# yhwu/rsicnv

Hardware: AMD Instinct MI355X
Metric: bases/sec through RSI pipeline (bin+GC+NB+segment) (higher is better)
Workload: dtype int32

## Files before the change

### include/rsi_hot.h

```cpp
#ifndef RSI_HOT_H
#define RSI_HOT_H
#include <stddef.h>
#include <stdint.h>
#ifdef __cplusplus
extern "C" {
#endif

typedef enum rsi_status {
  RSI_OK = 0,
  RSI_ERR_NO_DEVICE = -1,
  RSI_ERR_BAD_ARG = -2,
  RSI_ERR_HIP = -3,
  RSI_ERR_TOO_SMALL = -4,
  RSI_ERR_UNSUPPORTED = -5,
  RSI_ERR_INTERNAL = -6
} rsi_status;

typedef struct rsi_params {
  int32_t m;
  int32_t gcadjust;
  int32_t trans;
  int32_t merge;
  int32_t maxchkbp;
  int32_t debug;
// ... 259 lines not shown
void rsi_track_index_free(rsi_track_index* ix);
int rsi_hot_set_track_index(rsi_ctx* ctx, rsi_track_index* ix);
int rsi_track_index_append(rsi_track_index* dst, const rsi_track_index* src, int64_t shift);
int rsi_track_index_write_tbi(rsi_track_index* ix, const char* path);
int rsi_track_index_counts(const rsi_track_index* ix, int64_t* nref, int64_t* nchunks, int64_t* nwindows);
int64_t rsi_track_index_debug_tbi(const rsi_track_index* ix, uint8_t* out, int64_t cap);

int rsi_hot_loaded_depth(rsi_ctx* ctx, const void** d_depth, int64_t* n);
typedef struct rsi_depth_summary {
  int64_t n, sum;
  int64_t over;
  int64_t negative;
  int32_t min, max;
} rsi_depth_summary;
int rsi_hot_depth_summary(rsi_ctx* ctx, const void* d_depth, int64_t n, rsi_depth_summary* out, int64_t* dist, int dist_cap);
typedef struct rsi_depth_region { int64_t n, sum; int32_t min, max; } rsi_depth_region;
int rsi_hot_depth_regions(rsi_ctx* ctx, const void* d_depth, int64_t n, int nreg, const int64_t* start, const int64_t* end, rsi_depth_region* out);
int rsi_hot_write_window_track(rsi_ctx* ctx, const void* d_depth, int64_t n, const char* chrom, int64_t W, const char* path, int append,
                               rsi_track_stats* stats);
int rsi_hot_write_region_track(rsi_ctx* ctx, const void* d_depth, int64_t n, const char* chrom, int nreg, const int64_t* start,
                               const int64_t* end, const char* path, int append, rsi_track_stats* stats);
typedef struct rsi_depth_stats {
  int64_t launches;
  int64_t workgroups;
  int64_t bytes;
  double ms;
  double kernel_ms;
} rsi_depth_stats;
int rsi_hot_last_depth_stats(const rsi_ctx* ctx, rsi_depth_stats* out);
int rsi_hot_debug_depth_summary(rsi_ctx* ctx, const int32_t* values, int64_t n, int64_t span, rsi_depth_summary* out, int64_t* dist, int dist_cap);
int rsi_hot_debug_depth_regions(rsi_ctx* ctx, const int32_t* values, int64_t n, int tile, int nreg, const int64_t* start, const int64_t* end,
                                rsi_depth_region* out);
int64_t rsi_hot_debug_region_track(rsi_ctx* ctx, const int32_t* values, int64_t n, const char* chrom, int64_t W, int nreg, const int64_t* start,
                                   const int64_t* end, int span, int tile, int64_t slice_lines, int64_t pos0, char* out, int64_t cap,
                                   rsi_track_stats* stats);

int rsi_result_ncalls(const rsi_result* r, int which);
const rsi_call* rsi_result_calls(const rsi_result* r, int which);
const rsi_chrom_stats* rsi_result_stats(const rsi_result* r);
int rsi_result_noncode(const rsi_result* r, int32_t* pairs, int cap);
int rsi_result_format_row(const rsi_result* r, int i, const char* chrom, char* buf, int cap);
void rsi_result_free(rsi_result* r);

int64_t rsi_hot_fetch_i32(rsi_ctx* ctx, const char* name, int32_t* out, int64_t cap);
int64_t rsi_hot_fetch_f32(rsi_ctx* ctx, const char* name, float* out, int64_t cap);
int64_t rsi_hot_fetch_i64(rsi_ctx* ctx, const char* name, int64_t* out, int64_t cap);

int rsi_hot_debug_level_sums(rsi_ctx* ctx, const float* T, const int32_t* status, int64_t nb, int Lmax, float* sums, int32_t* counts);
int rsi_hot_debug_scan(rsi_ctx* ctx, const float* T, const int32_t* medint, int64_t nb, double RDmedian, double tmedian, double tlamda,
                       int Lmax, int32_t* status, int32_t* info);
int rsi_hot_debug_segments(rsi_ctx* ctx, const float* T, const int32_t* status, int64_t nb, const int32_t* runs, int nruns, double tmedian,
                           double tlamda, int64_t pairs_per_item, int32_t* seg_start, int32_t* seg_end, int32_t* seg_type, double* seg_score,
                           int32_t* info);
int rsi_hot_debug_sharpen(rsi_ctx* ctx, const int32_t* depth, int64_t n, int storage, int32_t* start, int32_t* end, const int32_t* type,
                          int njobs, int32_t* info);
typedef struct rsi_cand_record {
  int32_t capacity, top, margin, cut, nleft, nright;
  int32_t road;
  int32_t flags, nref, nbody, nwin, left_reach, right_reach, body_min, body_max;
  int32_t type, status, geno;
  double body_q[3], body_s1, body_s2, ref_q[3], ref_s1, ref_s2;
  double p1, cnvmed, cnvsd, cnviqr, refmed, refsd, refiqr;
} rsi_cand_record;
int rsi_hot_debug_candidate_tests(rsi_ctx* ctx, const int32_t* depth, int64_t n, int storage, int64_t span_all, double RDmedian, int m,
                                  double minmlen, double chklen, double buffer, int maxchkbp, const int32_t* start, const int32_t* end,
                                  const int32_t* type, const int32_t* status, int ncand, const int32_t* index, int nindex, int form,
                                  rsi_cand_record* out, int32_t* info);
int rsi_hot_debug_range_sums(rsi_ctx* ctx, const int32_t* depth, int64_t n, int storage, const int32_t* lo, const int32_t* hi, int nranges,
                             int64_t* sums, int32_t* info);
int rsi_hot_debug_block_stage(rsi_ctx* ctx, const int32_t* binmedint, const int32_t* status, int64_t nb, int64_t ncompact, double RDmedian,
                              const rsi_params* P, rsi_call* segs, int nsegs, int use_tester, int sparse, int32_t* road, int32_t* info);
int rsi_hot_debug_merge(rsi_ctx* ctx, const int32_t* depth, int64_t n, int storage, double RDmedian, const rsi_params* P, const rsi_call* list,
                        int nlist, int use_tester, rsi_call* out, int32_t* nout, int32_t* info);
int rsi_hot_debug_calls(rsi_ctx* ctx, const int32_t* depth, int64_t n, int storage, double RDmedian, double RDsd, const rsi_params* P,
                        const rsi_call* segs, int nsegs, const int32_t* noncode_start, const int32_t* noncode_end, int nnoncode, int use_tester,
                        rsi_call* blocks, rsi_call* raw, rsi_call* kept, int32_t* counts, int32_t* info);
int rsi_hot_debug_nb_transform(rsi_ctx* ctx, const int64_t* binsum, int64_t nb, int m, int64_t ncompact, double RDmedian, double r,
                               float* raw, float* T, int32_t* info);
int rsi_hot_debug_filterstatus(rsi_ctx* ctx, const float* T, const int32_t* status, int64_t nb, int Lmax, double dev, int32_t* status_out,
                               int32_t* info);
int rsi_hot_debug_grid_median(rsi_ctx* ctx, const float* x, const int32_t* mask, int64_t nb, int mode, double center, double* out,
                              int32_t* info);
int rsi_hot_debug_grid_mad_i32(rsi_ctx* ctx, const int32_t* x, int64_t nb, double center, double* out, int32_t* info);

int rsi_hot_debug_classify(rsi_ctx* ctx, const uint8_t* fasta, int64_t n, const int64_t* start, const int64_t* end, int count,
                           uint64_t* gcbits, uint64_t* nbits);

int rsi_hot_debug_per_base(rsi_ctx* ctx, const rsi_params* p, const int32_t* depth, const uint8_t* fasta, int64_t n, const int64_t* start,
                           const int64_t* end, int count, rsi_chrom_stats* out);

int rsi_hot_kernel_times(const rsi_ctx* ctx, const char** names, float* ms, int cap);
int rsi_hot_phase_times(const rsi_ctx* ctx, const char** names, double* ms, int cap);
void rsi_hot_set_timing(rsi_ctx* ctx, int on);
void rsi_hot_set_timing_kernel(rsi_ctx* ctx, const char* name);

typedef struct rsi_pool rsi_pool;
#define RSI_MAX_TIMED 64
typedef struct rsi_batch_times {
  int32_t nkernels, nphases;
  const char* kernel_name[RSI_MAX_TIMED];
  double kernel_ms[RSI_MAX_TIMED];
  int64_t kernel_launches[RSI_MAX_TIMED];
  int64_t kernel_bases[RSI_MAX_TIMED];
  const char* phase_name[RSI_MAX_TIMED];
  double phase_ms[RSI_MAX_TIMED];
} rsi_batch_times;

rsi_pool* rsi_pool_create(int device, int nworkers, int* status);
void rsi_pool_destroy(rsi_pool* pool);
int rsi_pool_workers(const rsi_pool* pool);
int rsi_pool_hw_queues(const rsi_pool* pool);
rsi_ctx* rsi_pool_worker(rsi_pool* pool, int w);
void rsi_pool_set_timing(rsi_pool* pool, int on);
void rsi_pool_set_timing_kernel(rsi_pool* pool, const char* name);
void rsi_pool_set_schedule(rsi_pool* pool, int isolate, int streamers);
const char* rsi_pool_last_error(const rsi_pool* pool);
int rsi_pool_run(rsi_pool* pool, const rsi_params* p, int nchrom, const void* const* d_depth,
                 const void* const* d_fasta, const int64_t* n, rsi_result** out, int* status,
                 rsi_batch_times* times);

int rsi_plot_expand(const int32_t* rdc, int64_t ncompact, const int32_t* regions, int npairs, int32_t* out, int64_t n);
int rsi_plot_write_files(const rsi_call* c, const char* title, const int32_t* rd, int64_t n, double chrom_median, int m,
                         double minmlen, double chklen, const char* format, double gnuplot_version, const char* datfile,
                         const char* gpfile, const char* imgfile);

typedef struct rsi_plot_batch rsi_plot_batch;
rsi_plot_batch* rsi_plot_batch_new(int64_t n, int m, double minmlen, double chklen);
void rsi_plot_batch_free(rsi_plot_batch* b);
int rsi_plot_batch_add(rsi_plot_batch* b, const rsi_call* c);
int rsi_plot_batch_add_span(rsi_plot_batch* b, int start, int end, int type);
int rsi_plot_batch_size(const rsi_plot_batch* b);
int rsi_plot_batch_refusal(const rsi_plot_batch* b, int i);
const char* rsi_plot_refusal_text(int refusal);
int64_t rsi_plot_batch_queries(const rsi_plot_batch* b);
int rsi_plot_batch_fill_host(rsi_plot_batch* b, const int32_t* rd, int64_t n);
double rsi_plot_batch_chrom_median(const rsi_plot_batch* b);
int rsi_plot_batch_compare(const rsi_plot_batch* a, const rsi_plot_batch* b);
int rsi_plot_batch_write(const rsi_plot_batch* b, int i, const char* title, const char* format, double gnuplot_version, const char* datfile,
                         const char* gpfile, const char* imgfile);
typedef struct rsi_plot_stats {
  int64_t launches, batches, tiles;
  int64_t calls, queries;
  int64_t bytes_up, bytes_down;
  int64_t bytes;
  double ms, expand_ms;
} rsi_plot_stats;
int rsi_hot_plot_depth(rsi_ctx* ctx, const void* d_depth, int64_t n, rsi_plot_batch* b);
int rsi_hot_plot_run(rsi_ctx* ctx, const rsi_result* res, rsi_plot_batch* b);
int rsi_hot_last_plot_stats(const rsi_ctx* ctx, rsi_plot_stats* out);
int rsi_hot_debug_plot(rsi_ctx* ctx, const int32_t* depth, int64_t n, int tile, int64_t workspace_bytes, rsi_plot_batch* b);
int rsi_hot_debug_plot_expand(rsi_ctx* ctx, const int32_t* rdc, int64_t ncompact, int storage, const int32_t* regions, int npairs, int32_t* out, int64_t n);

int rsi_pool_run_host(rsi_pool* pool, const rsi_params* p, int nchrom, const int32_t* const* depth,
                      const uint8_t* const* fasta, const int64_t* n, rsi_result** out, int* status,
                      rsi_batch_times* times);

uint64_t rsi_pool_submit(rsi_pool* pool, const rsi_params* p, int nchrom, const void* const* d_depth,
                         const void* const* d_fasta, const int64_t* n, rsi_result** out, int* status,
                         rsi_batch_times* times);
int rsi_pool_wait(rsi_pool* pool, uint64_t ticket);

#ifdef __cplusplus
}
#endif
#endif
```

### rsicnv_amd/api.py

```python
import contextlib
import ctypes as C
import os

import numpy as np

POOL_HW_QUEUES, MIN_HW_QUEUES = 32, 4


def _queue_count(s):
    return int(s) if s is not None and 1 <= len(s) <= 9 and all(c in "0123456789" for c in s) else -1


def _process_setup(env=os.environ):
    user = env.get("RSI_HOT_HW_QUEUES")
    if user != "keep":
        want = _queue_count(user)
        if want >= 0:
            env["GPU_MAX_HW_QUEUES"] = str(min(POOL_HW_QUEUES, max(MIN_HW_QUEUES, want)))
        elif _queue_count(env.get("GPU_MAX_HW_QUEUES")) < POOL_HW_QUEUES:
            env["GPU_MAX_HW_QUEUES"] = str(POOL_HW_QUEUES)
    return max(0, _queue_count(env.get("GPU_MAX_HW_QUEUES")))


HW_QUEUES = _process_setup()

_HERE = os.path.dirname(os.path.abspath(__file__))
LIB_PATH = os.environ.get("RSI_HOT_LIB") or os.path.join(_HERE, "librsi_hot.so")

RSI_OK = 0
STATUS_NAMES = {0: "RSI_OK", -1: "RSI_ERR_NO_DEVICE", -2: "RSI_ERR_BAD_ARG", -3: "RSI_ERR_HIP",
                -4: "RSI_ERR_TOO_SMALL", -5: "RSI_ERR_UNSUPPORTED", -6: "RSI_ERR_INTERNAL"}

CAND_RECORD = np.dtype([(k, np.int32) for k in ("capacity", "top", "margin", "cut", "nleft", "nright", "road", "flags", "nref", "nbody", "nwin",
                                                "left_reach", "right_reach", "body_min", "body_max", "type", "status", "geno")] +
                       [("body_q", np.float64, 3), ("body_s1", np.float64), ("body_s2", np.float64), ("ref_q", np.float64, 3),
                        ("ref_s1", np.float64), ("ref_s2", np.float64)] +
                       [(k, np.float64) for k in ("p1", "cnvmed", "cnvsd", "cnviqr", "refmed", "refsd", "refiqr")])
assert CAND_RECORD.itemsize == 18 * 4 + 17 * 8

CALL_RECORD = np.dtype([(k, np.int32) for k in ("start", "end", "type", "geno", "status", "length", "qscore", "pad")] +
                       [(k, np.float64) for k in ("score", "p1", "cnvmed", "cnvsd", "cnviqr", "refmed", "refsd", "refiqr")])
assert CALL_RECORD.itemsize == 8 * 4 + 8 * 8
LIST_INFO = ("spec_hits", "single_tests", "host_fallbacks", "block_batch_hits", "waits", "sum_launches", "sum_reused", "sum_redone", "tests")

GENO_RECORD = np.dtype([(k, np.int32) for k in ("n_body", "n_flank", "body_min", "body_max")] +
                       [("body_sum", np.int64), ("flank_sum", np.int64), ("body_q", np.float64, 3), ("flank_q", np.float64, 3),
                        ("chrom_median", np.float64)])
assert GENO_RECORD.itemsize == 4 * 4 + 2 * 8 + 7 * 8

DEPTH_SUMMARY = np.dtype([(k, np.int64) for k in ("n", "sum", "over", "negative")] + [("min", np.int32), ("max", np.int32)])
DEPTH_REGION = np.dtype([("n", np.int64), ("sum", np.int64), ("min", np.int32), ("max", np.int32)])
assert DEPTH_SUMMARY.itemsize == 40 and DEPTH_REGION.itemsize == 24
DEPTH_BINS = 65536

EXPORTS = ["rsi_default_params", "rsi_hot_create", "rsi_hot_destroy", "rsi_hot_last_error", "rsi_hot_run",
           "rsi_hot_run_device", "rsi_hot_load_depth_text", "rsi_hot_run_text", "rsi_hot_load_depth_bam", "rsi_hot_run_bam", "rsi_bam_references", "rsi_result_annotate_bam", "rsi_result_summary", "rsi_summary_format_row", "rsi_summary_format_rows", "rsi_result_pairs", "rsi_result_ncalls", "rsi_result_calls", "rsi_result_stats", "rsi_result_noncode",
           "rsi_result_format_row", "rsi_result_free", "rsi_hot_fetch_i32", "rsi_hot_fetch_f32", "rsi_hot_fetch_i64",
           "rsi_hot_kernel_times", "rsi_hot_phase_times", "rsi_hot_set_timing", "rsi_hot_process_setup", "rsi_pool_create", "rsi_pool_destroy", "rsi_pool_workers", "rsi_pool_hw_queues", "rsi_pool_worker",
           "rsi_pool_set_timing", "rsi_pool_set_timing_kernel", "rsi_hot_set_timing_kernel", "rsi_pool_set_schedule", "rsi_pool_last_error", "rsi_pool_run", "rsi_pool_run_host", "rsi_pool_submit", "rsi_pool_wait", "rsi_plot_expand", "rsi_plot_write_files", "rsi_result_log_line", "rsi_hot_debug_level_sums", "rsi_hot_debug_scan", "rsi_hot_debug_segments", "rsi_hot_debug_sharpen", "rsi_hot_debug_candidate_tests", "rsi_hot_debug_range_sums", "rsi_hot_debug_block_stage", "rsi_hot_debug_merge", "rsi_hot_debug_calls", "rsi_hot_debug_nb_transform", "rsi_hot_debug_filterstatus", "rsi_hot_debug_grid_median", "rsi_hot_debug_grid_mad_i32", "rsi_synth_generate_host", "rsi_synth_generate_device", "rsi_synth_write_depth_text", "rsi_synth_write_fasta", "rsi_synth_append_genome_text",
           "rsi_genome_text_open", "rsi_genome_text_next", "rsi_genome_text_release", "rsi_genome_text_copy_depth",
           "rsi_genome_text_kernel_ms", "rsi_genome_text_close", "rsi_genome_text_last_error", "rsi_hot_run_depth_device",
           "rsi_hot_last_inflate_stats", "rsi_hot_inflate_bgzf", "rsi_genome_text_inflate_stats",
           "rsi_synth_append_genome_bgzf", "rsi_genome_text_open_samples", "rsi_genome_text_samples", "rsi_genome_text_max_resident",
           "rsi_genome_text_sample_depth", "rsi_genome_text_copy_sample_depth", "rsi_synth_append_genome_samples",
           "rsi_genome_bedgraph_open", "rsi_synth_append_genome_bedgraph", "rsi_genome_bedgraph_open_indexed", "rsi_genome_text_index_range",
           "rsi_hot_set_exclude", "rsi_exclude_read_bed", "rsi_hot_debug_classify", "rsi_hot_debug_per_base",
           "rsi_hot_write_track", "rsi_hot_write_track_device", "rsi_hot_debug_track",
           "rsi_hot_write_bin_track", "rsi_hot_debug_bin_track",
           "rsi_hot_set_track_format", "rsi_hot_last_deflate_stats", "rsi_bgzf_write_eof", "rsi_hot_debug_deflate",
           "rsi_track_index_create", "rsi_track_index_free", "rsi_hot_set_track_index", "rsi_track_index_append",
           "rsi_track_index_write_tbi", "rsi_track_index_counts", "rsi_track_index_debug_tbi",
           "rsi_ref_open", "rsi_ref_close", "rsi_ref_last_error", "rsi_ref_count", "rsi_ref_sequence", "rsi_ref_find", "rsi_ref_format",
           "rsi_ref_index_path", "rsi_ref_load_device", "rsi_ref_load_host", "rsi_ref_device_alloc", "rsi_ref_device_free",
           "rsi_hot_run_text_dfasta", "rsi_hot_run_bam_dfasta",
           "rsi_hot_set_bam_read", "rsi_hot_last_bam_read_stats",
           "rsi_hot_set_bam_pairs", "rsi_result_annotate_device", "rsi_hot_last_pairs_stats", "rsi_hot_debug_pair_sample",
           "rsi_hot_debug_pair_annotate",
           "rsi_hot_set_bam_pin", "rsi_hot_stat_calls", "rsi_hot_pin_sample", "rsi_hot_pin_calls", "rsi_hot_last_pin_stats",
           "rsi_hot_debug_pin_sample", "rsi_hot_debug_pin_calls",
           "rsi_hot_geno_calls", "rsi_hot_last_geno_stats", "rsi_hot_debug_geno",
           "rsi_hot_loaded_depth", "rsi_hot_depth_summary", "rsi_hot_depth_regions", "rsi_hot_write_window_track", "rsi_hot_write_region_track",
           "rsi_hot_last_depth_stats", "rsi_hot_debug_depth_summary", "rsi_hot_debug_depth_regions", "rsi_hot_debug_region_track",
           "rsi_plot_batch_new", "rsi_plot_batch_free", "rsi_plot_batch_add", "rsi_plot_batch_add_span", "rsi_plot_batch_size",
           "rsi_plot_batch_refusal", "rsi_plot_refusal_text", "rsi_plot_batch_queries", "rsi_plot_batch_fill_host",
           "rsi_plot_batch_chrom_median", "rsi_plot_batch_compare", "rsi_plot_batch_write", "rsi_hot_plot_depth", "rsi_hot_plot_run", "rsi_hot_last_plot_stats",
           "rsi_hot_debug_plot", "rsi_hot_debug_plot_expand",
           "rsi_ref_debug_set_chunks", "rsi_ref_debug_fai_line", "rsi_ref_debug_ranges", "rsi_ref_debug_gzi", "rsi_ref_debug_cover"]


class RsiParams(C.Structure):
    _fields_ = [("m", C.c_int32), ("gcadjust", C.c_int32), ("trans", C.c_int32), ("merge", C.c_int32),
                ("maxchkbp", C.c_int32), ("debug", C.c_int32), ("cap", C.c_double), ("epsilon", C.c_double),
                ("threshold", C.c_double), ("chklen", C.c_double), ("minmlen", C.c_double),
                ("buffer", C.c_double), ("p", C.c_double)]


class RsiCall(C.Structure):
    _fields_ = [("start", C.c_int32), ("end", C.c_int32), ("type", C.c_int32), ("geno", C.c_int32),
                ("status", C.c_int32), ("length", C.c_int32), ("qscore", C.c_int32), ("pad", C.c_int32),
                ("score", C.c_double), ("p1", C.c_double), ("cnvmed", C.c_double), ("cnvsd", C.c_double),
                ("cnviqr", C.c_double), ("refmed", C.c_double), ("refsd", C.c_double), ("refiqr", C.c_double)]


class RsiChromStats(C.Structure):
    _fields_ = [("n", C.c_int64), ("n_compact", C.c_int64), ("nbins", C.c_int64), ("n_noncode", C.c_int32),
                ("Lmax", C.c_int32), ("gc_rdmean", C.c_double), ("cap_median", C.c_double), ("RDmedian", C.c_double),
                ("RDsd", C.c_double), ("nb_mad", C.c_double), ("nb_r", C.c_double), ("nb_tmin", C.c_double),
                ("tmedian1", C.c_double), ("tsigma1", C.c_double), ("tlamda1", C.c_double), ("tmedian2", C.c_double),
                ("tsigma2", C.c_double), ("tlamda2", C.c_double), ("trim_escapes", C.c_int32),
                ("inexact_sums", C.c_int32), ("t_device_ms", C.c_double), ("t_kernels_ms", C.c_double),
                ("byte_escapes", C.c_int64), ("scan_tiles", C.c_int32), ("scan_tiles_listed", C.c_int32)]


RSI_MAX_TIMED = 64
SUMMARY_HEAD, SUMMARY_CALL = 8, 8


class RsiTextStats(C.Structure):
    _fields_ = [("bytes", C.c_int64), ("lines", C.c_int64), ("stored", C.c_int64), ("beyond", C.c_int64),
                ("fallback", C.c_int32), ("pad", C.c_int32), ("t_total_ms", C.c_double), ("t_parse_kernel_ms", C.c_double)]


class RsiInflateStats(C.Structure):
    _fields_ = [("format", C.c_int32), ("eof_block", C.c_int32), ("input_error", C.c_int32), ("pad", C.c_int32), ("compressed_bytes", C.c_int64), ("text_bytes", C.c_int64),
                ("blocks", C.c_int64), ("t_inflate_kernel_ms", C.c_double), ("t_host_inflate_ms", C.c_double)]


class RsiTrackStats(C.Structure):
    _fields_ = [("n", C.c_int64), ("lines", C.c_int64), ("bytes", C.c_int64), ("slices", C.c_int64),
                ("t_total_ms", C.c_double), ("t_kernel_ms", C.c_double), ("t_write_ms", C.c_double)]


class RsiDeflateStats(C.Structure):
    _fields_ = [("members", C.c_int64), ("stored_members", C.c_int64), ("text_bytes", C.c_int64), ("file_bytes", C.c_int64),
                ("t_kernel_ms", C.c_double)]


INFLATE_FORMATS = {0: "text", 1: "bgzf", 2: "gzip"}
TRACK_FORMATS = {"text": 0, "bgzf": 1}


class RsiRefSeq(C.Structure):
# ... 589 lines not shown
                              maxchkbp=100000):
        d = np.ascontiguousarray(depth, dtype=np.int32)
        c = np.ascontiguousarray(cands, dtype=np.int32).reshape(-1, 4)
        cols = [np.ascontiguousarray(c[:, j]) for j in range(4)]
        ix = np.ascontiguousarray(index, dtype=np.int32).reshape(-1)
        out = np.zeros(max(ix.size, 1), dtype=CAND_RECORD)
        info = np.zeros(8, dtype=np.int32)
        self.lib.rsi_hot_debug_candidate_tests.argtypes = [C.c_void_p, C.c_void_p, C.c_int64, C.c_int, C.c_int64, C.c_double, C.c_int, C.c_double,
                                                           C.c_double, C.c_double, C.c_int, C.c_void_p, C.c_void_p, C.c_void_p, C.c_void_p, C.c_int,
                                                           C.c_void_p, C.c_int, C.c_int, C.c_void_p, C.c_void_p]
        self._check(self.lib.rsi_hot_debug_candidate_tests(self.ctx, d.ctypes.data, d.size, int(storage), int(span_all), float(RDmedian), int(m),
                                                           float(minmlen), float(chklen), float(buffer), int(maxchkbp), cols[0].ctypes.data,
                                                           cols[1].ctypes.data, cols[2].ctypes.data, cols[3].ctypes.data, c.shape[0],
                                                           ix.ctypes.data, ix.size, int(form), out.ctypes.data, info.ctypes.data))
        return out[:ix.size], info

    def debug_range_sums(self, depth, storage, lo, hi):
        d = np.ascontiguousarray(depth, dtype=np.int32)
        a = np.ascontiguousarray(lo, dtype=np.int32).reshape(-1)
        b = np.ascontiguousarray(hi, dtype=np.int32).reshape(-1)
        assert a.size == b.size
        sums = np.zeros(max(a.size, 1), dtype=np.int64)
        info = np.zeros(2, dtype=np.int32)
        self.lib.rsi_hot_debug_range_sums.argtypes = [C.c_void_p, C.c_void_p, C.c_int64, C.c_int, C.c_void_p, C.c_void_p, C.c_int, C.c_void_p, C.c_void_p]
        self._check(self.lib.rsi_hot_debug_range_sums(self.ctx, d.ctypes.data, d.size, int(storage), a.ctypes.data, b.ctypes.data, a.size,
                                                      sums.ctypes.data, info.ctypes.data))
        return sums[:a.size], info

    def debug_block_stage(self, binmedint, status, segs, ncompact, RDmedian, tester=True, sparse=False, **params):
        b = np.ascontiguousarray(binmedint, dtype=np.int32)
        st = np.ascontiguousarray(status, dtype=np.int32)
        assert b.size == st.size
        L = np.array(segs, dtype=CALL_RECORD).reshape(-1)
        road = np.full(max(L.size, 1), -1, dtype=np.int32)
        info = np.zeros(10, dtype=np.int32)
        P = make_params(**params)
        self.lib.rsi_hot_debug_block_stage.argtypes = [C.c_void_p, C.c_void_p, C.c_void_p, C.c_int64, C.c_int64, C.c_double, C.c_void_p, C.c_void_p,
                                                       C.c_int, C.c_int, C.c_int, C.c_void_p, C.c_void_p]
        self._check(self.lib.rsi_hot_debug_block_stage(self.ctx, b.ctypes.data, st.ctypes.data, b.size, int(ncompact), float(RDmedian), C.addressof(P),
                                                       L.ctypes.data, L.size, int(bool(tester)), int(bool(sparse)), road.ctypes.data, info.ctypes.data))
        return L, road[:L.size], dict(zip(LIST_INFO, (int(v) for v in info)))

    def debug_merge(self, depth, storage, cands, RDmedian, tester=True, **params):
        d = np.ascontiguousarray(depth, dtype=np.int32)
        L = np.ascontiguousarray(np.array(cands, dtype=CALL_RECORD).reshape(-1))
        out = np.zeros(max(L.size, 1), dtype=CALL_RECORD)
        nout = np.zeros(1, dtype=np.int32)
        info = np.zeros(10, dtype=np.int32)
        P = make_params(**params)
        self.lib.rsi_hot_debug_merge.argtypes = [C.c_void_p, C.c_void_p, C.c_int64, C.c_int, C.c_double, C.c_void_p, C.c_void_p, C.c_int, C.c_int,
                                                 C.c_void_p, C.c_void_p, C.c_void_p]
        self._check(self.lib.rsi_hot_debug_merge(self.ctx, d.ctypes.data, d.size, int(storage), float(RDmedian), C.addressof(P), L.ctypes.data, L.size,
                                                 int(bool(tester)), out.ctypes.data, nout.ctypes.data, info.ctypes.data))
        return out[:int(nout[0])], dict(zip(LIST_INFO, (int(v) for v in info)))

    def debug_calls(self, depth, storage, segs, noncode, RDmedian, RDsd, tester=True, **params):
        d = np.ascontiguousarray(depth, dtype=np.int32)
        L = np.ascontiguousarray(np.array(segs, dtype=CALL_RECORD).reshape(-1))
        nc = np.asarray(noncode, dtype=np.int32).reshape(-1, 2)
        a, b = np.ascontiguousarray(nc[:, 0]), np.ascontiguousarray(nc[:, 1])
        outs = [np.zeros(max(L.size, 1), dtype=CALL_RECORD) for _ in range(3)]
        counts = np.zeros(3, dtype=np.int32)
        info = np.zeros(10, dtype=np.int32)
        P = make_params(**params)
        self.lib.rsi_hot_debug_calls.argtypes = [C.c_void_p, C.c_void_p, C.c_int64, C.c_int, C.c_double, C.c_double, C.c_void_p, C.c_void_p, C.c_int,
                                                 C.c_void_p, C.c_void_p, C.c_int, C.c_int, C.c_void_p, C.c_void_p, C.c_void_p, C.c_void_p, C.c_void_p]
        self._check(self.lib.rsi_hot_debug_calls(self.ctx, d.ctypes.data, d.size, int(storage), float(RDmedian), float(RDsd), C.addressof(P),
                                                 L.ctypes.data, L.size, a.ctypes.data if a.size else None, b.ctypes.data if b.size else None, a.size,
                                                 int(bool(tester)), outs[0].ctypes.data, outs[1].ctypes.data, outs[2].ctypes.data, counts.ctypes.data,
                                                 info.ctypes.data))
        return outs[0][:counts[0]], outs[1][:counts[1]], outs[2][:counts[2]], dict(zip(LIST_INFO, (int(v) for v in info)))

    def debug_nb_transform(self, binsum, m, ncompact, RDmedian, r):
        b = np.ascontiguousarray(binsum, dtype=np.int64)
        raw = np.zeros(b.size, dtype=np.float32)
        T = np.zeros(b.size, dtype=np.float32)
        info = np.zeros(8, dtype=np.int32)
        self.lib.rsi_hot_debug_nb_transform.argtypes = [C.c_void_p, C.c_void_p, C.c_int64, C.c_int, C.c_int64, C.c_double, C.c_double, C.c_void_p,
                                                        C.c_void_p, C.c_void_p]
        self._check(self.lib.rsi_hot_debug_nb_transform(self.ctx, b.ctypes.data, b.size, int(m), int(ncompact), float(RDmedian), float(r),
                                                        raw.ctypes.data, T.ctypes.data, info.ctypes.data))
        return raw, T, info

    def debug_filterstatus(self, T, status, Lmax, dev):
        t = np.ascontiguousarray(T, dtype=np.float32)
        st = np.ascontiguousarray(status, dtype=np.int32)
        assert st.size == t.size
        out = np.zeros(t.size, dtype=np.int32)
        info = np.zeros(10, dtype=np.int32)
        self.lib.rsi_hot_debug_filterstatus.argtypes = [C.c_void_p, C.c_void_p, C.c_void_p, C.c_int64, C.c_int, C.c_double, C.c_void_p, C.c_void_p]
        self._check(self.lib.rsi_hot_debug_filterstatus(self.ctx, t.ctypes.data, st.ctypes.data, t.size, int(Lmax), float(dev), out.ctypes.data,
                                                        info.ctypes.data))
        return out, info

    GRID_MODES = {"pair": 0, "mad": 1, "host": 2}

    def debug_grid_median(self, x, mask=None, mode="pair", center=0.0):
        out = np.zeros(4, dtype=np.float64)
        info = np.zeros(8, dtype=np.int32)
        if mode == "med":
            assert mask is None
            xi = np.ascontiguousarray(x, dtype=np.int32)
            self.lib.rsi_hot_debug_grid_mad_i32.argtypes = [C.c_void_p, C.c_void_p, C.c_int64, C.c_double, C.c_void_p, C.c_void_p]
            self._check(self.lib.rsi_hot_debug_grid_mad_i32(self.ctx, xi.ctypes.data, xi.size, float(center), out.ctypes.data, info.ctypes.data))
            return out, info
        xf = np.ascontiguousarray(x, dtype=np.float32)
        mk = None if mask is None else np.ascontiguousarray(mask, dtype=np.int32)
        assert mk is None or mk.size == xf.size
        self.lib.rsi_hot_debug_grid_median.argtypes = [C.c_void_p, C.c_void_p, C.c_void_p, C.c_int64, C.c_int, C.c_double, C.c_void_p, C.c_void_p]
        self._check(self.lib.rsi_hot_debug_grid_median(self.ctx, xf.ctypes.data, None if mk is None else mk.ctypes.data, xf.size,
                                                       self.GRID_MODES[mode], float(center), out.ctypes.data, info.ctypes.data))
        return out, info

    def set_exclude(self, exclude):
        if exclude is None or len(exclude) == 0:
            self._check(self.lib.rsi_hot_set_exclude(self.ctx, None, None, 0))
            return
        s, e = _interval_arrays(exclude)
        self._check(self.lib.rsi_hot_set_exclude(self.ctx, s.ctypes.data, e.ctypes.data, s.size))

    def debug_classify(self, fasta, exclude=None):
        f = np.ascontiguousarray(fasta, dtype=np.uint8)
        gc = np.zeros(f.size // 64 + 1, dtype=np.uint64)
        nb = np.zeros(f.size // 64 + 1, dtype=np.uint64)
        if exclude is None or len(exclude) == 0:
            rc = self.lib.rsi_hot_debug_classify(self.ctx, f.ctypes.data, f.size, None, None, 0, gc.ctypes.data, nb.ctypes.data)
        else:
            s, e = _interval_arrays(exclude)
            rc = self.lib.rsi_hot_debug_classify(self.ctx, f.ctypes.data, f.size, s.ctypes.data, e.ctypes.data, s.size, gc.ctypes.data, nb.ctypes.data)
        self._check(rc)
        return gc, nb

    def debug_per_base(self, params, depth, fasta, exclude=None):
        d = np.ascontiguousarray(depth, dtype=np.int32)
        f = np.ascontiguousarray(fasta, dtype=np.uint8)
        if d.shape != f.shape or d.ndim != 1:
            raise ValueError("depth and fasta must be 1-D arrays of the same length")
        st = RsiChromStats()
        if exclude is None or len(exclude) == 0:
            rc = self.lib.rsi_hot_debug_per_base(self.ctx, C.byref(params), d.ctypes.data, f.ctypes.data, d.size, None, None, 0, C.byref(st))
        else:
            s, e = _interval_arrays(exclude)
            rc = self.lib.rsi_hot_debug_per_base(self.ctx, C.byref(params), d.ctypes.data, f.ctypes.data, d.size, s.ctypes.data, e.ctypes.data,
                                                 s.size, C.byref(st))
        self.last_stats = {k[0]: getattr(st, k[0]) for k in RsiChromStats._fields_}
        self._check(rc)
        return self.last_stats

    def run(self, params, depth, fasta, exclude=None):
        d = np.ascontiguousarray(depth, dtype=np.int32)
        f = np.ascontiguousarray(fasta, dtype=np.uint8)
        if d.shape != f.shape or d.ndim != 1:
            raise ValueError("depth and fasta must be 1-D arrays of the same length")
        out = C.c_void_p()
        if exclude is not None:
            self.set_exclude(exclude)
        self._check(self.lib.rsi_hot_run(self.ctx, C.byref(params), d.ctypes.data, f.ctypes.data, d.size, C.byref(out)))
        return Result(self.lib, out)

    def load_depth_text(self, path, n):
        st = RsiTextStats()
        self._check(self.lib.rsi_hot_load_depth_text(self.ctx, os.fsencode(path), int(n), C.byref(st)))
        return {f[0]: getattr(st, f[0]) for f in RsiTextStats._fields_ if f[0] != "pad"}

    def inflate_bgzf(self, data):
        data = bytes(data)
# ... 728 lines not shown
```

### rsicnv_amd/csrc/kernels.h

```cpp
#pragma once
#include <hip/hip_runtime.h>
#include <stdint.h>
#include <mutex>
#include "device_util.h"
#include "bam_walk_core.h"

namespace rsik {

inline void note_launch() {
  const hipError_t e = hipGetLastError();
  if (e != hipSuccess && tl_launch_error == hipSuccess) tl_launch_error = e;
}
inline void drain_stale_errors() { (void)hipGetLastError(); tl_launch_error = hipSuccess; }
inline hipError_t take_launch_error() { const hipError_t e = tl_launch_error; tl_launch_error = hipSuccess; return e; }
#define RSI_LAUNCH(...) do { hipLaunchKernelGGL(__VA_ARGS__); rsik::note_launch(); } while (0)

constexpr int kGcLevels = 202;
constexpr int kHistValues = 65536;
constexpr int kResClasses = 32;
constexpr int kTileBases = 4096;

void launch_fasta_classify(const uint8_t* fasta, int64_t n, uint64_t* gcbits, uint64_t* nbits, int64_t nwords,
                           const FillList& fill, hipStream_t stream);
void launch_fill(const FillList& fill, hipStream_t stream);
// ... 44 lines not shown
                        hipStream_t stream);

size_t gc_rescale_slab_bytes(int64_t n);
void launch_gc_rescale(const int32_t* depth, const uint64_t* gcbits, int64_t n, const double* table,
                       int adjust, int32_t* out, uint32_t* hist, ValueHistAux* aux, void* slabs, void* gsum,
                       unsigned int* counters, ValueMedian* vm, const void* head_src, void* head_dst, size_t head_bytes,
                       hipStream_t stream, uint8_t* out8 = nullptr,
                       PhaseParams* pp = nullptr ,
                       double cap_mult = 0.0);
void launch_gc_materialize(const int32_t* depth, const uint64_t* gcbits, int64_t n, const double* table, int32_t* out,
                           unsigned int* counter, hipStream_t stream);
size_t value_hist8_slab_bytes(int64_t n);
void launch_value_hist8(const uint8_t* depth8, const int32_t* depth, const uint64_t* gcbits, int64_t n, const double* table,
                        uint32_t* hist, ValueHistAux* aux, void* slabs, void* gsum, unsigned int* counters, ValueMedian* vm,
                        const void* head_src, void* head_dst, size_t head_bytes, uint8_t* rescaled8 ,
                        const unsigned int* escapes , hipStream_t stream);
unsigned int byte_escape_limit(int64_t n);

struct BinAccum {
  unsigned long long big;
  unsigned int vmax;
  unsigned int pad;
};
constexpr int kRegInline = 48;
struct K4Regions { long long brk[kRegInline]; long long cum[kRegInline + 1]; };
struct K4Form { int vr = 0, sw7 = -1, parts = 0, tile_bins = 0, tmpl = -1; };
struct K4Args {
  const int32_t* src; const uint8_t* src8; const uint64_t* gcbits; int64_t n; const double* table;
  const int64_t* cbreak; const int64_t* cum; const K4Regions* inl; int nreg; int64_t ncompact; int32_t capval; int m;
  uint8_t* rdc8; int32_t* rdc; int32_t* binmed; int64_t* binsum; uint32_t* res_hist; BinAccum* acc;
  void* slabs; void* gsum; unsigned int* counters; const void* exp_src; void* exp_dst; size_t exp_bytes;
  const unsigned int* rtab; const unsigned int* escapes; PhaseParams* pp; int vbase; int raw; hipStream_t stream;
  K4Form* form;
};
size_t cap_compact_slab_bytes(int m, int32_t capval, int64_t ncompact, int vbase);
int cap_compact_overwrites(int m, int32_t capval, int64_t ncompact, int vbase);
constexpr int kK4Window = 512;
int hist_window_base(double center, int width);
void launch_cap_compact_bin(const K4Args& a);

int cap_compact16_applies(int m, int32_t capval, int64_t ncompact);
size_t cap_compact16_slab_bytes(int m, int64_t ncompact);
void launch_cap_compact_bin16(const K4Args& a);

int cap_compact8_applies(int m, int32_t capval);
size_t cap_compact8_slab_bytes(int m, int32_t capval, int64_t ncompact);
struct ByteShape { int vr; bool sw7; bool operator==(const ByteShape& o) const { return vr == o.vr && sw7 == o.sw7; } };
inline ByteShape byte_shape(int32_t capval) { int vr = 64; while (vr < 256 && vr <= capval) vr <<= 1; return {vr, capval <= 127}; }
void launch_cap_compact_bin8(const K4Args& a);

void launch_rescale_compact_bin8(const K4Args& a);

int rescale_compact_split_applies(int m, int32_t capval, int64_t ncompact, int nreg);
size_t rescale_compact_split_slab_bytes(int32_t capval, int64_t ncompact);
size_t rescale_compact_split_rdc_bytes(int64_t ncompact);
void launch_rescale_compact_stream(const K4Args& a);
void launch_bin_median8(const K4Args& a);

struct PerBaseSwitches {
  bool joint;
  bool spec;
  bool k4j_fix;
  bool k4split;
  bool nogc_bytes;
  bool k4w;
  bool k1b_inside;
};
enum class K4Route { stream, joint, bytes, wide16, int32 };
struct K4Plan {
  K4Route route;
  bool fixed;
  bool raw;
  bool bytes_fit;
  ByteShape shape;
  const char* marks[2];
};
K4Plan k4_plan(bool gcadjust, bool capped, int32_t capval, int m, int64_t ncompact, int nreg, bool deep, bool joint_ok,
               const PerBaseSwitches& sw);

void launch_nb_raw(const int64_t* binsum, int64_t nb, int m, int64_t ncompact, double r, float* raw,
                   uint32_t* rawmin_bits, hipStream_t stream);
struct MinMaxF { uint32_t min_inv, max_bits; unsigned int nonfinite; unsigned int pad; };
struct GridMedian { double med, ymin; unsigned long long count; uint32_t np, flags; };
enum { kGridEmpty = 1, kGridNonFinite = 2, kGridDegenerate = 4, kGridTooWide = 8 };
struct GridChain { MinMaxF* mm; uint32_t* hist; uint32_t cap; unsigned int* counters; };
struct GridExport { const void* src[2]; void* dst[2]; size_t bytes[2]; };

void launch_nb_scale_minmax(float* x, int64_t nb, const uint32_t* rawmin_bits, double med_raw, double del_raw, double dup_raw,
                            double RDmedian, const GridChain& c, GridMedian* out, hipStream_t stream);
void launch_i32_to_f32_minmax(const int32_t* in, float* out_f, int64_t nb, double center, const GridChain& c, GridMedian* out,
                              hipStream_t stream);
void launch_minmax_f32(const float* x, const int32_t* mask, int64_t nb, int use_abs, double center, MinMaxF* mm,
                       hipStream_t stream);
void launch_hist_f32(const float* x, const int32_t* mask, int64_t nb, int use_abs, double center, double ymin,
                     uint32_t* hist, uint32_t np, hipStream_t stream);
void launch_minmax_plan(const float* x, const int32_t* mask, int64_t nb, int use_abs, double center, const double* d_center,
                        const GridChain& c, GridMedian* out, hipStream_t stream);
void launch_hist_walk(const float* x, const int32_t* mask, int64_t nb, int use_abs, double center, const double* d_center,
                      const GridChain& c, GridMedian* out, const GridExport* ex, const FillList* fill, hipStream_t stream);
bool hist_walk_pack16(int64_t nb);

struct ScanParams {
  int64_t nb;
  int32_t Lmax;
  int16_t pad;
  int16_t kcap;
  double tmedian;
  double lim_del;
  double lim_dup;
};
constexpr int kMaxScanL = 10400;
constexpr int kScanLdsL = 3800;
constexpr int kScanPad = 8;
constexpr int kThrInline = 232;
struct ScanThr { double del[kThrInline]; double dup[kThrInline]; };
void launch_rsi_scan(const float* T, const int32_t* medint, const ScanParams& sp, const double* thr_del,
                     const double* thr_dup, const ScanThr* inl, uint32_t* first_del, uint32_t* first_dup, uint32_t* counters,
                     uint32_t* tiles, void* tile_ws , hipStream_t stream);
size_t scan_tile_workspace_bytes(int Lmax);
constexpr int kMaxLevels = 10416;
inline int scan_level_stride(int Lmax) { return (Lmax + 1 + kScanPad + 3) & ~3; }
constexpr int kScanRecEscapes = 0, kScanRecInexact = 1, kScanRecStop = 2 , kScanRecTiles = 8, kScanRecLevels = 16;
constexpr size_t kScanWorkBytes = 64 + 2 * (size_t)kMaxLevels * 4;
void launch_level_stop(const uint32_t* first_del, const uint32_t* first_dup, int64_t nb, int32_t Lmax, uint32_t* work, void* both,
                       unsigned int* counter, void* host_copy, size_t host_bytes, hipStream_t stream);
void launch_resolve_runs(const uint32_t* first_del, const uint32_t* first_dup, const uint32_t* levels, int64_t nb, int32_t* status,
                         int32_t* copy, uint64_t* runs, uint32_t* count, uint32_t cap, unsigned int* counter, void* host_copy,
                         uint32_t host_entries, hipStream_t stream);

struct BestSeg { double score; int32_t start; int32_t len; };
struct SegItem { int32_t run; int32_t len; int32_t Lbeg; int32_t Lend; };
constexpr int kRunsInline = 200, kItemsInline = 150;
constexpr int kBestLds = 6144;
struct RunsInline { int32_t se[2 * kRunsInline]; int32_t off[kRunsInline]; };
struct ItemsInline { SegItem it[kItemsInline]; int32_t off[kRunsInline]; };
void launch_run_prefix(const float* T, const int32_t* run_start, const int32_t* run_end, const RunsInline* inl, int nruns,
                       const int64_t* poff, double* scratch, const int32_t* status, int32_t* status_out, hipStream_t stream);
void launch_best_items(const void* items, const ItemsInline* inl, int nitems, const int64_t* poff, const double* scratch,
                       double tmedian, BestSeg* out, hipStream_t stream);
void launch_trim_runs(const float* T, int32_t* status, const int32_t* run_start, const int32_t* run_end, const RunsInline* inl,
                      int nruns, double delthr, double addthr, hipStream_t stream);

size_t level_sums_head_bytes(int Lmax_cap);
size_t level_sums_workspace_bytes(int64_t nb, int32_t clist_cap, int Lmax_cap);
void launch_level_sums(const float* T, const int32_t* status, int64_t nb, int Lmax, void* ws, int Lmax_cap, int32_t clist_cap, float* out,
                       unsigned int* counter, void* host_copy, hipStream_t stream);

constexpr int kMaxDevices = 16;
void report_attribute_failure(const char* kernel, const char* what);
#define RSI_ALLOW_FULL_LDS(kernel)                                                                                  \
  do {                                                                                                              \
    static std::once_flag once__[rsik::kMaxDevices];                                                                \
    int dev__ = 0;                                                                                                  \
    if (hipGetDevice(&dev__) != hipSuccess || dev__ < 0 || dev__ >= rsik::kMaxDevices) dev__ = 0;                   \
    std::call_once(once__[dev__], [dev__] {                                                                         \
      hipFuncAttributes a__;                                                                                        \
      int lds__ = 0;                                                                                                \
      if (hipFuncGetAttributes(&a__, reinterpret_cast<const void*>(kernel)) != hipSuccess) {                        \
        rsik::report_attribute_failure(#kernel, "hipFuncGetAttributes"); return;                                    \
      }                                                                                                             \
      if (hipDeviceGetAttribute(&lds__, hipDeviceAttributeMaxSharedMemoryPerBlock, dev__) != hipSuccess || lds__ <= 0) \
        lds__ = 160 * 1024;                                                                                         \
      if (hipFuncSetAttribute(reinterpret_cast<const void*>(kernel), hipFuncAttributeMaxDynamicSharedMemorySize,   \
                              lds__ - (int)a__.sharedSizeBytes) != hipSuccess)                                      \
        rsik::report_attribute_failure(#kernel, "hipFuncSetAttribute(MaxDynamicSharedMemorySize)");                 \
    });                                                                                                             \
  } while (0)

constexpr unsigned kCandHistBins = 16384;
struct EdgeJob {
  int32_t start, end, type, pad;
};
struct CandJob {
  int32_t start, end;
  int32_t kind;
  int32_t margin;
  int32_t capacity;
  int32_t top;
  int32_t nleft, nright;
  int32_t left_off, right_off;
  int32_t budget;
  int32_t cut;
  double right_cap;
// ... 211 lines not shown
```

### rsicnv_amd/csrc/kernels_bin.hip

```cpp
#include <type_traits>
#include "kernels.h"
#include "device_util.h"

namespace rsik {

namespace {

constexpr int kThreads = 256;
constexpr int kMaxGrid = 256 * 2;

__device__ inline int lane_id() { return threadIdx.x & 63; }
inline int grid_for(int64_t items, int per_block) {
  int64_t g = (items + per_block - 1) / per_block;
  if (g < 1) g = 1;
  if (g > kMaxGrid) g = kMaxGrid;
  return (int)g;
}

__device__ inline uint32_t f32_key(float f) {
  const uint32_t b = __float_as_uint(f);
  return (b & 0x80000000u) ? ~b : (b | 0x80000000u);
}

__global__ __launch_bounds__(kThreads) void k_nb_raw(const int64_t* __restrict__ binsum, int64_t nb, int m,
                                                     int64_t ncompact, double r, float* __restrict__ raw,
                                                     uint32_t* __restrict__ rawmin_key) {
  uint32_t kmin = 0xffffffffu;
  for (int64_t b = (int64_t)blockIdx.x * kThreads + threadIdx.x; b < nb; b += (int64_t)gridDim.x * kThreads) {
    const int64_t i1 = b * m;
    int64_t i2 = b * m + m - 1;
    if (i2 > ncompact - 1) i2 = ncompact - 1;
    const double m2 = (double)(i2 - i1 + 1);
    const double sum = (double)binsum[b];
    const double q = (sum + 0.25) / (m2 * r - 0.5);
    const double t = 2.0 * sqrt(r) * log(sqrt(q) + sqrt(1.0 + q));
    const float f = (float)t;
    raw[b] = f;
    const uint32_t k = f32_key(f);
    kmin = k < kmin ? k : kmin;
  }
  for (int d = 32; d >= 1; d >>= 1) { const uint32_t o = __shfl_xor(kmin, d); kmin = o < kmin ? o : kmin; }
  __shared__ uint32_t s_min[kThreads / 64];
  if (lane_id() == 0) s_min[threadIdx.x >> 6] = kmin;
  __syncthreads();
  if (threadIdx.x == 0) {
    for (int w = 1; w < kThreads / 64; ++w) kmin = s_min[w] < kmin ? s_min[w] : kmin;
    if (kmin != 0xffffffffu) atomicMax(rawmin_key, ~kmin);
  }
}

__device__ inline float sel_value(const float* __restrict__ x, int64_t i, int use_abs, double center) {
  const float v = x[i];
  return use_abs ? (float)fabs((double)v - center) : v;
}

__device__ __forceinline__ void minmax_body(const float* __restrict__ x, const int32_t* __restrict__ mask, int64_t nb,
                                            int use_abs, double center, MinMaxF* __restrict__ mm) {
  uint32_t kmin = 0xffffffffu, kmax = 0;
  unsigned int bad = 0;
  for (int64_t i = (int64_t)blockIdx.x * kThreads + threadIdx.x; i < nb; i += (int64_t)gridDim.x * kThreads) {
    if (mask && mask[i] != 0) continue;
    const float v = sel_value(x, i, use_abs, center);
    if (!(fabsf(v) <= 3.0e38f)) bad = 1;
    const uint32_t k = f32_key(v);
    kmin = k < kmin ? k : kmin;
    kmax = k > kmax ? k : kmax;
  }
  for (int d = 32; d >= 1; d >>= 1) {
    const uint32_t a = __shfl_xor(kmin, d), b = __shfl_xor(kmax, d);
    kmin = a < kmin ? a : kmin; kmax = b > kmax ? b : kmax; bad |= __shfl_xor(bad, d);
  }
  __shared__ uint32_t s_min[kThreads / 64], s_max[kThreads / 64], s_bad[kThreads / 64];
  if (lane_id() == 0) { s_min[threadIdx.x >> 6] = kmin; s_max[threadIdx.x >> 6] = kmax; s_bad[threadIdx.x >> 6] = bad; }
  __syncthreads();
  if (threadIdx.x == 0) {
    for (int w = 1; w < kThreads / 64; ++w) { kmin = s_min[w] < kmin ? s_min[w] : kmin; kmax = s_max[w] > kmax ? s_max[w] : kmax; bad |= s_bad[w]; }
    if (kmin != 0xffffffffu) atomicMax(&mm->min_inv, ~kmin);
    if (kmax != 0) atomicMax(&mm->max_bits, kmax);
    if (bad) atomicOr(&mm->nonfinite, 1u);
  }
}

__global__ __launch_bounds__(kThreads) void k_minmax_f32(const float* __restrict__ x, const int32_t* __restrict__ mask,
                                                         int64_t nb, int use_abs, double center, MinMaxF* __restrict__ mm) {
  minmax_body(x, mask, nb, use_abs, center, mm);
}
constexpr uint32_t kLdsBins = 12288;

constexpr int kHistRun = 8;

template <bool PACK16 = false>
__device__ __forceinline__ void hist_body(const float* __restrict__ x, const int32_t* __restrict__ mask, int64_t nb, int use_abs,
                                          double center, double ymin, uint32_t* __restrict__ hist, uint32_t np, int use_lds,
                                          unsigned int* s_h) {
  const uint32_t nl = use_lds ? (np < (uint32_t)use_lds ? np : (uint32_t)use_lds) : 0;
  auto lds_add = [&](uint32_t k, uint32_t c) { if (PACK16) atomicAdd(&s_h[k >> 1], c << ((k & 1u) << 4)); else atomicAdd(&s_h[k], c); };
  auto bucket = [&](float v) {
    const double idx = ((double)v - ymin) / 0.01 + 0.5;
    uint32_t k = (uint32_t)(unsigned long long)idx;
    return k >= np ? np - 1 : k;
  };
  __shared__ uint32_t s_wb;
  if (threadIdx.x == 0) s_wb = 0u;
  if (use_lds) { for (uint32_t e = threadIdx.x; e < (PACK16 ? (nl + 1) / 2 : nl); e += kThreads) s_h[e] = 0; }
  if (use_lds && np > nl && threadIdx.x < 64) {
    const int lane = (int)threadIdx.x;
    const int64_t i = (int64_t)(((unsigned long long)(2 * lane + 1) * (unsigned long long)nb) >> 7);
    const bool valid = i < nb && !(mask && mask[i] != 0);
    const uint32_t k = valid ? bucket(sel_value(x, i, use_abs, center)) : 0xffffffffu;
    int rank = 0;
    for (int j = 0; j < 64; ++j) {
      const uint32_t kj = (uint32_t)__builtin_amdgcn_readlane((int)k, j);
      rank += (kj < k || (kj == k && j < lane)) ? 1 : 0;
    }
    const int nvalid = __popcll(__ballot(valid));
    if (valid && rank == nvalid / 2) s_wb = k < nl / 2 ? 0u : (k - nl / 2 > np - nl ? np - nl : k - nl / 2);
  }
  if (use_lds) __syncthreads();
  const uint32_t wb = use_lds ? s_wb : 0u;
  auto count = [&](uint32_t k, uint32_t c) { if (k - wb < nl) lds_add(k - wb, c); else atomicAdd(&hist[k], c); };
  const int64_t nchunks = (nb + kHistRun - 1) / kHistRun;
  for (int64_t c = (int64_t)blockIdx.x * kThreads + threadIdx.x; c < nchunks; c += (int64_t)gridDim.x * kThreads) {
    uint32_t pend_k = 0xffffffffu, pend_c = 0;
    const int64_t i0 = c * kHistRun, i1 = i0 + kHistRun < nb ? i0 + kHistRun : nb;
    auto one = [&](float xv) {
      const float v = use_abs ? (float)fabs((double)xv - center) : xv;
      const uint32_t k = bucket(v);
      if (k != pend_k) {
        if (pend_c) count(pend_k, pend_c);
        pend_k = k; pend_c = 0;
      }
      ++pend_c;
    };
    if (i1 - i0 == kHistRun) {
      static_assert(kHistRun == 8, "two quads per run");
      const float4 a = *reinterpret_cast<const float4*>(x + i0), b = *reinterpret_cast<const float4*>(x + i0 + 4);
      int4 ma = make_int4(0, 0, 0, 0), mb = ma;
      if (mask) { ma = *reinterpret_cast<const int4*>(mask + i0); mb = *reinterpret_cast<const int4*>(mask + i0 + 4); }
      const float xv[8] = {a.x, a.y, a.z, a.w, b.x, b.y, b.z, b.w};
      const int mv[8] = {ma.x, ma.y, ma.z, ma.w, mb.x, mb.y, mb.z, mb.w};
#pragma unroll
      for (int e = 0; e < 8; ++e) if (mv[e] == 0) one(xv[e]);
    } else {
      for (int64_t i = i0; i < i1; ++i) {
        if (mask && mask[i] != 0) continue;
        one(x[i]);
      }
    }
    if (pend_c) count(pend_k, pend_c);
  }
  if (use_lds) {
    __syncthreads();
    for (uint32_t e = threadIdx.x; e < nl; e += kThreads) {
      const unsigned int c = PACK16 ? (s_h[e >> 1] >> ((e & 1u) << 4)) & 0xffffu : s_h[e];
      if (c) atomicAdd(&hist[wb + e], c);
    }
  }
}

__global__ __launch_bounds__(kThreads) void k_hist_f32(const float* __restrict__ x, const int32_t* __restrict__ mask,
                                                       int64_t nb, int use_abs, double center, double ymin,
                                                       uint32_t* __restrict__ hist, uint32_t np, int use_lds) {
  extern __shared__ unsigned int s_h[];
  hist_body(x, mask, nb, use_abs, center, ymin, hist, np, use_lds, s_h);
}

__device__ inline float f32_unkey(uint32_t k) { return __uint_as_float((k & 0x80000000u) ? (k & 0x7fffffffu) : ~k); }

__device__ inline void grid_plan_block(MinMaxF* __restrict__ mm, uint32_t cap, uint32_t* __restrict__ hist, GridMedian* __restrict__ g) {
  const uint32_t kmin = ~ld_cg(&mm->min_inv), kmax = ld_cg(&mm->max_bits), bad = ld_cg(&mm->nonfinite);
  uint32_t flags = 0, np = 0;
  double ymin = 0.0;
  if (kmin == 0xffffffffu) flags = kGridEmpty;
  else if (bad) flags = kGridNonFinite;
  else {
    ymin = (double)f32_unkey(kmin);
    const double ymax = (double)f32_unkey(kmax);
    if ((ymax - ymin) < 0.01) flags = kGridDegenerate;
    else {
      const size_t n = (size_t)((ymax - ymin) / 0.01 + 2);
      if (n > cap) flags = kGridTooWide; else np = (uint32_t)n;
    }
  }
  for (uint32_t e = threadIdx.x; e < np; e += kThreads) hist[e] = 0;
  __syncthreads();
  if (threadIdx.x == 0) {
    g->med = 0.0; g->ymin = ymin; g->count = 0; g->np = np; g->flags = flags;
    mm->min_inv = 0; mm->max_bits = 0; mm->nonfinite = 0;
  }
}

__device__ inline void minmax_commit(uint32_t kmin, uint32_t kmax, unsigned int bad, MinMaxF* __restrict__ mm) {
  for (int d = 32; d >= 1; d >>= 1) {
    const uint32_t a = __shfl_xor(kmin, d), b = __shfl_xor(kmax, d);
    kmin = a < kmin ? a : kmin; kmax = b > kmax ? b : kmax; bad |= __shfl_xor(bad, d);
  }
  __shared__ uint32_t s_min[kThreads / 64], s_max[kThreads / 64], s_bad[kThreads / 64];
  if (lane_id() == 0) { s_min[threadIdx.x >> 6] = kmin; s_max[threadIdx.x >> 6] = kmax; s_bad[threadIdx.x >> 6] = bad; }
  __syncthreads();
  if (threadIdx.x == 0) {
    for (int w = 1; w < kThreads / 64; ++w) { kmin = s_min[w] < kmin ? s_min[w] : kmin; kmax = s_max[w] > kmax ? s_max[w] : kmax; bad |= s_bad[w]; }
    if (kmin != 0xffffffffu) atomicMax(&mm->min_inv, ~kmin);
    if (kmax != 0) atomicMax(&mm->max_bits, kmax);
    if (bad) atomicOr(&mm->nonfinite, 1u);
  }
}

__global__ __launch_bounds__(kThreads) void k_minmax_plan(const float* __restrict__ x, const int32_t* __restrict__ mask,
                                                          int64_t nb, int use_abs, double center, const double* __restrict__ center_ptr,
                                                          MinMaxF* __restrict__ mm, unsigned int* __restrict__ counter, uint32_t cap,
                                                          uint32_t* __restrict__ hist, GridMedian* __restrict__ g) {
  const double c = center_ptr ? *center_ptr : center;
  uint32_t kmin = 0xffffffffu, kmax = 0;
  unsigned int bad = 0;
  auto one = [&](float xv) {
    const float v = use_abs ? (float)fabs((double)xv - c) : xv;
    if (!(fabsf(v) <= 3.0e38f)) bad = 1;
    const uint32_t k = f32_key(v);
    kmin = k < kmin ? k : kmin;
    kmax = k > kmax ? k : kmax;
  };
  const int64_t stride = (int64_t)gridDim.x * kThreads;
  int64_t i = (int64_t)blockIdx.x * kThreads + threadIdx.x;
  for (; i + 3 * stride < nb; i += 4 * stride) {
    float xv[4]; int mv[4] = {0, 0, 0, 0};
#pragma unroll
    for (int e = 0; e < 4; ++e) xv[e] = x[i + e * stride];
    if (mask) {
#pragma unroll
      for (int e = 0; e < 4; ++e) mv[e] = mask[i + e * stride];
    }
#pragma unroll
    for (int e = 0; e < 4; ++e) if (mv[e] == 0) one(xv[e]);
  }
  for (; i < nb; i += stride) {
    if (mask && mask[i] != 0) continue;
    one(x[i]);
  }
  minmax_commit(kmin, kmax, bad, mm);
  if (last_block_done(counter)) grid_plan_block(mm, cap, hist, g);
}

struct ExportPair { const void* src[2]; void* dst[2]; unsigned int bytes[2]; };

__device__ inline void grid_walk_block(const uint32_t* __restrict__ hist, GridMedian* __restrict__ g) {
  __shared__ unsigned long long s_sum[kThreads];
  __shared__ unsigned long long s_seen;
  __shared__ unsigned int s_cross;
  const uint32_t np = g->np;
  const uint32_t chunk = (((np + kThreads - 1) / kThreads) + 3u) & ~3u;
  const uint32_t b0 = threadIdx.x * chunk < np ? threadIdx.x * chunk : np;
  const uint32_t b1 = b0 + chunk < np ? b0 + chunk : np;
  const __amdgpu_buffer_rsrc_t rs = coherent_buffer(hist);
  unsigned long long mine = 0;
  for (uint32_t b = b0; b < b1; b += 32) {
    u32x4 v[8];
#pragma unroll
    for (int j = 0; j < 8; ++j) { const uint32_t q = b + 4u * j; v[j] = ld_cg_buf_x4(rs, (q < b1 ? q : b0) * 4u, 0u); }
#pragma unroll
    for (int j = 0; j < 8; ++j) {
      const uint32_t q = b + 4u * j;
      const unsigned int c[4] = {v[j].x, v[j].y, v[j].z, v[j].w};
#pragma unroll
      for (int e = 0; e < 4; ++e) mine += q + e < b1 ? c[e] : 0u;
    }
  }
  s_sum[threadIdx.x] = mine;
  if (threadIdx.x == 0) s_cross = 0xffffffffu;
  __syncthreads();
  unsigned long long seen = 0, total = 0;
  for (int t = 0; t < kThreads; ++t) { const unsigned long long v = s_sum[t]; if (t < (int)threadIdx.x) seen += v; total += v; }
  const unsigned long long r2 = total / 2;
  unsigned long long* med_bits = reinterpret_cast<unsigned long long*>(&g->med);
  if (threadIdx.x == 0) { st_cg(&g->count, total); if (r2 == 0) st_cg(med_bits, (unsigned long long)__double_as_longlong(g->ymin)); }
  if (r2 != 0 && mine != 0 && seen < r2 && seen + mine >= r2) { s_cross = b0; s_seen = seen; }
  __syncthreads();
  const uint32_t cb = s_cross;
  if (cb == 0xffffffffu) return;
  const unsigned long long before = s_seen;
  const uint32_t ce = cb + chunk < np ? cb + chunk : np;
  const uint32_t per = (chunk + kThreads - 1) / kThreads;
  const uint32_t m0 = cb + threadIdx.x * per < ce ? cb + threadIdx.x * per : ce;
  const uint32_t m1 = m0 + per < ce ? m0 + per : ce;
  unsigned long long part = 0;
  for (uint32_t bb = m0; bb < m1; ++bb) part += ld_cg(hist + bb);
  __syncthreads();
  s_sum[threadIdx.x] = part;
  __syncthreads();
  unsigned long long run = before;
  for (int t = 0; t < (int)threadIdx.x; ++t) run += s_sum[t];
  if (part != 0 && run < r2 && run + part >= r2) {
    for (uint32_t bb = m0; bb < m1; ++bb) {
      const unsigned long long upto = run + ld_cg(hist + bb);
      if (run < r2 && upto >= r2) st_cg(med_bits, (unsigned long long)__double_as_longlong(g->ymin + (double)bb * 0.01));
      run = upto;
    }
  }
}

template <bool PACK16>
__global__ __launch_bounds__(kThreads) void k_hist_walk(const float* __restrict__ x, const int32_t* __restrict__ mask,
                                                        int64_t nb, int use_abs, double center,
                                                        const double* __restrict__ center_ptr,
                                                        GridMedian* __restrict__ g, uint32_t* __restrict__ hist,
                                                        unsigned int* __restrict__ counter, ExportPair ex, FillList fill, uint32_t lds_bins) {
  extern __shared__ unsigned int s_h[];
  fill_ranges(fill);
  if (!g->flags) {
    const uint32_t np = g->np;
    hist_body<PACK16>(x, mask, nb, use_abs, center_ptr ? *center_ptr : center, g->ymin, hist, np, (int)lds_bins, s_h);
  }
  if (!last_block_done(counter)) return;
  if (!g->flags) grid_walk_block(hist, g);
  sync_drained();
  for (int k = 0; k < 2; ++k) export_words(ex.dst[k], ex.src[k], ex.bytes[k]);
}

struct NbLevels { double med_raw, del_raw, dup_raw, RDmedian; };
__global__ __launch_bounds__(kThreads) void k_nb_scale_mm(float* __restrict__ x, int64_t nb, const uint32_t* __restrict__ rawmin_inv,
                                                          NbLevels lv, MinMaxF* __restrict__ mm, unsigned int* __restrict__ counter,
                                                          uint32_t cap, uint32_t* __restrict__ hist, GridMedian* __restrict__ g) {
  const uint32_t key = ~(*rawmin_inv);
  const double tmin = (double)__uint_as_float((key & 0x80000000u) ? (key & 0x7fffffffu) : ~key);
  const double med_nbt = lv.med_raw - tmin;
  const double del_s = (lv.del_raw - tmin) / med_nbt * lv.RDmedian, dup_s = (lv.dup_raw - tmin) / med_nbt * lv.RDmedian;
  const double med_s = med_nbt / med_nbt * lv.RDmedian;
  const float lev0 = (float)del_s, lev1 = (float)dup_s, lev2 = (float)med_s;
  uint32_t kmin = 0xffffffffu, kmax = 0;
  unsigned int bad = 0;
  for (int64_t b = (int64_t)blockIdx.x * kThreads + threadIdx.x; b < nb; b += (int64_t)gridDim.x * kThreads) {
    float v = x[b];
    v = (float)((double)v - tmin);
    v = (float)((double)v / med_nbt * lv.RDmedian);
    if (b == 0) v = lev0;
    if (b == 1) v = lev1;
    if (b == 2) v = lev2;
    x[b] = v;
    if (!(fabsf(v) <= 3.0e38f)) bad = 1;
    const uint32_t k = f32_key(v);
    kmin = k < kmin ? k : kmin;
    kmax = k > kmax ? k : kmax;
  }
  minmax_commit(kmin, kmax, bad, mm);
  if (last_block_done(counter)) grid_plan_block(mm, cap, hist, g);
}

__global__ __launch_bounds__(kThreads) void k_i32_to_f32_mm(const int32_t* __restrict__ in, float* __restrict__ out, int64_t nb,
                                                            double center, MinMaxF* __restrict__ mm, unsigned int* __restrict__ counter,
                                                            uint32_t cap, uint32_t* __restrict__ hist, GridMedian* __restrict__ g) {
  uint32_t kmin = 0xffffffffu, kmax = 0;
  unsigned int bad = 0;
  for (int64_t b = (int64_t)blockIdx.x * kThreads + threadIdx.x; b < nb; b += (int64_t)gridDim.x * kThreads) {
    const float f = (float)in[b];
    out[b] = f;
    const float v = (float)fabs((double)f - center);
    if (!(fabsf(v) <= 3.0e38f)) bad = 1;
    const uint32_t k = f32_key(v);
    kmin = k < kmin ? k : kmin;
    kmax = k > kmax ? k : kmax;
  }
  minmax_commit(kmin, kmax, bad, mm);
  if (last_block_done(counter)) grid_plan_block(mm, cap, hist, g);
}

constexpr int kScanTile = 256;
constexpr uint32_t kUnmarked = 0xffffffffu;

template <class IX>
struct ScanLdsT {
  using index = IX;
  double* P;
  double* tot;
  uint32_t* TB;
  int* M;
  IX* CB;
  IX* RB;
  IX* PF;
  int stride;
  int count, kcap;
  __device__ IX& C(int q, int x) const { return CB[(size_t)q * stride + x]; }
  __device__ IX& R(int q, int r) const { return RB[(size_t)q * stride + r]; }
  __device__ uint32_t* level(int side, int k) const { return TB + ((size_t)side * (kcap + 1) + k) * count; }
};
enum { kCL = 0, kCG = 1, kCTd = 2, kCTu = 3 };
constexpr int kScanNarrowL = 32000;

__host__ __device__ inline size_t scan_lds_bytes(int count, int kcap, int ix_bytes = 2) {
  size_t b = ((size_t)(count + 1) + kThreads) * sizeof(double);
  b += 2 * (size_t)(kcap + 1) * count * 4 + (size_t)count * 4;
  b += 9 * (size_t)(count + 2) * ix_bytes;
  return b;
}
template <class SL>
__device__ inline void scan_lds_carve(SL& S, double* sm, int count, int kcap) {
  S.count = count; S.kcap = kcap; S.stride = count + 2;
  S.P = sm;
  S.tot = S.P + count + 1;
  S.TB = reinterpret_cast<uint32_t*>(S.tot + kThreads);
  S.M = reinterpret_cast<int*>(S.TB + 2 * (size_t)(kcap + 1) * count);
  S.CB = reinterpret_cast<typename SL::index*>(S.M + count);
  S.RB = S.CB + 4 * (size_t)S.stride;
  S.PF = S.RB + 4 * (size_t)S.stride;
}

template <class SL>
__device__ inline int scan_next(const SL& S, int q, int x, int vhi) {
  const int r = S.C(q, x);
  return r < (int)S.C(q, S.count) ? (int)S.R(q, r) : vhi;
}
template <class SL>
__device__ inline int scan_prev(const SL& S, int q, int x, int vlo) {
  const int r = S.C(q, x + 1);
  return r > 0 ? (int)S.R(q, r - 1) : vlo - 1;
}
template <class SL>
__device__ inline void scan_mark(const SL& S, int side, int lo, int hi, int L) {
  const int len = hi - lo + 1;
  int k = 31 - __clz(len);
  k = k > S.kcap ? S.kcap : k;
  const int step = 1 << k;
  uint32_t* tab = S.level(side, k);
  for (int a = lo; a + step - 1 < hi; a += step) atomicMin(&tab[a], (uint32_t)L);
  atomicMin(&tab[hi - step + 1], (uint32_t)L);
}

template <class SL>
__device__ __noinline__ long long scan_hit_slow(int count, int kcap, int w0, int L, int side, int vlo, int vhi, int ends,
                                                uint32_t* counters, double* gtile ) {
  extern __shared__ __align__(16) double sm[];
  SL S;
  if (gtile) scan_lds_carve(S, gtile, count, kcap); else scan_lds_carve(S, sm, count, kcap);
  const int qm = side ? kCG : kCL, qt = side ? kCTu : kCTd;
  int i1 = scan_next(S, qt, w0, vhi);
  i1 = scan_next(S, qm, i1, vhi);
  int i2 = scan_prev(S, qt, w0 + L - 1, vlo);
  i2 = scan_prev(S, qm, i2, vlo);
  if (i1 >= vhi || i2 < vlo) {
    if ((i1 >= vhi && (ends & 2)) || (i2 < vlo && (ends & 1))) atomicAdd(&counters[0], 1u);
    return -1;
  }
  if (i1 <= i2) scan_mark(S, side, i1, i2, L);
  return (long long)i1 | ((long long)i2 << 32);
}

struct ScanTile { int vlo, vhi, fl_del, ce_dup, ends; double lim_del, lim_dup; double* gtile; };
// ... 650 lines not shown
#pragma unroll
      for (int u = 0; u < 4; ++u) { const int L = L0 + u; sum[u] = (L < it.Lend && j + L <= it.len) ? Q[j + L] - pj : 0.0; }
#pragma unroll
      for (int u = 0; u < 4; ++u) {
        const int L = L0 + u;
        if (L < it.Lend && j + L <= it.len) {
          const double score = fabs(sum[u] / dL[u] - tmedian) * sq[u];
          if (seg_better(score, L, j, bs, bL, bj)) { bs = score; bL = L; bj = j; }
        }
      }
    }
  }
  s_s[threadIdx.x] = bs; s_L[threadIdx.x] = bL; s_j[threadIdx.x] = bj;
  __syncthreads();
  for (int d = kThreads / 2; d >= 1; d >>= 1) {
    if ((int)threadIdx.x < d) {
      if (seg_better(s_s[threadIdx.x + d], s_L[threadIdx.x + d], s_j[threadIdx.x + d], s_s[threadIdx.x], s_L[threadIdx.x], s_j[threadIdx.x])) {
        s_s[threadIdx.x] = s_s[threadIdx.x + d]; s_L[threadIdx.x] = s_L[threadIdx.x + d]; s_j[threadIdx.x] = s_j[threadIdx.x + d];
      }
    }
    __syncthreads();
  }
  if (threadIdx.x == 0) { out[blockIdx.x].score = s_s[0]; out[blockIdx.x].start = s_j[0]; out[blockIdx.x].len = s_L[0]; }
}

}

static int bounded_grid(int64_t n, int per_block, int cap) { const int g = grid_for(n, per_block); return g > cap ? cap : g; }
void launch_nb_raw(const int64_t* binsum, int64_t nb, int m, int64_t ncompact, double r, float* raw, uint32_t* rawmin_bits,
                   hipStream_t stream) {
  int grid = grid_for(nb, kThreads * 4);
  if (grid > 1024) grid = 1024;
  RSI_LAUNCH(k_nb_raw, dim3(grid), dim3(kThreads), 0, stream, binsum, nb, m, ncompact, r, raw, rawmin_bits);
}
void launch_nb_scale_minmax(float* x, int64_t nb, const uint32_t* rawmin_bits, double med_raw, double del_raw, double dup_raw,
                            double RDmedian, const GridChain& c, GridMedian* out, hipStream_t stream) {
  NbLevels lv{med_raw, del_raw, dup_raw, RDmedian};
  RSI_LAUNCH(k_nb_scale_mm, dim3(bounded_grid(nb, kThreads * 4, 512)), dim3(kThreads), 0, stream, x, nb, rawmin_bits, lv, c.mm, c.counters, c.cap,
                     c.hist, out);
}
void launch_i32_to_f32_minmax(const int32_t* in, float* out_f, int64_t nb, double center, const GridChain& c, GridMedian* out,
                              hipStream_t stream) {
  RSI_LAUNCH(k_i32_to_f32_mm, dim3(bounded_grid(nb, kThreads * 4, 512)), dim3(kThreads), 0, stream, in, out_f, nb, center, c.mm, c.counters, c.cap,
                     c.hist, out);
}
void launch_minmax_f32(const float* x, const int32_t* mask, int64_t nb, int use_abs, double center, MinMaxF* mm,
                       hipStream_t stream) {
  RSI_LAUNCH(k_minmax_f32, dim3(grid_for(nb, kThreads * 16)), dim3(kThreads), 0, stream, x, mask, nb, use_abs, center, mm);
}
void launch_hist_f32(const float* x, const int32_t* mask, int64_t nb, int use_abs, double center, double ymin, uint32_t* hist,
                     uint32_t np, hipStream_t stream) {
  const int use_lds = (int)kLdsBins;
  const size_t lds = (size_t)(np < kLdsBins ? np : kLdsBins) * 4;
  RSI_ALLOW_FULL_LDS(k_hist_f32);
  int grid = grid_for(nb, kThreads * kHistRun * 8);
  if (grid > 128) grid = 128;
  RSI_LAUNCH(k_hist_f32, dim3(grid), dim3(kThreads), lds, stream, x, mask, nb, use_abs, center, ymin, hist, np, use_lds);
}
void launch_minmax_plan(const float* x, const int32_t* mask, int64_t nb, int use_abs, double center, const double* d_center,
                        const GridChain& c, GridMedian* out, hipStream_t stream) {
  RSI_LAUNCH(k_minmax_plan, dim3(bounded_grid(nb, kThreads * 16, 256)), dim3(kThreads), 0, stream, x, mask, nb, use_abs, center, d_center, c.mm,
                     c.counters, c.cap, c.hist, out);
}
static int hist_walk_grid(int64_t nb) { const int g = grid_for(nb, kThreads * kHistRun * 2); return g > 256 ? 256 : g; }
bool hist_walk_pack16(int64_t nb) {
  const int64_t run = (int64_t)kThreads * kHistRun, stride = (int64_t)hist_walk_grid(nb) * run;
  const int64_t tail = nb % stride;
  const int64_t most = nb / stride * run + (tail < run ? tail : run);
  return most < 65536;
}
void launch_hist_walk(const float* x, const int32_t* mask, int64_t nb, int use_abs, double center, const double* d_center,
                      const GridChain& c, GridMedian* out, const GridExport* ex, const FillList* fill, hipStream_t stream) {
  const uint32_t bins = kLdsBins;
  const int grid = hist_walk_grid(nb);
  const bool pack16 = hist_walk_pack16(nb);
  const size_t lds = pack16 ? (size_t)bins * 2 : (size_t)bins * 4;
  ExportPair e{};
  if (ex) for (int k = 0; k < 2; ++k) { e.src[k] = ex->src[k]; e.dst[k] = ex->dst[k]; e.bytes[k] = (unsigned int)ex->bytes[k]; }
  FillList f{};
  if (fill) f = *fill;
  if (pack16) RSI_LAUNCH(k_hist_walk<true>, dim3(grid), dim3(kThreads), lds, stream, x, mask, nb, use_abs, center, d_center, out, c.hist, c.counters + 1, e, f, bins);
  else { RSI_ALLOW_FULL_LDS(k_hist_walk<false>); RSI_LAUNCH(k_hist_walk<false>, dim3(grid), dim3(kThreads), lds, stream, x, mask, nb, use_abs, center, d_center, out, c.hist, c.counters + 1, e, f, bins); }
}
constexpr int kGTileGrid = 256;
constexpr size_t kGTileBudget = size_t(8) << 30;
struct ScanShape { int count, kcap, grid; bool gtile, wide; size_t tile_bytes; };
static ScanShape scan_tile_shape(int Lmax) {
  ScanShape sh;
  const int halo = Lmax / 2 + 1;
  sh.count = kScanTile + 2 * halo;
  sh.kcap = 0;
  while ((2 << sh.kcap) <= Lmax && sh.kcap < 6) ++sh.kcap;
  sh.gtile = Lmax > kScanLdsL;
  sh.wide = Lmax > kScanNarrowL;
  if (!sh.gtile) while (sh.kcap > 0 && scan_lds_bytes(sh.count, sh.kcap) + 4 * kThreads * sizeof(int) + 1024 > 160 * 1024) --sh.kcap;
  sh.tile_bytes = scan_lds_bytes(sh.count, sh.kcap, sh.wide ? 4 : 2);
  sh.grid = kGTileGrid;
  if (sh.gtile) {
    const size_t slice = (sh.tile_bytes + 255) & ~size_t(255);
    if (slice * (size_t)sh.grid > kGTileBudget) sh.grid = (int)std::max<size_t>(1, kGTileBudget / slice);
  }
  return sh;
}
size_t scan_tile_workspace_bytes(int Lmax) {
  const ScanShape sh = scan_tile_shape(Lmax);
  return sh.gtile ? (size_t)sh.grid * ((sh.tile_bytes + 255) & ~size_t(255)) : 0;
}
void launch_rsi_scan(const float* T, const int32_t* medint, const ScanParams& sp_in, const double* thr_del, const double* thr_dup,
                     const ScanThr* inl, uint32_t* first_del, uint32_t* first_dup, uint32_t* counters, uint32_t* tiles, void* tile_ws,
                     hipStream_t stream) {
  ScanParams sp = sp_in;
  const ScanShape sh = scan_tile_shape(sp.Lmax);
  const bool gtile = sh.gtile;
  sp.kcap = (int16_t)sh.kcap;
  const size_t tile_bytes = sh.tile_bytes;
  const size_t lds = gtile ? 0 : tile_bytes;
  const unsigned long long gbytes = (tile_bytes + 255) & ~size_t(255);
  const int64_t ntiles = (sp.nb + kScanTile - 1) / kScanTile;
  static const ScanThr none{};
  const char* det_env = getenv("RSI_HOT_SCAN_DETECT");
  const size_t dlds = detect_lds_bytes(sp.Lmax);
  const bool detect = tiles != nullptr && !(det_env && atoi(det_env) == 0) && dlds + kThreads * 8 + 64 <= 160 * 1024;
  int parts = 1;
  if (detect || gtile) {
    const int groups = (sp.Lmax + kScanPad - 1) / kScanPad;
    parts = groups < kScanPartsMax ? groups : kScanPartsMax;
    if (const char* pe = getenv("RSI_HOT_SCAN_PARTS")) { const int v = atoi(pe); if (v >= 1 && v <= groups) parts = v; }
  }
  if (detect) {
    const int dgrid = (int)((sp.nb + kDetBins - 1) / kDetBins);
    if (inl) { RSI_ALLOW_FULL_LDS(k_scan_detect<true>); RSI_LAUNCH(k_scan_detect<true>, dim3(dgrid), dim3(kThreads), dlds, stream, T, sp.nb, sp.Lmax, nullptr, nullptr, tiles, counters, *inl); }
    else { RSI_ALLOW_FULL_LDS(k_scan_detect<false>); RSI_LAUNCH(k_scan_detect<false>, dim3(dgrid), dim3(kThreads), dlds, stream, T, sp.nb, sp.Lmax, thr_del, thr_dup, tiles, counters, none); }
  }
  int64_t grid = ntiles * parts;
  const int64_t resident = gtile ? sh.grid : 256 * (int64_t)(lds > 80 * 1024 ? 1 : lds > 52 * 1024 ? 2 : lds > 39 * 1024 ? 3 : 4);
  if ((detect || gtile) && grid > resident) grid = resident;
  const uint32_t* list = detect ? tiles : nullptr;
  unsigned char* gws = static_cast<unsigned char*>(tile_ws);
#define RSI_SCAN(INL_, GT_, WIDE_, ...) do { RSI_ALLOW_FULL_LDS((k_rsi_scan<INL_, GT_, WIDE_>));                                             \
    RSI_LAUNCH((k_rsi_scan<INL_, GT_, WIDE_>), dim3((unsigned)grid), dim3(kThreads), lds, stream, T, medint, sp, __VA_ARGS__, first_del, first_dup, \
               counters, list, parts, inl ? *inl : none, gws, gbytes); } while (0)
  if (gtile && sh.wide) RSI_SCAN(false, true, true, thr_del, thr_dup);
  else if (gtile) { if (inl) RSI_SCAN(true, true, false, nullptr, nullptr); else RSI_SCAN(false, true, false, thr_del, thr_dup); }
  else { if (inl) RSI_SCAN(true, false, false, nullptr, nullptr); else RSI_SCAN(false, false, false, thr_del, thr_dup); }
#undef RSI_SCAN
}
void launch_level_stop(const uint32_t* first_del, const uint32_t* first_dup, int64_t nb, int32_t Lmax, uint32_t* work, void* both,
                       unsigned int* counter, void* host_copy, size_t host_bytes, hipStream_t stream) {
  const size_t lds = (size_t)(Lmax + 1) * 8;
  if (lds + 256 <= 160 * 1024) {
    RSI_ALLOW_FULL_LDS(k_level_stop<false>);
    RSI_LAUNCH(k_level_stop<false>, dim3(grid_for(nb, kThreads * 16)), dim3(kThreads), lds, stream, first_del, first_dup, nb,
                       Lmax, work, static_cast<uint2*>(both), counter, host_copy, (unsigned int)host_bytes);
  } else {
    RSI_LAUNCH(k_level_stop<true>, dim3(grid_for(nb, kThreads * 16)), dim3(kThreads), 0, stream, first_del, first_dup, nb,
                       Lmax, work, static_cast<uint2*>(both), counter, host_copy, (unsigned int)host_bytes);
  }
}
void launch_resolve_runs(const uint32_t* first_del, const uint32_t* first_dup, const uint32_t* levels, int64_t nb, int32_t* status,
                         int32_t* copy, uint64_t* runs, uint32_t* count, uint32_t cap, unsigned int* counter, void* host_copy,
                         uint32_t host_entries, hipStream_t stream) {
  RSI_LAUNCH(k_resolve_runs, dim3(grid_for(nb, kThreads * 4)), dim3(kThreads), 0, stream, first_del, first_dup, levels, nb, status, copy,
                     runs, count, cap, counter, host_copy, host_entries);
}
void launch_trim_runs(const float* T, int32_t* status, const int32_t* run_start, const int32_t* run_end, const RunsInline* inl, int nruns,
                      double delthr, double addthr, hipStream_t stream) {
// ... 22 lines not shown
```

### rsicnv_amd/csrc/pipeline.hip

```cpp
#include <new>
#include "pipeline_internal.h"
#include "geno_host.h"
#include "pipeline_steps.h"

using namespace rsik;
using namespace rsip;
using rsih::Candidate;
using rsih::Region;

namespace {

struct ScanOut {
  double tmedian1 = 0, tsigma1 = 0, tlamda1 = 0, tmedian2 = 0, tsigma2 = 0, tlamda2 = 0;
  int Lmax = 0;
  rsih::IntSpan status2;
  std::vector<int> run_status;
  std::vector<rsih::IntSpan::Range> run_ranges;
  std::vector<Candidate> segs;
  uint32_t escapes = 0, inexact = 0;
  uint32_t tiles_listed = 0;
  std::vector<uint32_t> level_log[4];
  uint32_t stop_levels[4] = {0, 0, 0, 0};
  std::vector<std::string> fs_lines;
};
// ... 25 lines not shown
int grid_median(rsi_ctx* ctx, const float* d_x, const int32_t* d_mask, int64_t nb, int use_abs, double center,
                double* med, uint64_t* count) {
  uint8_t* small = ctx->small.as<uint8_t>();
  { Timer t(ctx, "minmax_f32"); launch_minmax_f32(d_x, d_mask, nb, use_abs, center, reinterpret_cast<MinMaxF*>(small + kOffMinMax), ctx->stream); }
  MinMaxF mm;
  HIPCHK(copy_d2h(ctx, &mm, small + kOffMinMax, sizeof(mm)));
  HIPCHK(hipMemsetAsync(small + kOffMinMax, 0, sizeof(MinMaxF), ctx->stream));
  HIPCHK(CTX_SYNC());
  if (mm.min_inv == 0u) { *count = 0; *med = 0; return RSI_OK; }
  if (mm.nonfinite) return fail(ctx, RSI_ERR_UNSUPPORTED, "non-finite value in the transformed bins");
  const double ymin = rsih::unkey_f32(~mm.min_inv), ymax = rsih::unkey_f32(mm.max_bits);
  if ((ymax - ymin) < 0.01) return selection_mean(ctx, d_x, d_mask, nb, use_abs, center, med, count);
  const size_t np = (size_t)((ymax - ymin) / 0.01 + 2);
  if (np > (64u << 20)) return fail(ctx, RSI_ERR_UNSUPPORTED, "transformed bin range too wide for the 0.01 grid");
  HIPCHK(ctx->hist_f.ensure(np * 4));
  HIPCHK(hipMemsetAsync(ctx->hist_f.p, 0, np * 4, ctx->stream));
  { Timer t(ctx, "hist_f32"); launch_hist_f32(d_x, d_mask, nb, use_abs, center, ymin, ctx->hist_f.as<uint32_t>(), (uint32_t)np, ctx->stream); }
  std::vector<uint32_t> h(np);
  HIPCHK(copy_d2h(ctx, h.data(), ctx->hist_f.p, np * 4));
  HIPCHK(CTX_SYNC());
  uint64_t total = 0;
  for (uint32_t c : h) total += c;
  *count = total;
  *med = rsih::hist_median_grid(h.data(), np, total, ymin);
  return RSI_OK;
}

constexpr uint32_t kGridCap = 1u << 20;
constexpr int32_t kFsListCap = 1 << 20;
struct ChainOut { GridMedian g[2]; uint32_t rawmin_inv; uint32_t pad[15]; };
GridChain grid_chain(rsi_ctx* ctx) {
  uint8_t* small = ctx->small.as<uint8_t>();
  return GridChain{reinterpret_cast<MinMaxF*>(small + kOffMinMax), ctx->hist_f.as<uint32_t>(), kGridCap,
                   reinterpret_cast<unsigned int*>(small + kOffDone) + kDoneBinSlot};
}
int nb_transform(rsi_ctx* ctx, const int64_t* d_binsum, int64_t nb, int m, int64_t ncompact, double RDmedian, double r, rsih::NbLevels& lev,
                 float* raw_out) {
  uint8_t* small = ctx->small.as<uint8_t>();
  hipStream_t st = ctx->stream;
  HIPCHK(ctx->tnb.ensure((size_t)nb * 4));
  HIPCHK(ctx->hist_f.ensure((size_t)kGridCap * 4));
  uint32_t* d_rawmin = reinterpret_cast<uint32_t*>(small + kOffRawMin);
  GridMedian* d_g = reinterpret_cast<GridMedian*>(small + kOffGrid);
  { Timer t(ctx, "nb_raw"); launch_nb_raw(d_binsum, nb, m, ncompact, r, ctx->tnb.as<float>(), d_rawmin, st); }
  if (raw_out) HIPCHK(hipMemcpyAsync(raw_out, ctx->tnb.p, (size_t)nb * 4, hipMemcpyDeviceToHost, st));
  lev = rsih::nb_reference_levels(RDmedian, m, r);
  { Timer t(ctx, "nb_scale"); launch_nb_scale_minmax(ctx->tnb.as<float>(), nb, d_rawmin, lev.med_raw, lev.del_raw, lev.dup_raw, RDmedian, grid_chain(ctx), d_g, st); }
  return RSI_OK;
}
void scan_fill_list(rsi_ctx* ctx, int pass, int64_t nb, FillList& fl) {
  uint8_t* small = ctx->small.as<uint8_t>();
  uint32_t* d_first_del = ctx->first_del.as<uint32_t>();
  const int64_t nbpad = (nb + 3) & ~int64_t(3);
  fill_add(fl, d_first_del, (size_t)(nbpad + nb) * 4, 0xffffffffu);
  fill_add(fl, small + kOffScanPass + (size_t)pass * kScanPassBytes, kScanPassBytes, 0u);
  fill_add(fl, small + kOffCounters, 32, 0u);
  if (pass == 0 && ctx->fs_ws.p) fill_add(fl, ctx->fs_ws.p, level_sums_head_bytes(kMaxL), 0u);
}
int grid_pair_issue(rsi_ctx* ctx, const float* d_x, const int32_t* d_mask, int64_t nb, bool with_median, double center, bool planned,
                    int fill_pass, ChainOut** out) {
  uint8_t* small = ctx->small.as<uint8_t>();
  GridMedian* d_g = reinterpret_cast<GridMedian*>(small + kOffGrid);
  const GridChain gc = grid_chain(ctx);
  ChainOut* slot = static_cast<ChainOut*>(mb_alloc(ctx, sizeof(ChainOut)));
  if (!slot) return fail(ctx, RSI_ERR_INTERNAL, "out of pinned mailbox memory");
  memset(slot, 0, sizeof(*slot));
  GateShared gs(ctx);
  if (with_median) {
    if (!planned) { Timer t(ctx, "minmax_plan"); launch_minmax_plan(d_x, d_mask, nb, 0, 0.0, nullptr, gc, d_g, ctx->stream); }
    { Timer t(ctx, "hist_walk"); launch_hist_walk(d_x, d_mask, nb, 0, 0.0, nullptr, gc, d_g, nullptr, nullptr, ctx->stream); }
    planned = false;
  }
  const double* d_center = with_median ? &d_g->med : nullptr;
  if (!planned) { Timer t(ctx, "minmax_plan"); launch_minmax_plan(d_x, d_mask, nb, 1, center, d_center, gc, d_g + 1, ctx->stream); }
  GridExport ex{};
  ex.src[0] = d_g; ex.dst[0] = slot->g; ex.bytes[0] = 2 * sizeof(GridMedian);
  ex.src[1] = small + kOffRawMin; ex.dst[1] = &slot->rawmin_inv; ex.bytes[1] = 4;
  FillList fl{};
  if (fill_pass >= 0) scan_fill_list(ctx, fill_pass, nb, fl);
  { Timer t(ctx, "hist_walk"); launch_hist_walk(d_x, d_mask, nb, 1, center, d_center, gc, d_g + 1, &ex, &fl, ctx->stream); }
  *out = slot;
  return RSI_OK;
}
struct Selection { const float* d_x; const int32_t* d_mask; int64_t nb; int use_abs; double center; };
int grid_result(rsi_ctx* ctx, const GridMedian& g, const Selection& sel, double* med, uint64_t* count) {
  if (g.flags & kGridEmpty) { *count = 0; *med = 0; return RSI_OK; }
  if (g.flags & kGridNonFinite) return fail(ctx, RSI_ERR_UNSUPPORTED, "non-finite value in the transformed bins");
  if (g.flags & kGridDegenerate) return selection_mean(ctx, sel.d_x, sel.d_mask, sel.nb, sel.use_abs, sel.center, med, count);
  *med = g.med; *count = g.count;
  return RSI_OK;
}

void scan_thresholds(double tmedian, double tlamda, int Lmax, std::vector<double>& del, std::vector<double>& dup) {
  del.assign((size_t)Lmax + 1 + kScanPad, -INFINITY);
  dup.assign((size_t)Lmax + 1 + kScanPad, INFINITY);
  del[0] = -1.0;
  for (int L = 1; L <= Lmax; ++L) {
    const double dL = (double)L, sq = sqrt(dL);
    auto score = [&](double sum) { const float meanf = (float)(sum / dL); return ((double)meanf - tmedian) * sq; };
    del[L] = rsih::last_true([&](double s) { return !(score(s) > -tlamda); });
    dup[L] = rsih::first_true([&](double s) { return !(score(s) < tlamda); });
  }
}

constexpr uint32_t kEagerBounds = 1024;
int runs_from_export(rsi_ctx* ctx, const uint32_t* slot, const uint64_t* d_list, std::vector<Region>& runs) {
  const uint32_t cnt = slot[0];
  runs.clear();
  if (cnt == 0) return RSI_OK;
  if (cnt > kMaxRunEntries) return fail(ctx, RSI_ERR_UNSUPPORTED, "boundary list overflow");
  std::vector<uint64_t> raw(cnt);
  memcpy(raw.data(), slot + 2, (size_t)std::min(cnt, kEagerBounds) * 8);
  if (cnt > kEagerBounds) {
    HIPCHK(copy_d2h(ctx, raw.data() + kEagerBounds, d_list + kEagerBounds, (size_t)(cnt - kEagerBounds) * 8));
    HIPCHK(CTX_SYNC());
  }
  if (!rsih::boundary_pairs(raw.data(), raw.size(), false, runs)) return fail(ctx, RSI_ERR_INTERNAL, "unbalanced run boundaries");
  runs.pop_back();
  return RSI_OK;
}

struct RunArgs { RunsInline inl; bool use_inl = false; int32_t* d_start = nullptr; int32_t* d_end = nullptr; };
int prepare_runs(rsi_ctx* ctx, const std::vector<Region>& runs, RunArgs& ra) {
  const size_t k = runs.size();
  if (k <= (size_t)kRunsInline) {
    memset(&ra.inl, 0, sizeof(ra.inl));
    for (size_t i = 0; i < k; ++i) { ra.inl.se[2 * i] = runs[i].start; ra.inl.se[2 * i + 1] = runs[i].end; }
    ra.use_inl = true;
    return RSI_OK;
  }
  HIPCHK(ctx->run_se.ensure(k * 8 + 64));
  std::vector<int32_t> se(2 * k);
  for (size_t i = 0; i < k; ++i) { se[i] = runs[i].start; se[k + i] = runs[i].end; }
  HIPCHK(copy_h2d(ctx, ctx->run_se.p, se.data(), k * 8));
  ra.use_inl = false;
  ra.d_start = ctx->run_se.as<int32_t>();
  ra.d_end = ctx->run_se.as<int32_t>() + k;
  return RSI_OK;
}

constexpr size_t kCandScratchBytes = size_t(512) << 20;
class DeviceTester : public rsih::NeighbourTester {
 public:
  DeviceTester(rsi_ctx* c, DepthRef rdc, int64_t n, double RDmedian) : ctx(c), d_rdc(rdc), N(n), median(RDmedian) {}
  double kernel_wait_ms = 0;
  int launches = 0;
  int force_split = -1, force_bytes = -1;
  std::vector<CandOut>* sink = nullptr;
  int mailbox_lists = 0, copied_lists = 0;

  bool sharpen(std::vector<Candidate>& L) override {
    if (L.empty()) return true;
    const int nj = (int)L.size();
    EdgeJob* slot = static_cast<EdgeJob*>(mb_alloc(ctx, (size_t)nj * sizeof(EdgeJob)));
    std::vector<EdgeJob> spill;
    EdgeJob* jobs = slot;
    if (!slot) { spill.resize((size_t)nj); jobs = spill.data(); }
    for (int i = 0; i < nj; ++i) jobs[i] = {L[(size_t)i].start, L[(size_t)i].end, L[(size_t)i].type, 0};
    {
      Phase ph(ctx, "cand.ensure");
      if (nj > ctx->sharpen_ws_jobs) {
        const int cap = std::max(256, 2 * nj);
        if (!ok(ctx->sharpen_ws.ensure(sharpen_workspace_bytes(cap)))) return false;
        if (!ok(hipMemsetAsync(ctx->sharpen_ws.p, 0, sharpen_workspace_zero_bytes(cap), ctx->stream))) return false;
        ctx->sharpen_ws_jobs = cap;
      }
// ... 271 lines not shown
    int64_t* d_poff = reinterpret_cast<int64_t*>(d_scratch + poff.back());
    HIPCHK(ctx->items.ensure(items.size() * sizeof(SegItem)));
    HIPCHK(ctx->best.ensure(items.size() * sizeof(BestSeg)));
    HIPCHK(copy_h2d(ctx, d_poff, poff.data(), poff.size() * 8));
    HIPCHK(copy_h2d(ctx, ctx->items.p, items.data(), items.size() * sizeof(SegItem)));
    HIPCHK(ctx->h_status2.ensure((size_t)nb * 4));
    HIPCHK(hipMemcpyAsync(ctx->h_status2.p, d_st2, (size_t)nb * 4, hipMemcpyDeviceToHost, ctx->stream));
    out.status2 = rsih::IntSpan(ctx->h_status2.as<int>(), nb);
    { Timer t(ctx, "run_prefix"); launch_run_prefix(d_T, ctx->run_se.as<int32_t>(), ctx->run_se.as<int32_t>() + kr, nullptr, (int)kr, d_poff, d_scratch, nullptr, nullptr, ctx->stream); }
    { Timer t(ctx, "best_subsegment"); launch_best_items(ctx->items.p, nullptr, (int)items.size(), d_poff, d_scratch, tmedian, ctx->best.as<BestSeg>(), ctx->stream); }
    HIPCHK(copy_d2h(ctx, best.data(), ctx->best.p, items.size() * sizeof(BestSeg)));
    HIPCHK(CTX_SYNC());
  }
  if (form) {
    form->runs = (int)runs.size(); form->items = (int)items.size(); form->inl = inl ? 1 : 0;
    form->mailbox_status = out.status2.ranges ? 1 : 0;
    form->pairs_per_item = pairs_per_item;
    for (const Region& r : runs) if (r.end - r.start + 2 > kBestLds) ++form->unstaged;
  }
  rsih::segments_from_best(runs, items, best.data(), out.status2, tlamda, out.segs);
  return RSI_OK;
}

struct FsForm { int runs = -1, inl = -1, copied = -1, route = 0, has_level0 = 0, trim = 0, leveldel = 0, leveladd = 0; float m0 = 0.0f; };
template <class Synced>
int rsi_filterstatus(rsi_ctx* ctx, const float* d_T, const int32_t* d_st1, int32_t* d_st1f, int64_t nb, int Lmax, double dev,
                     const uint32_t* rslot, Synced&& synced, std::vector<std::string>* fs_lines, FsForm* form) {
  int rc;
  const bool long_scan = Lmax > kMaxL;
  const int nlev = 2 * Lmax + 1;
  uint32_t* fs_slot = long_scan ? nullptr : static_cast<uint32_t*>(mb_alloc(ctx, (size_t)nlev * 8));
  if (!fs_slot && !long_scan) return fail(ctx, RSI_ERR_INTERNAL, "out of pinned mailbox memory");
  if (!long_scan) {
    GateShared gs(ctx);
    Timer t(ctx, "level_sums");
    launch_level_sums(d_T, d_st1, nb, Lmax, ctx->fs_ws.p, kMaxL, kFsListCap, ctx->fs_out.as<float>(),
                      reinterpret_cast<unsigned int*>(ctx->small.as<uint8_t>() + kOffDone) + kDoneBinSlot + 4, fs_slot, ctx->stream);
  }
  { Phase phc(ctx, "fs.wait"); HIPCHK(CTX_SYNC()); }
  if ((rc = synced()) != RSI_OK) return rc;
  {
    Phase phs(ctx, "fs.sums");
    std::vector<float> wsum((size_t)nlev, 0.0f);
    std::vector<int> wcnt((size_t)nlev, 0);
    if (fs_slot) {
      memcpy(wsum.data(), fs_slot, (size_t)nlev * 4);
      memcpy(wcnt.data(), fs_slot + nlev, (size_t)nlev * 4);
    }
    if (form) form->route = long_scan ? 2 : (wcnt[(size_t)Lmax] < 0 ? 1 : 0);
    if (long_scan || wcnt[(size_t)Lmax] < 0) {
      Phase phc(ctx, "fs.copy");
      HIPCHK(ctx->h_T.ensure((size_t)nb * 4));
      HIPCHK(ctx->h_status.ensure((size_t)nb * 4));
      HIPCHK(hipMemcpyAsync(ctx->h_T.p, d_T, (size_t)nb * 4, hipMemcpyDeviceToHost, ctx->stream));
      HIPCHK(hipMemcpyAsync(ctx->h_status.p, d_st1, (size_t)nb * 4, hipMemcpyDeviceToHost, ctx->stream));
      HIPCHK(CTX_SYNC());
      rsih::level_sums_host(ctx->h_T.as<float>(), ctx->h_status.as<int>(), nb, Lmax, wsum, wcnt);
    }
    rsih::LevelChoice lc = rsih::choose_levels(wsum, wcnt, Lmax, dev);
    phs.stop();
    Phase phr(ctx, "fs.runs");
    if (form) { form->has_level0 = lc.has_level0; form->trim = lc.trim; form->leveldel = lc.leveldel; form->leveladd = lc.leveladd; form->m0 = lc.m0; }
    if (lc.has_level0) {
      const float m0 = lc.m0;
      if (fs_lines) *fs_lines = std::move(lc.lines);
      if (lc.trim) {
        std::vector<Region> runs;
        GateShared gs(ctx);
        if ((rc = runs_from_export(ctx, rslot, ctx->runs.as<uint64_t>(), runs)) != RSI_OK) return rc;
        if (form) { form->runs = (int)runs.size(); form->copied = rslot[0] > kEagerBounds ? 1 : 0; form->inl = runs.size() <= (size_t)kRunsInline ? 1 : 0; }
        if (!runs.empty()) {
          RunArgs ra;
          if ((rc = prepare_runs(ctx, runs, ra)) != RSI_OK) return rc;
          Timer t(ctx, "trim_runs");
          launch_trim_runs(d_T, d_st1f, ra.d_start, ra.d_end, ra.use_inl ? &ra.inl : nullptr, (int)runs.size(), (double)m0 - dev, (double)m0 + dev, ctx->stream);
        }
      }
    }
  }
  return RSI_OK;
}

int run_scan(rsi_ctx* ctx, const rsi_params& P, bool use_med, const float* d_T, int64_t nb, double RDmedian,
             double factor, int LmaxBase, ChainOut* first, double nb_med_raw, double nb_del_raw, double nb_dup_raw, ScanOut& out) {
  const int32_t* d_medint = ctx->binmed.as<int32_t>();
  double tmedian, absmed;
  uint64_t cnt;
  int rc;
  rsih::NbScaled lv{0, 0};
  {
    Phase ph(ctx, "scan.quantiles");
    HIPCHK(CTX_SYNC());
    const GridMedian* g = first->g;
    if ((!use_med && (g[0].flags & kGridTooWide)) || (g[1].flags & kGridTooWide)) {
      GateShared gs(ctx);
      if (!use_med) {
        if ((rc = grid_median(ctx, d_T, nullptr, nb, 0, 0.0, &tmedian, &cnt)) != RSI_OK) return rc;
      } else {
        tmedian = RDmedian;
      }
      if ((rc = grid_median(ctx, d_T, nullptr, nb, 1, tmedian, &absmed, &cnt)) != RSI_OK) return rc;
    } else {
      tmedian = RDmedian;
      if (!use_med && (rc = grid_result(ctx, g[0], Selection{d_T, nullptr, nb, 0, 0.0}, &tmedian, &cnt)) != RSI_OK) return rc;
      if (!use_med && (g[0].flags & kGridDegenerate)) rc = grid_median(ctx, d_T, nullptr, nb, 1, tmedian, &absmed, &cnt);
      else rc = grid_result(ctx, g[1], Selection{d_T, nullptr, nb, 1, tmedian}, &absmed, &cnt);
      if (rc != RSI_OK) return rc;
    }
    if (!use_med) {
      lv = rsih::nb_scaled_levels(rsih::unkey_f32(~first->rawmin_inv), nb_med_raw, nb_del_raw, RDmedian);
      (void)nb_dup_raw;
    }
  }
  const rsih::ScanSetup su = rsih::scan_first_pass(use_med, tmedian, absmed, factor, LmaxBase, lv.t0, lv.t2, P.threshold, nb);
  double tsigma = su.tsigma, tlamda = su.tlamda;
  const double target = su.target, dev = su.dev;
  const int Lmax = su.Lmax;
  const bool clipped = su.clipped;
  out.tmedian1 = tmedian; out.tsigma1 = tsigma; out.tlamda1 = tlamda; out.Lmax = su.Lmax_ref;
  if (Lmax > kHardMaxL) return fail(ctx, RSI_ERR_UNSUPPORTED, "scan length Lmax beyond 4194304 bins");
  std::vector<uint32_t> spill1, spill2;
  auto take_record = [&](const uint32_t* w, int pass) -> int {
    const rsih::ScanRecord rec{w, Lmax};
    if (clipped && !rec.sweeps_stopped(nb)) return fail(ctx, RSI_ERR_TOO_SMALL, "fewer bins than the scan length, and a sweep reached them all (the reference exits in runmean)");
    out.escapes += rec.escapes(); out.inexact = rec.inexact(); out.tiles_listed += rec.tiles_listed();
    for (int k = 0; k < 2; ++k) {
      out.level_log[2 * pass + k].assign(rec.level_counts(k), rec.level_counts(k) + Lmax + 1);
      out.stop_levels[2 * pass + k] = rec.stop_level(k);
    }
    return RSI_OK;
  };

  int32_t* d_st1 = ctx->status1.as<int32_t>();
  int32_t* d_st1f = ctx->status1f.as<int32_t>();
  int32_t* d_st2 = ctx->status2.as<int32_t>();
  const uint32_t* wslot = nullptr;
  const uint32_t* rslot = nullptr;
  { Phase ph(ctx, "scan.pass"); GateShared gs(ctx); if ((rc = scan_pass(ctx, 0, d_T, d_medint, nb, RDmedian, tmedian, tlamda, Lmax, d_st1, d_st1f, &wslot, &rslot, &spill1)) != RSI_OK) return rc; }

  Phase ph_filter(ctx, "scan.filterstatus");
  if ((rc = rsi_filterstatus(ctx, d_T, d_st1, d_st1f, nb, Lmax, dev, rslot, [&] { return take_record(wslot, 0); }, &out.fs_lines, nullptr)) != RSI_OK) return rc;
  ph_filter.stop();
  Phase ph_q2(ctx, "scan.quantiles");
  double tmed2;
  uint64_t k = 0;
  ChainOut* second = nullptr;
  if ((rc = grid_pair_issue(ctx, d_T, d_st1f, nb, true, 0.0, false, 1, &second)) != RSI_OK) return rc;
  HIPCHK(CTX_SYNC());
  const GridMedian* g2 = second->g;
  {
    GateShared gs_q2(ctx);
    const bool wide2 = (g2[0].flags & kGridTooWide) != 0;
    if ((rc = wide2 ? grid_median(ctx, d_T, d_st1f, nb, 0, 0.0, &tmed2, &k) : grid_result(ctx, g2[0], Selection{d_T, d_st1f, nb, 0, 0.0}, &tmed2, &k)) != RSI_OK) return rc;
    if (k > (uint64_t)(nb / 2)) {
      tmedian = tmed2;
      if ((rc = (wide2 || (g2[1].flags & (kGridTooWide)) || (g2[0].flags & kGridDegenerate)) ? grid_median(ctx, d_T, d_st1f, nb, 1, tmedian, &absmed, &cnt)
                                                        : grid_result(ctx, g2[1], Selection{d_T, d_st1f, nb, 1, tmedian}, &absmed, &cnt)) != RSI_OK) return rc;
      const rsih::Lamda l2 = rsih::lamda_from_mad(absmed, factor, target);
      tsigma = l2.tsigma; tlamda = l2.tlamda;
    }
  }
  out.tmedian2 = tmedian; out.tsigma2 = tsigma; out.tlamda2 = tlamda;
  ph_q2.stop();
  { Phase ph(ctx, "scan.pass"); GateShared gs(ctx); if ((rc = scan_pass(ctx, 1, d_T, d_medint, nb, RDmedian, tmedian, tlamda, Lmax, d_st2, nullptr, &wslot, &rslot, &spill2)) != RSI_OK) return rc; }
  Phase ph_seg(ctx, "scan.segments");
  GateShared gs_seg(ctx);

  HIPCHK(CTX_SYNC());
  std::vector<Region> runs;
  if ((rc = runs_from_export(ctx, rslot, ctx->runs.as<uint64_t>(), runs)) != RSI_OK) return rc;
  if ((rc = take_record(wslot, 1)) != RSI_OK) return rc;
  return rsi_segments(ctx, d_T, d_st2, nb, runs, tmedian, tlamda, 0, out, nullptr);
}

void to_call(const Candidate& c, rsi_call* o) {
  memset(o, 0, sizeof(*o));
  o->start = c.start; o->end = c.end; o->type = c.type; o->geno = c.geno; o->status = c.status; o->length = c.length;
  const double q1 = c.p1 < 1.0E-10 ? 99 : -10.0 * log(c.p1) / log(10.0);
  o->qscore = (int)q1;
  o->score = c.score; o->p1 = c.p1; o->cnvmed = c.cnvmed; o->cnvsd = c.cnvsd; o->cnviqr = c.cnviqr;
  o->refmed = c.refmed; o->refsd = c.refsd; o->refiqr = c.refiqr;
}

struct PerBase {
  std::vector<Region> noncode;
  int64_t ncompact = 0, nb = 0;
  size_t res_vals = 0;
  std::vector<uint32_t> hres_all;
  double RDmedian = 0;
  bool host_stats = false;
  double mads[31] = {};
};
constexpr size_t kResHead = 256;

static int fetch_i32(rsi_ctx* ctx, const int32_t* d_src, int64_t n, std::vector<int32_t>& out) {
  out.resize((size_t)n);
  HIPCHK(hipMemcpyAsync(out.data(), d_src, (size_t)n * 4, hipMemcpyDeviceToHost, ctx->stream));
  HIPCHK(CTX_SYNC());
  return RSI_OK;
}

int materialize_rd_gc(rsi_ctx* ctx) {
  if (ctx->rd_gc_valid) return RSI_OK;
  if (!ctx->have_gc || !ctx->last_depth) return fail(ctx, RSI_ERR_BAD_ARG, "no GC-adjusted run to build rd_gc from");
  uint8_t* small = ctx->small.as<uint8_t>();
  HIPCHK(ctx->rd_gc.ensure((size_t)(ctx->n + 4) * 4));
  { Timer t(ctx, "gc_materialize", true); launch_gc_materialize(ctx->last_depth, ctx->gcbits.as<uint64_t>(), ctx->n, reinterpret_cast<double*>(small + kOffTable), ctx->rd_gc.as<int32_t>(), reinterpret_cast<unsigned int*>(small + kOffDone) + 4 * kDoneStride, ctx->stream); }
  ctx->rd_gc_valid = true;
  return RSI_OK;
}

int materialize_rdc(rsi_ctx* ctx) {
  if (!ctx->rdc_is_bytes || ctx->rdc_valid) return RSI_OK;
  HIPCHK(ctx->rdc.ensure((size_t)(ctx->ncompact + 4) * 4));
  { Timer t(ctx, "rdc_widen", true); launch_widen_u8(ctx->rdc8.as<uint8_t>(), ctx->ncompact, ctx->rdc.as<int32_t>(), ctx->stream); }
  ctx->rdc_valid = true;
  return RSI_OK;
}

static void issue_k4(rsi_ctx* ctx, const K4Plan& plan, K4Args a) {
  a.src8 = (plan.route == K4Route::bytes || plan.raw ? ctx->rescaled8 : ctx->depth8).as<uint8_t>();
  if (!plan.fixed) a.rtab = a.escapes = nullptr;
  a.raw = plan.raw;
  ctx->k4_form = K4Form{};
  a.form = &ctx->k4_form;
  if (plan.route == K4Route::stream && plan.raw) a.table = nullptr;
  {
    Timer t(ctx, "cap_compact_bin", true);
    switch (plan.route) {
      case K4Route::stream: launch_rescale_compact_stream(a); break;
      case K4Route::joint: launch_rescale_compact_bin8(a); break;
      case K4Route::bytes: launch_cap_compact_bin8(a); break;
      case K4Route::wide16: launch_cap_compact_bin16(a); break;
      case K4Route::int32: launch_cap_compact_bin(a); break;
    }
  }
  if (plan.route == K4Route::stream) { Timer t(ctx, "bin_median", true); launch_bin_median8(a); }
}

int issue_exclude_mask(rsi_ctx* ctx, std::vector<std::pair<int64_t, int64_t>> iv, int64_t n) {
  normalize_intervals(iv, n);
  if (iv.empty()) return RSI_OK;
  if (iv.size() > (size_t)0x7fffffff) return fail(ctx, RSI_ERR_UNSUPPORTED, "more than 2^31 excluded intervals");
  const size_t k = iv.size();
  ctx->excl_host.resize(2 * k);
  for (size_t i = 0; i < k; ++i) { ctx->excl_host[i] = iv[i].first; ctx->excl_host[k + i] = iv[i].second; }
  HIPCHK(ctx->excl_dev.ensure(2 * k * 8));
  HIPCHK(copy_h2d(ctx, ctx->excl_dev.p, ctx->excl_host.data(), 2 * k * 8));
  Timer t(ctx, "exclude_mask", true);
  launch_exclude_mask(ctx->excl_dev.as<int64_t>(), ctx->excl_dev.as<int64_t>() + k, (int)k, iv.front().first, iv.back().second,
                      ctx->gcbits.as<uint64_t>(), ctx->nbits.as<uint64_t>(), ctx->stream);
  return RSI_OK;
}

int per_base_phase(rsi_ctx* ctx, const rsi_params& P, const int32_t* d_depth, const uint8_t* d_fasta, int64_t n, rsi_result* res,
                   PerBase& pb) {
  std::vector<Region>& noncode = pb.noncode;
  PerBaseSwitches sw;
  sw.joint = !env_off("RSI_HOT_JOINT");
  sw.spec = !env_off("RSI_HOT_SPEC");
  sw.k4j_fix = !env_off("RSI_HOT_K4J_FIX");
  sw.k4split = !env_off("RSI_HOT_K4SPLIT");
  sw.nogc_bytes = !env_off("RSI_HOT_NOGC_BYTES");
  sw.k4w = !env_off("RSI_HOT_K4W");
  sw.k1b_inside = env_on("RSI_HOT_K1B_INSIDE");
  struct StreamTurn {
    GpuGate* g = nullptr;
    ~StreamTurn() { if (g) g->unlock(); }
    void release() { if (g) { g->unlock(); g = nullptr; } }
  } hbm_turn;
  if (ctx->gate) {
    Phase ph_wait(ctx, "wait.hbm_turn");
// ... 242 lines not shown
  const int64_t nb = ncompact / P.m;
  S.n_compact = ncompact; S.nbins = nb;
  ctx->ncompact = ncompact; ctx->nb = nb;
  if (ncompact <= 0 || nb < 8) return fail(ctx, RSI_ERR_TOO_SMALL, "nothing left after removing N regions");
  K4Regions inl;
  memset(&inl, 0, sizeof(inl));
  if ((int)noncode.size() <= kRegInline) {
    for (size_t k = 0; k < ct.cbreak.size(); ++k) inl.brk[k] = ct.cbreak[k];
    for (size_t k = 0; k < ct.cum.size(); ++k) inl.cum[k] = ct.cum[k];
  } else {
    std::vector<int64_t> both((size_t)4100 + ct.cum.size(), 0);
    std::copy(ct.cbreak.begin(), ct.cbreak.end(), both.begin());
    std::copy(ct.cum.begin(), ct.cum.end(), both.begin() + 4100);
    HIPCHK(copy_h2d(ctx, d_cbreak, both.data(), both.size() * 8));
  }
  HIPCHK(ctx->rdc.ensure((size_t)(ncompact + 4) * 4));
  HIPCHK(ctx->binmed.ensure((size_t)nb * 4));
  HIPCHK(ctx->binsum.ensure((size_t)nb * 8));
  const size_t res_vals = want_cap && capval < kHistValues - 1 ? (size_t)std::max(capval, 0) + 1 : (size_t)kHistValues;
  size_t exp_bytes = kResHead + res_vals * kResClasses * 4;
  const K4Plan plan = k4_plan(P.gcadjust, want_cap, capval, P.m, ncompact, (int)noncode.size(), deep, joint_ok, sw);
  PhaseParams hpp;
  memcpy(&hpp, head + kOffPhase, sizeof(hpp));
  bool spec_done = false;
  if (spec_slot) {
    const bool ran = spec_slot[3] != kSpecMagic;
    spec_done = ran && (!P.gcadjust || (joint_ok && !deep && !jinfo.esc_pending)) && hpp.regions_ok == 1 && hpp.capval == capval &&
                hpp.nreg == (int32_t)noncode.size() && hpp.ncompact == ncompact && plan.bytes_fit && plan.shape == spec_plan.shape &&
                (int)noncode.size() <= kMaxRegions;
    if (ran && !spec_done) HIPCHK(hipMemsetAsync(ctx->hist_res.p, 0, kResHead + (size_t)256 * kResClasses * 4, st));
    ctx->phases.push_back({spec_done ? "spec.k4j accepted" : "spec.k4j rejected", 1.0});
  }
  uint32_t* exp_slot = spec_done ? spec_slot : (exp_bytes <= kMailboxMaxCopy ? static_cast<uint32_t*>(mb_alloc(ctx, exp_bytes)) : nullptr);
  if (spec_done) {
    ctx->rdc_is_bytes = true;
    for (const char* mark : spec_plan.marks)
      if (mark) ctx->phases.push_back({mark, 1.0});
  } else {
    int vbase = 0;
    if (plan.route == K4Route::wide16 || plan.route == K4Route::int32) {
      if (P.gcadjust) {
        const int rcm = materialize_rd_gc(ctx);
        if (rcm != RSI_OK) return rcm;
        d_src = ctx->rd_gc.as<int32_t>();
      }
      vbase = want_cap ? hist_window_base(S.cap_median, kK4Window) : (P.gcadjust ? hist_window_base(S.gc_rdmean, kK4Window) : 0);
      if (plan.route == K4Route::wide16 || !cap_compact_overwrites(P.m, capval, ncompact, vbase)) HIPCHK(hipMemsetAsync(d_res, 0, res_vals * kResClasses * 4, st));
      HIPCHK(ctx->slabs.ensure(plan.route == K4Route::wide16 ? cap_compact16_slab_bytes(P.m, ncompact) : cap_compact_slab_bytes(P.m, capval, ncompact, vbase)));
    } else {
      HIPCHK(ctx->slabs.ensure(cap_compact8_slab_bytes(P.m, capval, ncompact)));
      HIPCHK(ctx->rdc8.ensure((size_t)ncompact + 64));
      if (plan.route == K4Route::stream) {
        HIPCHK(ctx->slabs.ensure(rescale_compact_split_slab_bytes(capval, ncompact)));
        HIPCHK(ctx->rdc8.ensure(rescale_compact_split_rdc_bytes(ncompact)));
      }
      ctx->rdc_is_bytes = true;
    }
    for (const char* mark : plan.marks)
      if (mark) ctx->phases.push_back({mark, 1.0});
    K4Args a = k4_args(inl, (int)noncode.size(), ncompact, capval, exp_slot, exp_slot ? exp_bytes : 0);
    a.vbase = vbase;
    issue_k4(ctx, plan, a);
  }
  BinAccum bacc;
  std::vector<uint32_t> hres_all(kResHead / 4 + res_vals * kResClasses);
  if (!exp_slot) HIPCHK(copy_d2h(ctx, hres_all.data(), ctx->hist_res.p, hres_all.size() * 4));
  if (!spec_done) HIPCHK(CTX_SYNC());
  if ((joint_ok || nogc_bytes) && plan.bytes_fit) { ctx->spec_capval = capval; ctx->spec_m = P.m; ctx->spec_cap = (double)P.cap; ctx->spec_gc = P.gcadjust != 0; }
  if (exp_slot) memcpy(hres_all.data(), exp_slot, exp_bytes);
  memcpy(&bacc, hres_all.data(), sizeof(bacc));
  const uint32_t* hres = hres_all.data() + kResHead / 4;
  if (bacc.big) {
    Phase ph_h(ctx, "a6.statistics on the host (depth > 65535)");
    if (ctx->rdc_is_bytes) return fail(ctx, RSI_ERR_INTERNAL, "values beyond the histogram on the byte path");
    std::vector<int32_t> rd;
    const int rcf = fetch_i32(ctx, ctx->rdc.as<int32_t>(), ncompact, rd);
    if (rcf != RSI_OK) return rcf;
    rsih::ChromStats cs;
    rsih::array_chrom_stats(rd, cs, pb.mads);
    const double RDmed = cs.median;
    S.RDsd = cs.sd;
    S.RDmedian = RDmed;
    pb.host_stats = true;
    pb.ncompact = ncompact; pb.nb = nb; pb.res_vals = 0; pb.RDmedian = RDmed;
    return RSI_OK;
  }
  rsih::ChromStats cs;
  if (!rsih::hist_chrom_stats(hres, res_vals, ncompact, cs)) return fail(ctx, RSI_ERR_INTERNAL, "empty depth histogram");
  const double RDmedian = cs.median;
  S.RDsd = cs.sd;
  S.RDmedian = RDmedian;
  pb.ncompact = ncompact; pb.nb = nb; pb.res_vals = res_vals; pb.RDmedian = RDmedian;
  pb.hres_all = std::move(hres_all);
  return RSI_OK;
}

int bin_level_stages(rsi_ctx* ctx, const rsi_params& P, int64_t n, rsi_result* res, const PerBase& pb,
                     std::vector<Candidate>& blocks, std::vector<Candidate>& raw, std::vector<Candidate>& kept,
                     std::vector<Candidate>& segs_all) {
  rsi_chrom_stats& S = res->stats;
  uint8_t* small = ctx->small.as<uint8_t>();
  hipStream_t st = ctx->stream;
  const std::vector<Region>& noncode = pb.noncode;
  const int64_t ncompact = pb.ncompact, nb = pb.nb;
  const size_t res_vals = pb.res_vals;
  const uint32_t* hres = pb.hres_all.data() + kResHead / 4;
  const double RDmedian = pb.RDmedian;
  int rc = RSI_OK;

  if (!(RDmedian < 5)) {
    Phase ph_nb(ctx, "a9-10.mad+nb");
    GateShared gs_nb(ctx);
    double mads[31];
    const uint64_t sublen = (uint64_t)(ncompact / 31);
    if (sublen == 0) return fail(ctx, RSI_ERR_TOO_SMALL, "fewer than 31 bases");
    if (pb.host_stats) std::copy(pb.mads, pb.mads + 31, mads);
    else if (!rsih::hist_subsample_mads(hres, res_vals, RDmedian, sublen, mads)) return fail(ctx, RSI_ERR_INTERNAL, "empty MAD histogram");
    const double mad = rsih::grid_quantiles(mads, (size_t)31).med;
    const double r = RDmedian / mad;
    S.nb_mad = mad; S.nb_r = r;
    const double factor = sqrt(2.0 * (1.0 + P.epsilon) * log(3.1E9));
    const int LmaxBase = std::max(20, 10000 / P.m);

    HIPCHK(ctx->first_del.ensure((size_t)(2 * nb + 8) * 4));
    HIPCHK(ctx->status1.ensure((size_t)nb * 4));
    HIPCHK(ctx->status1f.ensure((size_t)nb * 4));
    HIPCHK(ctx->status2.ensure((size_t)nb * 4));
    HIPCHK(ctx->runs.ensure((size_t)kMaxRunEntries * 8));
    HIPCHK(ctx->scan_tiles.ensure((size_t)(nb / 256 + 2) * 4));
    HIPCHK(ctx->fs_ws.ensure(level_sums_workspace_bytes(nb, kFsListCap, kMaxL)));
    HIPCHK(ctx->fs_out.ensure((size_t)(2 * kMaxL + 1) * 8 + 64));

    GridMedian* d_g = reinterpret_cast<GridMedian*>(small + kOffGrid);
    rsih::NbLevels lev;
    if ((rc = nb_transform(ctx, ctx->binsum.as<int64_t>(), nb, P.m, ncompact, RDmedian, r, lev, nullptr)) != RSI_OK) return rc;
    const double med_raw = lev.med_raw, del_raw = lev.del_raw, dup_raw = lev.dup_raw;
    bool nb_planned = true;
    ctx->have_nb = true;

    ph_nb.stop();
    gs_nb.release();
    rsih::CallerInput in;
    int short_neighbourhoods = 0;
    in.short_neighbourhoods = &short_neighbourhoods;
    in.P = P; in.RDmedian = RDmedian; in.RDsd = S.RDsd; in.ncompact = ncompact; in.noncode = &noncode;
    HIPCHK(ctx->h_medint.ensure((size_t)nb * 4));
    struct CopyJoin { rsi_ctx* c; ~CopyJoin() { (void)join_copy(c); } } copy_join{ctx};
    HIPCHK(hipMemcpyAsync(ctx->h_medint.p, ctx->binmed.p, (size_t)nb * 4, hipMemcpyDeviceToHost, ctx->copy_stream));
    ctx->copy_pending = true;
    HIPCHK(hipEventRecord(ctx->copy_ev, ctx->copy_stream));
    ctx->copy_recorded = true;
    in.binmedint = rsih::IntSpan(ctx->h_medint.as<int>(), nb);

    auto do_scan = [&](bool use_med, std::vector<Candidate>& segs) -> int {
      ScanOut so;
      const float* d_T;
      ChainOut* first = nullptr;
      int rc2;
      if (use_med) {
        HIPCHK(ctx->tmed.ensure((size_t)nb * 4));
        { Timer t(ctx, "i32_to_f32"); launch_i32_to_f32_minmax(ctx->binmed.as<int32_t>(), ctx->tmed.as<float>(), nb, RDmedian, grid_chain(ctx), d_g + 1, st); }
        d_T = ctx->tmed.as<float>();
        ctx->have_med = true;
        nb_planned = false;
        if ((rc2 = grid_pair_issue(ctx, d_T, nullptr, nb, false, RDmedian, true, 0, &first)) != RSI_OK) return rc2;
      } else {
        d_T = ctx->tnb.as<float>();
        if ((rc2 = grid_pair_issue(ctx, d_T, nullptr, nb, true, 0.0, nb_planned, 0, &first)) != RSI_OK) return rc2;
        nb_planned = false;
      }
      rc2 = run_scan(ctx, P, use_med, d_T, nb, RDmedian, factor, LmaxBase, first, med_raw, del_raw, dup_raw, so);
      if (rc2 != RSI_OK) return rc2;
      S.nb_tmin = rsih::unkey_f32(~first->rawmin_inv);
      ctx->last_scan_med = use_med;
      S.tmedian1 = so.tmedian1; S.tsigma1 = so.tsigma1; S.tlamda1 = so.tlamda1;
      S.tmedian2 = so.tmedian2; S.tsigma2 = so.tsigma2; S.tlamda2 = so.tlamda2;
      S.Lmax = so.Lmax; S.trim_escapes += (int)so.escapes; S.inexact_sums = (int)so.inexact;
      S.scan_tiles = (int32_t)((nb + 255) / 256); S.scan_tiles_listed = (int32_t)so.tiles_listed;
      for (int w = 0; w < 4; ++w) { res->level_log[w] = so.level_log[w]; res->stop_levels[w] = so.stop_levels[w]; }
      res->fs_lines = so.fs_lines;
      res->log_nb = !use_med;
      for (const Candidate& c : so.segs) segs_all.push_back(c);
      segs = so.segs;
      {
        Phase ph(ctx, "a15.blocks");
        HIPCHK(join_copy(ctx));
        DeviceTester block_tester(ctx, DepthRef{ctx->binmed.p, 4}, nb, RDmedian);
        rsih::CallProfile bprof;
        in.block_tester = env_off("RSI_HOT_BLOCK_BATCH") ? nullptr : &block_tester;
        in.prof = &bprof;
        rsih::test_block_segments(in, so.status2, segs);
        in.block_tester = nullptr;
        in.prof = nullptr;
        if (block_tester.failed) return RSI_ERR_HIP;
        if (bprof.block_batch_hits) ctx->phases.push_back({"a15.block batch hits", (double)bprof.block_batch_hits});
      }
      return RSI_OK;
    };
    std::vector<Candidate> tested;
    if (P.trans != 0) { if ((rc = do_scan(true, tested)) != RSI_OK) return rc; }
    if (P.trans == 0) { if ((rc = do_scan(false, tested)) != RSI_OK) return rc; }
    if (P.trans == 2) {
      std::vector<Candidate> more;
      if ((rc = do_scan(false, more)) != RSI_OK) return rc;
      tested.insert(tested.end(), more.begin(), more.end());
    }
    auto mirror_source = [ctx, ncompact]() -> int32_t* {
      if (materialize_rdc(ctx) != RSI_OK) return nullptr;
      if (ctx->mirror_cap < (size_t)ncompact) {
        if (ctx->mirror) (void)hipHostFree(ctx->mirror);
        ctx->mirror = nullptr;
        ctx->mirror_cap = (size_t)ncompact + (size_t)ncompact / 8 + 1024;
        if (hipHostMalloc(reinterpret_cast<void**>(&ctx->mirror), ctx->mirror_cap * sizeof(int32_t), hipHostMallocDefault) != hipSuccess) {
          ctx->mirror = nullptr; ctx->mirror_cap = 0;
        }
      }
      return ctx->mirror;
    };
    rsih::DepthPager pager(ctx->rdc.as<int32_t>(), ncompact, st, mirror_source, nullptr, 0, ctx->sync_ev);
    rsih::CallProfile prof;
    in.prof = &prof;
    const DepthRef depth_ref = ctx->rdc_is_bytes ? DepthRef{ctx->rdc8.p, 1} : DepthRef{ctx->rdc.p, 4};
    DeviceTester tester(ctx, depth_ref, ncompact, RDmedian);
    const bool host_tests = env_int("RSI_HOT_HOST_CANDIDATES", 0) != 0;
    in.tester = host_tests ? nullptr : &tester;
    { Phase ph(ctx, "a16-19.calls"); rsih::call_from_segments(in, tested, pager, blocks, raw, kept); }
    if (tester.failed) return RSI_ERR_HIP;
    if (short_neighbourhoods) return fail(ctx, RSI_ERR_UNSUPPORTED, "a candidate longer than the neighbourhood left around it (the reference aborts in isitcnv, rsi.cpp:107)");
    if (pager.failed()) return fail(ctx, RSI_ERR_INTERNAL, "no pinned host memory for the candidate stages' depth mirror");
    ctx->phases.push_back({"calls.device(wait)", tester.kernel_wait_ms});
    ctx->phases.push_back({"calls.device_ms", prof.device_ms});
    ctx->phases.push_back({"calls.final", prof.final_tests});
    ctx->phases.push_back({"calls.launches", (double)tester.launches});
    ctx->phases.push_back({"calls.spec_hits", (double)prof.spec_hits});
    ctx->phases.push_back({"calls.single_tests", (double)prof.single_tests});
    ctx->phases.push_back({"calls.host_fallbacks", (double)prof.host_fallbacks});
    ctx->phases.push_back({"calls.fetch", pager.fetch_ms()});
    ctx->phases.push_back({"calls.gather(incl fetch)", prof.gather});
    ctx->phases.push_back({"calls.winmean", prof.winmean});
    ctx->phases.push_back({"calls.quantiles", prof.quantiles});
    ctx->phases.push_back({"calls.variance", prof.variance});
    ctx->phases.push_back({"calls.sharpen", prof.sharpen});
    ctx->phases.push_back({"calls.merge(incl tests)", prof.merge});
    ctx->phases.push_back({"calls.ntests", (double)prof.tests});
  }
  return RSI_OK;
}

int run_enter(rsi_ctx* ctx, const rsi_params& P, const int32_t* d_depth, const uint8_t* d_fasta, int64_t n) {
  ctx->run_m = 0; ctx->run_rdmedian = 0.0;
  if (n <= 0 || n >= (1ll << 31) - 4096) return fail(ctx, RSI_ERR_BAD_ARG, "chromosome length must be in (0, 2^31)");
  if (P.m < 1 || (P.m % 2) != 1) return fail(ctx, RSI_ERR_BAD_ARG, "m must be odd (the reference forces it, rsi.cpp:2061-2064)");
  if (P.m > 3000) return fail(ctx, RSI_ERR_UNSUPPORTED, "bin size above 3000 is not supported by the bin kernel");
  if (((uintptr_t)d_depth & 15) || ((uintptr_t)d_fasta & 15)) return fail(ctx, RSI_ERR_BAD_ARG, "device inputs must be 16-byte aligned");
// ... 925 lines not shown
  return RSI_OK;
}
extern "C" {

int rsi_hot_geno_calls(rsi_ctx* ctx, int m, int ncalls, const int32_t* start, const int32_t* end, rsi_geno_record* out) {
  if (!ctx || ncalls < 0 || m < 1 || (ncalls > 0 && (!start || !end || !out))) return fail(ctx, RSI_ERR_BAD_ARG, "bad argument");
  if (!ctx->run_m || ctx->ncompact <= 0 || !(ctx->rdc_is_bytes ? ctx->rdc8.p : ctx->rdc.p))
    return fail(ctx, RSI_ERR_BAD_ARG, "geno: the context holds no successful run's compacted depth (none yet, the last one failed, or a debug hook has overwritten it)");
  HIPCHK(hipSetDevice(ctx->device));
  if (!ctx_enter(ctx)) return RSI_ERR_HIP;
  mailbox_reset(ctx);
  const int npairs = (int)(ctx->noncode_pairs.size() / 2);
  std::vector<rsigeno::Ranges> lines((size_t)ncalls);
  for (int i = 0; i < ncalls; ++i)
    lines[(size_t)i] = rsigeno::line_ranges(rsigeno::map_line(start[i], end[i], ctx->n, ctx->noncode_pairs.data(), npairs), m, ctx->ncompact);
  return geno_run(ctx, ctx->rdc_is_bytes ? ctx->rdc8.p : ctx->rdc.p, ctx->rdc_is_bytes ? 1 : 4, ctx->ncompact, lines, 0, ctx->run_rdmedian, out);
}

int rsi_hot_last_geno_stats(const rsi_ctx* ctx, rsi_geno_stats* out) {
  if (!ctx || !out) return RSI_ERR_BAD_ARG;
  *out = ctx->geno.stats;
  return RSI_OK;
}

int rsi_hot_debug_geno(rsi_ctx* ctx, const int32_t* depth, int64_t n, int storage, const int32_t* lo, const int32_t* hi, const int32_t* flo0,
                       const int32_t* fhi0, const int32_t* flo1, const int32_t* fhi1, int njobs, int tile, rsi_geno_record* out) {
  if (njobs < 0 || tile < 0 || (njobs > 0 && (!lo || !hi || !flo0 || !fhi0 || !flo1 || !fhi1 || !out))) return fail(ctx, RSI_ERR_BAD_ARG, "bad argument");
  DepthRef ref;
  int rc;
  if ((rc = debug_depth_upload(ctx, depth, n, storage, &ref)) != RSI_OK) return rc;
  std::vector<rsigeno::Ranges> lines((size_t)njobs);
  for (int i = 0; i < njobs; ++i) {
    rsigeno::Ranges& r = lines[(size_t)i];
    r.body.a = lo[i]; r.body.b = hi[i]; r.left.a = flo0[i]; r.left.b = fhi0[i]; r.right.a = flo1[i]; r.right.b = fhi1[i];
  }
  return geno_run(ctx, ref.p, storage, n, lines, tile, 0.0, out);
}

int rsi_hot_debug_grid_median(rsi_ctx* ctx, const float* x, const int32_t* mask, int64_t nb, int mode, double center, double* out,
                              int32_t* info) {
  int rc;
  if (!x || mode < 0 || mode > 2) return fail(ctx, RSI_ERR_BAD_ARG, "bad argument");
  if ((rc = grid_debug_enter(ctx, nb, out, info)) != RSI_OK) return rc;
  HIPCHK(ctx->tnb.ensure((size_t)nb * 4));
  HIPCHK(hipMemcpyAsync(ctx->tnb.p, x, (size_t)nb * 4, hipMemcpyHostToDevice, ctx->stream));
  ctx->have_nb = false;
  const int32_t* d_mask = nullptr;
  if (mask) {
    HIPCHK(ctx->status1f.ensure((size_t)nb * 4));
    HIPCHK(hipMemcpyAsync(ctx->status1f.p, mask, (size_t)nb * 4, hipMemcpyHostToDevice, ctx->stream));
    d_mask = ctx->status1f.as<int32_t>();
  }
  const float* d_x = ctx->tnb.as<float>();
  if (mode == 1) return grid_debug_mad(ctx, d_x, d_mask, nb, center, false, out, info);
  double med = 0, mad = 0;
  uint64_t c0 = 0, c1 = 0;
  if (mode == 2) {
    info[5] = 2;
    if ((rc = grid_median(ctx, d_x, d_mask, nb, 0, 0.0, &med, &c0)) != RSI_OK) return rc;
    if ((rc = grid_median(ctx, d_x, d_mask, nb, 1, med, &mad, &c1)) != RSI_OK) return rc;
  } else {
    ChainOut* co = nullptr;
    if ((rc = grid_pair_issue(ctx, d_x, d_mask, nb, true, 0.0, false, -1, &co)) != RSI_OK) return rc;
    HIPCHK(CTX_SYNC());
    const GridMedian g0 = co->g[0], g1 = co->g[1];
    grid_debug_record(g0, info);
    grid_debug_record(g1, info + 2);
    info[4] = hist_walk_pack16(nb) ? 1 : 0;
    if ((g0.flags | g1.flags) & kGridTooWide) {
      info[5] = 2;
      if ((rc = grid_median(ctx, d_x, d_mask, nb, 0, 0.0, &med, &c0)) != RSI_OK) return rc;
      if ((rc = grid_median(ctx, d_x, d_mask, nb, 1, med, &mad, &c1)) != RSI_OK) return rc;
    } else {
      if ((rc = grid_result(ctx, g0, Selection{d_x, d_mask, nb, 0, 0.0}, &med, &c0)) != RSI_OK) return rc;
      if (g0.flags & kGridDegenerate) { info[5] = 1; rc = grid_median(ctx, d_x, d_mask, nb, 1, med, &mad, &c1); }
      else rc = grid_result(ctx, g1, Selection{d_x, d_mask, nb, 1, med}, &mad, &c1);
      if (rc != RSI_OK) return rc;
    }
  }
  out[0] = med; out[1] = (double)c0; out[2] = mad; out[3] = (double)c1;
  return RSI_OK;
}

int rsi_hot_debug_grid_mad_i32(rsi_ctx* ctx, const int32_t* x, int64_t nb, double center, double* out, int32_t* info) {
  int rc;
  if (!x) return fail(ctx, RSI_ERR_BAD_ARG, "bad argument");
  if ((rc = grid_debug_enter(ctx, nb, out, info)) != RSI_OK) return rc;
  ctx->run_m = 0;
  HIPCHK(ctx->binmed.ensure((size_t)nb * 4));
  HIPCHK(ctx->tmed.ensure((size_t)nb * 4));
  HIPCHK(hipMemcpyAsync(ctx->binmed.p, x, (size_t)nb * 4, hipMemcpyHostToDevice, ctx->stream));
  ctx->have_med = false;
  GridMedian* d_g = reinterpret_cast<GridMedian*>(ctx->small.as<uint8_t>() + kOffGrid);
  { Timer t(ctx, "i32_to_f32"); launch_i32_to_f32_minmax(ctx->binmed.as<int32_t>(), ctx->tmed.as<float>(), nb, center, grid_chain(ctx), d_g + 1, ctx->stream); }
  return grid_debug_mad(ctx, ctx->tmed.as<float>(), nullptr, nb, center, true, out, info);
}

int rsi_hot_phase_times(const rsi_ctx* ctx, const char** names, double* ms, int cap) {
  if (!ctx) return 0;
  int k = 0;
  for (const auto& p : ctx->phases) { if (k < cap) { names[k] = p.first; ms[k] = p.second; } ++k; }
  return k;
}

int rsi_hot_kernel_times(const rsi_ctx* ctx, const char** names, float* ms, int cap) {
  if (!ctx) return 0;
  int k = 0;
  for (const KernelTime& t : ctx->ktimes) {
    if (k < cap) { names[k] = t.name; ms[k] = (float)elapsed_ms(t.a, t.b); }
    ++k;
  }
  return k;
}

int rsi_result_format_row(const rsi_result* r, int i, const char* chrom, char* buf, int cap) {
  if (!r || i < 0 || i >= (int)r->lists[0].size()) return RSI_ERR_BAD_ARG;
  const rsi_call& c = r->lists[0][(size_t)i];
  static const char* kType[3] = {"DEL", "DUP", "UNKNOWN"};
  const int k = snprintf(buf, (size_t)cap, "%s\t%d\t%d\t%s\t%d\t%d\t%g(%g);%g(%g);%g(%g)\tRP=%d;Q0=%g\trsi", chrom, c.start, c.end,
                         kType[c.type < 0 || c.type > 2 ? 2 : c.type], c.qscore, c.end - c.start + 1, c.cnvmed,
                         c.cnviqr / 1.349, c.refmed, c.refiqr / 1.349, r->stats.RDmedian, r->stats.RDsd,
                         (size_t)i < r->rp.size() ? r->rp[(size_t)i] : -1, (size_t)i < r->q0.size() ? r->q0[(size_t)i] : -1.0);
  return k;
}

int rsi_result_log_line(const rsi_result* r, int i, char* buf, int cap) {
  if (!r || i < 0 || !buf || cap <= 0) return 0;
  int left = i;
  if (r->log_nb) {
    if (left == 0) { snprintf(buf, (size_t)cap, "RD median : %g", r->stats.RDmedian); return i + 1; }
    if (left == 1) { snprintf(buf, (size_t)cap, "RD median absolute deviation : %g", r->stats.nb_mad); return i + 1; }
    left -= 2;
  }
  for (int w = 0; w < 4; ++w) {
    if (w == 2) {
      if (left < (int)r->fs_lines.size()) { snprintf(buf, (size_t)cap, "%s", r->fs_lines[(size_t)left].c_str()); return i + 1; }
      left -= (int)r->fs_lines.size();
    }
    const int stop = (int)r->stop_levels[w];
    const std::vector<uint32_t>& h = r->level_log[w];
    if (stop <= 0 || h.empty()) continue;
    if (left >= stop) { left -= stop; continue; }
    const int L = left + 1;
    unsigned long long cum = 0;
    for (int l = 1; l <= L && l < (int)h.size(); ++l) cum += h[(size_t)l];
    const double portion = (double)(int)cum / (double)(int)r->stats.nbins;
    snprintf(buf, (size_t)cap, "%s\t%d\t%d\t%d\t%g", (w & 1) ? "DUP+" : "DEL-", L, (int)cum, (int)r->stats.nbins, portion);
    return i + 1;
  }
  return 0;
}

int rsi_result_summary(const rsi_result* r, int chrom_id, double* out, int max_calls) {
  if (!r || !out || max_calls < 0) return RSI_ERR_BAD_ARG;
  const std::vector<rsi_call>& L = r->lists[0];
  const int stored = (int)std::min<size_t>(L.size(), (size_t)max_calls);
  out[0] = (double)chrom_id; out[1] = r->stats.RDmedian; out[2] = r->stats.RDsd; out[3] = (double)L.size(); out[4] = (double)stored;
  out[5] = out[6] = out[7] = 0.0;
  for (int i = 0; i < stored; ++i) {
    const rsi_call& c = L[(size_t)i];
    double* o = out + RSI_SUMMARY_HEAD + RSI_SUMMARY_CALL * i;
    o[0] = c.start; o[1] = c.end; o[2] = c.type; o[3] = c.qscore; o[4] = c.cnvmed; o[5] = c.cnviqr; o[6] = c.refmed; o[7] = c.refiqr;
  }
  return RSI_SUMMARY_HEAD + RSI_SUMMARY_CALL * stored;
}

// ... 54 lines not shown
```

### rsicnv_amd/csrc/pipeline_internal.h

```cpp
#pragma once
#include <hip/hip_runtime.h>
#include <math.h>
#include <stdio.h>
#include <stdlib.h>
#include <string.h>
#include <time.h>
#include <sys/prctl.h>
#include <fcntl.h>
#include <unistd.h>
#include <sys/stat.h>
#include <algorithm>
#include <atomic>
#include <chrono>
#include <condition_variable>
#include <mutex>
#include <thread>
#include <string>
#include <vector>

#include "../../include/rsi_hot.h"
#include "bam_host.h"
#include "host_calls.h"
#include "hostmath.h"
#include "kernels.h"
// ... 96 lines not shown
  bool log_nb = false;
  rsi_chrom_stats stats;
  rsi_params params;
};

struct rsi_ctx {
  int device = 0;
  hipStream_t stream = nullptr;
  hipEvent_t sync_ev = nullptr;
  hipStream_t copy_stream = nullptr;
  hipEvent_t copy_ev = nullptr;
  bool copy_pending = false, copy_recorded = false;
  std::string err;
  int timing = 0;
  std::string timing_kernel = "cap_compact_bin";
  std::vector<KernelTime> ktimes;
  std::vector<hipEvent_t> event_pool;
  size_t event_next = 0;
  DevBuf in_depth, in_fasta;
  DevBuf in_d8, in_esc;
  PinBuf h_d8;
  DevBuf text_dev[2], text_wg;
  char* text_pin[2] = {nullptr, nullptr};
  size_t text_pin_cap = 0;
  rsi_inflate_stats last_inflate{};
  rsing::BgzfLaunch inflate;
  int bam_read = RSI_BAM_READ_HOST;
  size_t bam_chunk = 0;
  rsi_bam_read_stats last_bam_read{};
  struct BamDev {
    PinBuf cpin[2], wpin;
    DevBuf cdev[2], wdev, guess, segout, lists, rec, reflen;
    rsing::BgzfLaunch inflate[2];
    hipStream_t istream = nullptr;
    hipEvent_t ev[2][4] = {{nullptr, nullptr, nullptr, nullptr}, {nullptr, nullptr, nullptr, nullptr}};
    hipEvent_t find[2] = {nullptr, nullptr};
  } bamdev;
  struct Pairs {
    bool armed = false, valid = false;
    DevBuf tab, words, ws, calls, out;
    size_t cap = 0;
    int64_t n = 0, tid_len = 0;
    int tid = -1, parity = 0;
    int32_t maxspan = 0;
    uint32_t flags = 0;
    std::vector<hipEvent_t> events;
    size_t ev_next = 0;
    rsi_pairs_stats stats{};
  } pairs;
  struct Pin {
    bool armed = false, valid = false, sampled = false;
    DevBuf tab, pool, cursor, rdc, drd, scan, state, bps, out;
    size_t cap = 0, pool_cap = 0;
    int64_t n = 0;
    uint32_t cursor_h = 1;
    bool launched = false;
    hipEvent_t ev[2] = {nullptr, nullptr};
    double t_table_ms = 0;
    rsi_pin_stats stats{};
  } pin;
  struct Geno {
    DevBuf tiles, hist, state, out;
    rsi_geno_stats stats{};
  } geno;
  struct Depth {
    DevBuf acc, dist, tiles, state;
    hipEvent_t ev[2] = {nullptr, nullptr};
    rsi_depth_stats stats{};
  } depth;
  struct Plot {
    DevBuf ws, full, pairs;
    hipEvent_t ev[2] = {nullptr, nullptr};
    rsi_plot_stats stats{};
  } plot;
  int64_t n_in = 0;
  DevBuf gcbits, nbits, rd_gc, rdc, binmed, binsum, tnb, tmed, first_del;
  DevBuf depth8, rescaled8;
  DevBuf slabs;
  DevBuf gsum;
  DevBuf status1, status1f, status2, hist_val, hist_res, hist_f, small, thr, runs, run_se, scratch, items, best;
  DevBuf cand_jobs, cand_chains, cand_outs, cand_i32, cand_i64, cand_mid, cand_hist;
  DevBuf sharpen_ws;
  DevBuf fs_ws, fs_out;
  DevBuf scan_tiles;
  DevBuf scan_ws;
  DevBuf joint_tot;
  int32_t spec_capval = -1; int32_t spec_m = 0; double spec_cap = 0.0; bool spec_gc = true;
  int sharpen_ws_jobs = 0;
  int64_t n = 0, ncompact = 0, nb = 0;
  int run_m = 0; double run_rdmedian = 0.0;
  bool have_gc = false, have_nb = false, have_med = false;
  DevBuf rdc8;
  bool rdc_is_bytes = false, rdc_valid = false;
  bool rd_gc_valid = false;
  const int32_t* last_depth = nullptr;
  int last_scan_med = 0;
  std::vector<int32_t> noncode_pairs;
  rsik::K4Form k4_form;
  std::vector<std::pair<const char*, double>> phases;
  DevBuf scan_work_big;
  PinBuf h_T, h_status, h_status2, h_medint;
  char* mailbox = nullptr;
  size_t mb_cap = 0, mb_used = 0;
  struct Pending { void* dst; const void* src; size_t bytes; };
  std::vector<Pending> pending;
  int32_t* mirror = nullptr;
  size_t mirror_cap = 0;
  GpuGate* gate = nullptr;
  std::atomic<int64_t> reserve_n{0};
  bool poisoned = false;
  bool gate_shared = false;
  std::vector<std::pair<int64_t, int64_t>> excl_armed;
  std::vector<int64_t> excl_host;
  DevBuf excl_dev;
  struct TrackWs {
    void* dev = nullptr; size_t dev_bytes = 0;
    char* pin[2] = {nullptr, nullptr}; size_t pin_bytes = 0;
    void* pin_state = nullptr;
    hipEvent_t ev[12] = {nullptr, nullptr, nullptr, nullptr, nullptr, nullptr, nullptr, nullptr, nullptr, nullptr, nullptr, nullptr};
    void* idx_dev = nullptr; char* idx_pin = nullptr; size_t idx_bytes = 0;
  } track;
  int track_format = RSI_TRACK_TEXT;
  rsi_deflate_stats last_deflate{};
  rsi_track_index* track_index = nullptr;
};

namespace rsip {


#define HIPCHK(expr)                                                                          \
  do {                                                                                        \
    hipError_t e__ = (expr);                                                                  \
    if (e__ != hipSuccess) {                                                                  \
      ctx->err = std::string(#expr) + ": " + hipGetErrorString(e__);                          \
      set_global_error(ctx->err);                                                             \
      return RSI_ERR_HIP;                                                                     \
    }                                                                                         \
  } while (0)

constexpr double kStreamWaitDeadlineMs = 60000.0;
inline hipError_t event_wait(hipEvent_t ev, bool busy_pool = false) {
  static const int spin_env = env_int("RSI_HOT_SPIN", -1);
  const int spins = spin_env >= 0 ? spin_env : (busy_pool ? 50 : 2000);
  hipError_t e = hipSuccess;
  for (int spin = 0; spin < spins; ++spin) {
    e = hipEventQuery(ev);
    if (e != hipErrorNotReady) return e;
  }
  const int slack_before = prctl(PR_GET_TIMERSLACK, 0UL, 0UL, 0UL, 0UL);
  (void)prctl(PR_SET_TIMERSLACK, 2000UL, 0UL, 0UL, 0UL);
  const auto t0 = std::chrono::steady_clock::now();
  for (;;) {
    struct timespec nap = {0, 10000};
    nanosleep(&nap, nullptr);
    e = hipEventQuery(ev);
    if (e != hipErrorNotReady) break;
    if (std::chrono::duration<double, std::milli>(std::chrono::steady_clock::now() - t0).count() > kStreamWaitDeadlineMs) { e = hipErrorLaunchTimeOut; break; }
  }
  if (slack_before > 0) (void)prctl(PR_SET_TIMERSLACK, (unsigned long)slack_before, 0UL, 0UL, 0UL);
  return e;
}
inline hipError_t stream_wait(hipStream_t stream, hipEvent_t ev, bool busy_pool = false) {
  const hipError_t e = hipEventRecord(ev, stream);
  return e != hipSuccess ? e : event_wait(ev, busy_pool);
}

// ... 158 lines not shown
```

### rsicnv_amd/csrc/pipeline_steps.h

```cpp
#pragma once
#include <math.h>
#include <stdio.h>
#include <string.h>
#include <algorithm>
#include <string>
#include <vector>
#include "host_calls.h"
#include "hostmath.h"
#include "kernels.h"

namespace rsih {

inline bool boundary_pairs(const uint64_t* raw, size_t cnt, bool end_exclusive, std::vector<Region>& out) {
  out.clear();
  std::vector<int64_t> s, e;
  for (size_t i = 0; i < cnt; ++i) { const uint64_t v = raw[i]; ((v & 1) ? e : s).push_back((int64_t)(v >> 1)); }
  if (s.size() != e.size()) return false;
  std::sort(s.begin(), s.end());
  std::sort(e.begin(), e.end());
  for (size_t i = 0; i < s.size(); ++i) out.push_back({(int)s[i], (int)(e[i] - (end_exclusive ? 1 : 0))});
  return true;
}

inline float unkey_f32(uint32_t k) {
// ... 21 lines not shown
    t.cbreak[k] = (int64_t)noncode[k].start - t.cum[k];
    t.cum[k + 1] = t.cum[k] + (noncode[k].end - noncode[k].start + 1);
  }
  t.ncompact = n - t.cum.back();
  return t;
}

struct CapMedian { double med; bool beyond; };
inline CapMedian cap_median(const rsik::ValueMedian& vm, int64_t n) {
  CapMedian c;
  c.med = (double)vm.lo;
  if (vm.lo <= vm.hi && (double)vm.hi - (double)vm.lo >= 1.0 && vm.med >= 0) c.med = (double)vm.med;
  c.beyond = (uint64_t)n / 2 > vm.inrange;
  return c;
}
inline int32_t cap_value(double med, double cap) { return (int32_t)(med * cap); }

struct ChromStats { double median = 0, sd = 0; };
inline bool hist_chrom_stats(const uint32_t* hres, size_t res_vals, int64_t ncompact, ChromStats& out) {
  std::vector<uint64_t> hall(res_vals, 0);
  for (size_t v = 0; v < res_vals; ++v) for (int c = 0; c < rsik::kResClasses; ++c) hall[v] += hres[v * rsik::kResClasses + c];
  Quantiles qall;
  if (!hist_quantiles_int(hall.data(), hall.size(), (uint64_t)ncompact, qall)) return false;
  out.median = qall.med;
  {
    unsigned __int128 s1 = 0, s2 = 0;
    for (size_t v = 0; v < res_vals; ++v) { s1 += (unsigned __int128)v * hall[v]; s2 += (unsigned __int128)v * v * hall[v]; }
    const double d1 = (double)s1, d2 = (double)s2;
    const double mean = d1 / double((int)ncompact);
    out.sd = sqrt(d2 / double((int)ncompact) - mean * mean);
  }
  return true;
}
inline bool hist_subsample_mads(const uint32_t* hres, size_t res_vals, double RDmedian, uint64_t sublen, double mads[31]) {
  for (int j = 0; j < 31; ++j) {
    std::vector<uint64_t> hd(res_vals + 1, 0);
    for (size_t v = 0; v < res_vals; ++v) {
      const uint32_t c = hres[v * rsik::kResClasses + j];
      if (!c) continue;
      const int a = (int)fabs((float)(int)v - RDmedian);
      hd[(size_t)a] += c;
    }
    Quantiles qd;
    if (!hist_quantiles_int(hd.data(), hd.size(), sublen, qd)) return false;
    mads[j] = qd.med;
  }
  return true;
}
inline double rank_value_i32(std::vector<int32_t>& v, uint64_t rank) {
  if (v.empty()) return 0.0;
  const auto mm = std::minmax_element(v.begin(), v.end());
  const int32_t lo = *mm.first, hi = *mm.second;
  if ((double)hi - (double)lo < 1.0 || rank == 0) return (double)lo;
  const size_t k = (size_t)std::min<uint64_t>(rank, v.size()) - 1;
  std::nth_element(v.begin(), v.begin() + k, v.end());
  return (double)v[k];
}
inline void array_chrom_stats(const std::vector<int32_t>& rd, ChromStats& out, double mads[31]) {
  const int64_t ncompact = (int64_t)rd.size();
  out.sd = sqrt(variance_pop(rd.data(), (size_t)ncompact));
  const uint64_t sublen = (uint64_t)(ncompact / 31);
  std::vector<int32_t> sub((size_t)sublen);
  std::vector<int32_t> sorted = rd;
  const double RDmed = rank_value_i32(sorted, (uint64_t)ncompact / 2);
  for (int j = 0; j < 31 && sublen > 0; ++j) {
    for (uint64_t k = 0; k < sublen; ++k) sub[(size_t)k] = (int)fabs((float)rd[(size_t)(j + 31 * k)] - RDmed);
    mads[j] = rank_value_i32(sub, sublen / 2);
  }
  out.median = RDmed;
}

struct NbLevels { double med_raw, del_raw, dup_raw; };
inline NbLevels nb_reference_levels(double RDmedian, int m, double r) {
  auto nbf = [&](double sum) {
    const double mm = (double)m;
    return 2.0 * sqrt(r) * log(sqrt((sum + 0.25) / (mm * r - 0.5)) + sqrt(1.0 + (sum + 0.25) / (mm * r - 0.5)));
  };
  return NbLevels{nbf(RDmedian * m), nbf(RDmedian / 2.0 * (double)m), nbf(RDmedian * 1.5 * (double)m)};
}
struct NbScaled { float t0, t2; };
inline NbScaled nb_scaled_levels(double tmin, double nb_med_raw, double nb_del_raw, double RDmedian) {
  const double med_nbt = nb_med_raw - tmin;
  return NbScaled{(float)((nb_del_raw - tmin) / med_nbt * RDmedian), (float)(med_nbt / med_nbt * RDmedian)};
}

struct Lamda { double tsigma, tlamda; };
inline Lamda lamda_from_mad(double absmed, double factor, double target) {
  Lamda l;
  l.tsigma = absmed / 0.6745;
  l.tlamda = factor * l.tsigma;
  l.tlamda = std::max(l.tlamda, target);
  return l;
}
struct ScanSetup { double tsigma, tlamda, target, dev; int cal_max, Lmax_ref, Lmax; bool clipped; };
inline ScanSetup scan_first_pass(bool use_med, double tmedian, double absmed, double factor, int LmaxBase, float t0, float t2,
                                 double threshold, int64_t nb) {
  ScanSetup s;
  if (!use_med) {
    s.target = (t2 - t0) * sqrt(2.5);
    const Lamda l = lamda_from_mad(absmed, factor, s.target);
    s.tsigma = l.tsigma; s.tlamda = l.tlamda;
    const double dnb = fabsf(t2 - t0) + 0.0001;
    const double q = s.tlamda * 2 / dnb;
    s.cal_max = (int)(q * q);
    s.dev = s.tsigma * 3.0;
  } else {
    s.target = tmedian * sqrt(2.0);
    const Lamda l = lamda_from_mad(absmed, factor, s.target);
    s.tsigma = l.tsigma; s.tlamda = l.tlamda;
    if (threshold > 0) s.tlamda = tmedian * threshold;
    const double q = s.tlamda * 4 / (tmedian + 0.001);
    s.cal_max = (int)(q * q);
    s.dev = tmedian * 0.6;
  }
  s.Lmax = LmaxBase;
  if (s.Lmax < s.cal_max) s.Lmax = s.cal_max;
  s.Lmax_ref = s.Lmax;
  s.clipped = s.Lmax > nb;
  if (s.clipped) s.Lmax = (int)nb;
  return s;
}

struct ScanRecord {
  const uint32_t* w;
  int Lmax;
  uint32_t escapes() const { return w[rsik::kScanRecEscapes]; }
  uint32_t inexact() const { return w[rsik::kScanRecInexact]; }
  uint32_t stop_level(int sweep) const { return w[rsik::kScanRecStop + sweep]; }
  uint32_t tiles_listed() const { return w[rsik::kScanRecTiles]; }
  const uint32_t* level_counts(int sweep) const { return w + rsik::kScanRecLevels + (size_t)sweep * rsik::scan_level_stride(Lmax); }
  bool sweeps_stopped(int64_t nb) const {
    for (int k = 0; k < 2; ++k) {
      const uint32_t* cnt = level_counts(k);
      uint64_t cum = 0;
      for (uint32_t L = 0; L <= stop_level(k) && L <= (uint32_t)Lmax; ++L) cum += cnt[L];
      if (!((double)(int)cum / (double)(int)nb > 0.2)) return false;
    }
    return true;
  }
};

inline void level_sums_host(const float* tv, const int* st, int64_t nb, int Lmax, std::vector<float>& wsum, std::vector<int>& wcnt) {
  std::fill(wsum.begin(), wsum.end(), 0.0f);
  std::fill(wcnt.begin(), wcnt.end(), 0);
  float s0 = 0.0f;
  int n0 = 0;
  for (int64_t i = 0; i < nb; ++i) {
    const int sv = st[i];
    if (sv == 0) { s0 += tv[i]; ++n0; }
    else { wsum[(size_t)(sv + Lmax)] += tv[i]; ++wcnt[(size_t)(sv + Lmax)]; }
  }
  wsum[(size_t)Lmax] = s0; wcnt[(size_t)Lmax] = n0;
}
struct LevelChoice {
  bool has_level0 = false, trim = false;
  int lo = 0, hi = 0, leveldel = 0, leveladd = 0;
  float m0 = 0.0f;
  std::vector<std::string> lines;
};
inline LevelChoice choose_levels(const std::vector<float>& wsum, const std::vector<int>& wcnt, int Lmax, double dev) {
  LevelChoice c;
  int lo = 0, hi = 0;
  { int a = 0, b = 2 * Lmax; while (a < b && wcnt[a] == 0) ++a; while (b > a && wcnt[b] == 0) --b; lo = a - Lmax; hi = b - Lmax; }
  const int nl = hi - lo + 1;
  std::vector<float> lsum(wsum.begin() + (lo + Lmax), wsum.begin() + (hi + Lmax + 1));
  std::vector<int> lcnt(wcnt.begin() + (lo + Lmax), wcnt.begin() + (hi + Lmax + 1));
// ... 65 lines not shown
```

Before: 263.5 billion.

## Compute NB transform median/MAD via keyed histogram over capped bin sums

When depth values are capped, each bin sum can take at most m*capval+1 distinct values. The NB transform and its grid median/MAD are therefore computed through a histogram over those keys, with a per-key value table, instead of evaluating the transcendental transform per bin and running separate minmax and histogram passes over floats. This is meant to cut the per-bin log/sqrt work and the extra passes over T. It adds new kernels, a declined-path fallback and an env switch, and the median results must match the float grid path exactly.

```diff
diff --git a/include/rsi_hot.h b/include/rsi_hot.h
--- a/include/rsi_hot.h
+++ b/include/rsi_hot.h
@@ -365,6 +365,8 @@
 int rsi_hot_debug_grid_median(rsi_ctx* ctx, const float* x, const int32_t* mask, int64_t nb, int mode, double center, double* out,
                               int32_t* info);
 int rsi_hot_debug_grid_mad_i32(rsi_ctx* ctx, const int32_t* x, int64_t nb, double center, double* out, int32_t* info);
+int rsi_hot_debug_nb_keyed(rsi_ctx* ctx, const int64_t* binsum, const int32_t* mask, int64_t nb, int m, int64_t K, double RDmedian, double r,
+                           float* T, double* out, int32_t* info);
 
 int rsi_hot_debug_classify(rsi_ctx* ctx, const uint8_t* fasta, int64_t n, const int64_t* start, const int64_t* end, int count,
                            uint64_t* gcbits, uint64_t* nbits);
diff --git a/rsicnv_amd/api.py b/rsicnv_amd/api.py
--- a/rsicnv_amd/api.py
+++ b/rsicnv_amd/api.py
@@ -57,7 +57,7 @@
            "rsi_hot_run_device", "rsi_hot_load_depth_text", "rsi_hot_run_text", "rsi_hot_load_depth_bam", "rsi_hot_run_bam", "rsi_bam_references", "rsi_result_annotate_bam", "rsi_result_summary", "rsi_summary_format_row", "rsi_summary_format_rows", "rsi_result_pairs", "rsi_result_ncalls", "rsi_result_calls", "rsi_result_stats", "rsi_result_noncode",
            "rsi_result_format_row", "rsi_result_free", "rsi_hot_fetch_i32", "rsi_hot_fetch_f32", "rsi_hot_fetch_i64",
            "rsi_hot_kernel_times", "rsi_hot_phase_times", "rsi_hot_set_timing", "rsi_hot_process_setup", "rsi_pool_create", "rsi_pool_destroy", "rsi_pool_workers", "rsi_pool_hw_queues", "rsi_pool_worker",
-           "rsi_pool_set_timing", "rsi_pool_set_timing_kernel", "rsi_hot_set_timing_kernel", "rsi_pool_set_schedule", "rsi_pool_last_error", "rsi_pool_run", "rsi_pool_run_host", "rsi_pool_submit", "rsi_pool_wait", "rsi_plot_expand", "rsi_plot_write_files", "rsi_result_log_line", "rsi_hot_debug_level_sums", "rsi_hot_debug_scan", "rsi_hot_debug_segments", "rsi_hot_debug_sharpen", "rsi_hot_debug_candidate_tests", "rsi_hot_debug_range_sums", "rsi_hot_debug_block_stage", "rsi_hot_debug_merge", "rsi_hot_debug_calls", "rsi_hot_debug_nb_transform", "rsi_hot_debug_filterstatus", "rsi_hot_debug_grid_median", "rsi_hot_debug_grid_mad_i32", "rsi_synth_generate_host", "rsi_synth_generate_device", "rsi_synth_write_depth_text", "rsi_synth_write_fasta", "rsi_synth_append_genome_text",
+           "rsi_pool_set_timing", "rsi_pool_set_timing_kernel", "rsi_hot_set_timing_kernel", "rsi_pool_set_schedule", "rsi_pool_last_error", "rsi_pool_run", "rsi_pool_run_host", "rsi_pool_submit", "rsi_pool_wait", "rsi_plot_expand", "rsi_plot_write_files", "rsi_result_log_line", "rsi_hot_debug_level_sums", "rsi_hot_debug_scan", "rsi_hot_debug_segments", "rsi_hot_debug_sharpen", "rsi_hot_debug_candidate_tests", "rsi_hot_debug_range_sums", "rsi_hot_debug_block_stage", "rsi_hot_debug_merge", "rsi_hot_debug_calls", "rsi_hot_debug_nb_transform", "rsi_hot_debug_nb_keyed", "rsi_hot_debug_filterstatus", "rsi_hot_debug_grid_median", "rsi_hot_debug_grid_mad_i32", "rsi_synth_generate_host", "rsi_synth_generate_device", "rsi_synth_write_depth_text", "rsi_synth_write_fasta", "rsi_synth_append_genome_text",
            "rsi_genome_text_open", "rsi_genome_text_next", "rsi_genome_text_release", "rsi_genome_text_copy_depth",
            "rsi_genome_text_kernel_ms", "rsi_genome_text_close", "rsi_genome_text_last_error", "rsi_hot_run_depth_device",
            "rsi_hot_last_inflate_stats", "rsi_hot_inflate_bgzf", "rsi_genome_text_inflate_stats",
@@ -813,6 +813,19 @@
                                                         raw.ctypes.data, T.ctypes.data, info.ctypes.data))
         return raw, T, info
 
+    def debug_nb_keyed(self, binsum, m, K, RDmedian, r, mask=None):
+        b = np.ascontiguousarray(binsum, dtype=np.int64)
+        mk = None if mask is None else np.ascontiguousarray(mask, dtype=np.int32)
+        assert mk is None or mk.size == b.size
+        T = np.zeros(b.size, dtype=np.float32)
+        out = np.zeros(4, dtype=np.float64)
+        info = np.zeros(8, dtype=np.int32)
+        self.lib.rsi_hot_debug_nb_keyed.argtypes = [C.c_void_p, C.c_void_p, C.c_void_p, C.c_int64, C.c_int, C.c_int64, C.c_double, C.c_double,
+                                                    C.c_void_p, C.c_void_p, C.c_void_p]
+        self._check(self.lib.rsi_hot_debug_nb_keyed(self.ctx, b.ctypes.data, None if mk is None else mk.ctypes.data, b.size, int(m), int(K),
+                                                    float(RDmedian), float(r), T.ctypes.data, out.ctypes.data, info.ctypes.data))
+        return T, out, info
+
     def debug_filterstatus(self, T, status, Lmax, dev):
         t = np.ascontiguousarray(T, dtype=np.float32)
         st = np.ascontiguousarray(status, dtype=np.int32)
diff --git a/rsicnv_amd/csrc/kernels.h b/rsicnv_amd/csrc/kernels.h
--- a/rsicnv_amd/csrc/kernels.h
+++ b/rsicnv_amd/csrc/kernels.h
@@ -150,7 +150,8 @@
                    uint32_t* rawmin_bits, hipStream_t stream);
 struct MinMaxF { uint32_t min_inv, max_bits; unsigned int nonfinite; unsigned int pad; };
 struct GridMedian { double med, ymin; unsigned long long count; uint32_t np, flags; };
-enum { kGridEmpty = 1, kGridNonFinite = 2, kGridDegenerate = 4, kGridTooWide = 8 };
+enum { kGridEmpty = 1, kGridNonFinite = 2, kGridDegenerate = 4, kGridTooWide = 8,
+       kGridDeclined = 16  };
 struct GridChain { MinMaxF* mm; uint32_t* hist; uint32_t cap; unsigned int* counters; };
 struct GridExport { const void* src[2]; void* dst[2]; size_t bytes[2]; };
 
@@ -167,6 +168,13 @@
 void launch_hist_walk(const float* x, const int32_t* mask, int64_t nb, int use_abs, double center, const double* d_center,
                       const GridChain& c, GridMedian* out, const GridExport* ex, const FillList* fill, hipStream_t stream);
 bool hist_walk_pack16(int64_t nb);
+
+constexpr int64_t kNbKeyMax = 1 << 15;
+size_t nb_keys_workspace_bytes();
+void launch_nb_keys(const int64_t* binsum, const int32_t* mask, int64_t nb, int m, int64_t K, double r, double med_raw, double del_raw,
+                    double dup_raw, double RDmedian, void* ws, uint32_t* rawmin_bits, const GridChain& c, GridMedian* g,
+                    const GridExport* ex, const FillList* fill, hipStream_t stream);
+void launch_nb_apply(const int64_t* binsum, int64_t nb, int64_t K, const void* ws, float* T, const FillList* fill, hipStream_t stream);
 
 struct ScanParams {
   int64_t nb;
diff --git a/rsicnv_amd/csrc/kernels_bin.hip b/rsicnv_amd/csrc/kernels_bin.hip
--- a/rsicnv_amd/csrc/kernels_bin.hip
+++ b/rsicnv_amd/csrc/kernels_bin.hip
@@ -21,6 +21,31 @@
   const uint32_t b = __float_as_uint(f);
   return (b & 0x80000000u) ? ~b : (b | 0x80000000u);
 }
+
+__device__ __forceinline__ float nb_raw_value(double sum, double m2, double r) {
+  const double q = (sum + 0.25) / (m2 * r - 0.5);
+  const double t = 2.0 * sqrt(r) * log(sqrt(q) + sqrt(1.0 + q));
+  return (float)t;
+}
+struct NbLevels { double med_raw, del_raw, dup_raw, RDmedian; };
+struct NbScale { double tmin, med_nbt, RDmedian; float lev[3]; };
+__device__ __forceinline__ NbScale nb_scale_constants(uint32_t rawmin_inv, const NbLevels& lv) {
+  const uint32_t key = ~rawmin_inv;
+  NbScale s;
+  s.tmin = (double)__uint_as_float((key & 0x80000000u) ? (key & 0x7fffffffu) : ~key);
+  s.med_nbt = lv.med_raw - s.tmin;
+  s.RDmedian = lv.RDmedian;
+  const double del_s = (lv.del_raw - s.tmin) / s.med_nbt * lv.RDmedian, dup_s = (lv.dup_raw - s.tmin) / s.med_nbt * lv.RDmedian;
+  const double med_s = s.med_nbt / s.med_nbt * lv.RDmedian;
+  s.lev[0] = (float)del_s; s.lev[1] = (float)dup_s; s.lev[2] = (float)med_s;
+  return s;
+}
+__device__ __forceinline__ float nb_scaled_value(float raw, const NbScale& s) {
+  const float v = (float)((double)raw - s.tmin);
+  return (float)((double)v / s.med_nbt * s.RDmedian);
+}
+__device__ __forceinline__ float abs_dev_value(float v, double center) { return (float)fabs((double)v - center); }
+__device__ __forceinline__ bool f32_out_of_range(float v) { return !(fabsf(v) <= 3.0e38f); }
 
 __global__ __launch_bounds__(kThreads) void k_nb_raw(const int64_t* __restrict__ binsum, int64_t nb, int m,
                                                      int64_t ncompact, double r, float* __restrict__ raw,
@@ -31,10 +56,7 @@
     int64_t i2 = b * m + m - 1;
     if (i2 > ncompact - 1) i2 = ncompact - 1;
     const double m2 = (double)(i2 - i1 + 1);
-    const double sum = (double)binsum[b];
-    const double q = (sum + 0.25) / (m2 * r - 0.5);
-    const double t = 2.0 * sqrt(r) * log(sqrt(q) + sqrt(1.0 + q));
-    const float f = (float)t;
+    const float f = nb_raw_value((double)binsum[b], m2, r);
     raw[b] = f;
     const uint32_t k = f32_key(f);
     kmin = k < kmin ? k : kmin;
@@ -51,7 +73,7 @@
 
 __device__ inline float sel_value(const float* __restrict__ x, int64_t i, int use_abs, double center) {
   const float v = x[i];
-  return use_abs ? (float)fabs((double)v - center) : v;
+  return use_abs ? abs_dev_value(v, center) : v;
 }
 
 __device__ __forceinline__ void minmax_body(const float* __restrict__ x, const int32_t* __restrict__ mask, int64_t nb,
@@ -89,17 +111,19 @@
 
 constexpr int kHistRun = 8;
 
+__device__ __forceinline__ uint32_t grid_bucket(float v, double ymin, uint32_t np) {
+  const double idx = ((double)v - ymin) / 0.01 + 0.5;
+  const uint32_t k = (uint32_t)(unsigned long long)idx;
+  return k >= np ? np - 1 : k;
+}
+
 template <bool PACK16 = false>
 __device__ __forceinline__ void hist_body(const float* __restrict__ x, const int32_t* __restrict__ mask, int64_t nb, int use_abs,
                                           double center, double ymin, uint32_t* __restrict__ hist, uint32_t np, int use_lds,
                                           unsigned int* s_h) {
   const uint32_t nl = use_lds ? (np < (uint32_t)use_lds ? np : (uint32_t)use_lds) : 0;
   auto lds_add = [&](uint32_t k, uint32_t c) { if (PACK16) atomicAdd(&s_h[k >> 1], c << ((k & 1u) << 4)); else atomicAdd(&s_h[k], c); };
-  auto bucket = [&](float v) {
-    const double idx = ((double)v - ymin) / 0.01 + 0.5;
-    uint32_t k = (uint32_t)(unsigned long long)idx;
-    return k >= np ? np - 1 : k;
-  };
+  auto bucket = [&](float v) { return grid_bucket(v, ymin, np); };
   __shared__ uint32_t s_wb;
   if (threadIdx.x == 0) s_wb = 0u;
   if (use_lds) { for (uint32_t e = threadIdx.x; e < (PACK16 ? (nl + 1) / 2 : nl); e += kThreads) s_h[e] = 0; }
@@ -124,7 +148,7 @@
     uint32_t pend_k = 0xffffffffu, pend_c = 0;
     const int64_t i0 = c * kHistRun, i1 = i0 + kHistRun < nb ? i0 + kHistRun : nb;
     auto one = [&](float xv) {
-      const float v = use_abs ? (float)fabs((double)xv - center) : xv;
+      const float v = use_abs ? abs_dev_value(xv, center) : xv;
       const uint32_t k = bucket(v);
       if (k != pend_k) {
         if (pend_c) count(pend_k, pend_c);
@@ -167,8 +191,8 @@
 
 __device__ inline float f32_unkey(uint32_t k) { return __uint_as_float((k & 0x80000000u) ? (k & 0x7fffffffu) : ~k); }
 
-__device__ inline void grid_plan_block(MinMaxF* __restrict__ mm, uint32_t cap, uint32_t* __restrict__ hist, GridMedian* __restrict__ g) {
-  const uint32_t kmin = ~ld_cg(&mm->min_inv), kmax = ld_cg(&mm->max_bits), bad = ld_cg(&mm->nonfinite);
+struct GridPlan { uint32_t flags, np; double ymin; };
+__device__ __forceinline__ GridPlan grid_plan_values(uint32_t kmin, uint32_t kmax, uint32_t bad, uint32_t cap) {
   uint32_t flags = 0, np = 0;
   double ymin = 0.0;
   if (kmin == 0xffffffffu) flags = kGridEmpty;
@@ -182,6 +206,13 @@
       if (n > cap) flags = kGridTooWide; else np = (uint32_t)n;
     }
   }
+  return GridPlan{flags, np, ymin};
+}
+__device__ inline void grid_plan_block(MinMaxF* __restrict__ mm, uint32_t cap, uint32_t* __restrict__ hist, GridMedian* __restrict__ g) {
+  const uint32_t kmin = ~ld_cg(&mm->min_inv), kmax = ld_cg(&mm->max_bits), bad = ld_cg(&mm->nonfinite);
+  const GridPlan pl = grid_plan_values(kmin, kmax, bad, cap);
+  const uint32_t flags = pl.flags, np = pl.np;
+  const double ymin = pl.ymin;
   for (uint32_t e = threadIdx.x; e < np; e += kThreads) hist[e] = 0;
   __syncthreads();
   if (threadIdx.x == 0) {
@@ -214,7 +245,7 @@
   uint32_t kmin = 0xffffffffu, kmax = 0;
   unsigned int bad = 0;
   auto one = [&](float xv) {
-    const float v = use_abs ? (float)fabs((double)xv - c) : xv;
+    const float v = use_abs ? abs_dev_value(xv, c) : xv;
     if (!(fabsf(v) <= 3.0e38f)) bad = 1;
     const uint32_t k = f32_key(v);
     kmin = k < kmin ? k : kmin;
@@ -243,11 +274,10 @@
 
 struct ExportPair { const void* src[2]; void* dst[2]; unsigned int bytes[2]; };
 
-__device__ inline void grid_walk_block(const uint32_t* __restrict__ hist, GridMedian* __restrict__ g) {
+__device__ inline void grid_walk_block(const uint32_t* __restrict__ hist, GridMedian* __restrict__ g, const uint32_t np, const double ymin) {
   __shared__ unsigned long long s_sum[kThreads];
   __shared__ unsigned long long s_seen;
   __shared__ unsigned int s_cross;
-  const uint32_t np = g->np;
   const uint32_t chunk = (((np + kThreads - 1) / kThreads) + 3u) & ~3u;
   const uint32_t b0 = threadIdx.x * chunk < np ? threadIdx.x * chunk : np;
   const uint32_t b1 = b0 + chunk < np ? b0 + chunk : np;
@@ -272,7 +302,7 @@
   for (int t = 0; t < kThreads; ++t) { const unsigned long long v = s_sum[t]; if (t < (int)threadIdx.x) seen += v; total += v; }
   const unsigned long long r2 = total / 2;
   unsigned long long* med_bits = reinterpret_cast<unsigned long long*>(&g->med);
-  if (threadIdx.x == 0) { st_cg(&g->count, total); if (r2 == 0) st_cg(med_bits, (unsigned long long)__double_as_longlong(g->ymin)); }
+  if (threadIdx.x == 0) { st_cg(&g->count, total); if (r2 == 0) st_cg(med_bits, (unsigned long long)__double_as_longlong(ymin)); }
   if (r2 != 0 && mine != 0 && seen < r2 && seen + mine >= r2) { s_cross = b0; s_seen = seen; }
   __syncthreads();
   const uint32_t cb = s_cross;
@@ -292,7 +322,7 @@
   if (part != 0 && run < r2 && run + part >= r2) {
     for (uint32_t bb = m0; bb < m1; ++bb) {
       const unsigned long long upto = run + ld_cg(hist + bb);
-      if (run < r2 && upto >= r2) st_cg(med_bits, (unsigned long long)__double_as_longlong(g->ymin + (double)bb * 0.01));
+      if (run < r2 && upto >= r2) st_cg(med_bits, (unsigned long long)__double_as_longlong(ymin + (double)bb * 0.01));
       run = upto;
     }
   }
@@ -311,27 +341,20 @@
     hist_body<PACK16>(x, mask, nb, use_abs, center_ptr ? *center_ptr : center, g->ymin, hist, np, (int)lds_bins, s_h);
   }
   if (!last_block_done(counter)) return;
-  if (!g->flags) grid_walk_block(hist, g);
+  if (!g->flags) grid_walk_block(hist, g, g->np, g->ymin);
   sync_drained();
   for (int k = 0; k < 2; ++k) export_words(ex.dst[k], ex.src[k], ex.bytes[k]);
 }
 
-struct NbLevels { double med_raw, del_raw, dup_raw, RDmedian; };
 __global__ __launch_bounds__(kThreads) void k_nb_scale_mm(float* __restrict__ x, int64_t nb, const uint32_t* __restrict__ rawmin_inv,
                                                           NbLevels lv, MinMaxF* __restrict__ mm, unsigned int* __restrict__ counter,
                                                           uint32_t cap, uint32_t* __restrict__ hist, GridMedian* __restrict__ g) {
-  const uint32_t key = ~(*rawmin_inv);
-  const double tmin = (double)__uint_as_float((key & 0x80000000u) ? (key & 0x7fffffffu) : ~key);
-  const double med_nbt = lv.med_raw - tmin;
-  const double del_s = (lv.del_raw - tmin) / med_nbt * lv.RDmedian, dup_s = (lv.dup_raw - tmin) / med_nbt * lv.RDmedian;
-  const double med_s = med_nbt / med_nbt * lv.RDmedian;
-  const float lev0 = (float)del_s, lev1 = (float)dup_s, lev2 = (float)med_s;
+  const NbScale sc = nb_scale_constants(*rawmin_inv, lv);
+  const float lev0 = sc.lev[0], lev1 = sc.lev[1], lev2 = sc.lev[2];
   uint32_t kmin = 0xffffffffu, kmax = 0;
   unsigned int bad = 0;
   for (int64_t b = (int64_t)blockIdx.x * kThreads + threadIdx.x; b < nb; b += (int64_t)gridDim.x * kThreads) {
-    float v = x[b];
-    v = (float)((double)v - tmin);
-    v = (float)((double)v / med_nbt * lv.RDmedian);
+    float v = nb_scaled_value(x[b], sc);
     if (b == 0) v = lev0;
     if (b == 1) v = lev1;
     if (b == 2) v = lev2;
@@ -361,6 +384,180 @@
   }
   minmax_commit(kmin, kmax, bad, mm);
   if (last_block_done(counter)) grid_plan_block(mm, cap, hist, g);
+}
+
+constexpr uint32_t kKeyLds = 16384;
+constexpr uint32_t kKeyPad = (uint32_t)kNbKeyMax + 8;
+constexpr int64_t kKeySliceMax = 61440;
+struct NbKeyArgs {
+  const int64_t* binsum; const int32_t* mask; int64_t nb, slice;
+  int m; uint32_t K; double r; NbLevels lv;
+  uint32_t* keyhist; float* tval; uint32_t* occ_key; uint32_t* occ_cnt; uint32_t* occ_val; uint32_t* flag;
+  uint32_t* rawmin_inv; unsigned int* counter; uint32_t cap; uint32_t* hist; GridMedian* g;
+};
+
+__device__ inline void block_minmax(uint32_t& kmin, uint32_t& kmax, unsigned int& bad) {
+  __shared__ uint32_t s_bmin[kThreads / 64], s_bmax[kThreads / 64], s_bbad[kThreads / 64];
+  for (int d = 32; d >= 1; d >>= 1) {
+    const uint32_t a = __shfl_xor(kmin, d), b = __shfl_xor(kmax, d);
+    kmin = a < kmin ? a : kmin; kmax = b > kmax ? b : kmax; bad |= __shfl_xor(bad, d);
+  }
+  __syncthreads();
+  if (lane_id() == 0) { s_bmin[threadIdx.x >> 6] = kmin; s_bmax[threadIdx.x >> 6] = kmax; s_bbad[threadIdx.x >> 6] = bad; }
+  __syncthreads();
+  kmin = s_bmin[0]; kmax = s_bmax[0]; bad = s_bbad[0];
+  for (int w = 1; w < kThreads / 64; ++w) { kmin = s_bmin[w] < kmin ? s_bmin[w] : kmin; kmax = s_bmax[w] > kmax ? s_bmax[w] : kmax; bad |= s_bbad[w]; }
+}
+__device__ inline void grid_record_store(GridMedian* g, double med, double ymin, unsigned long long count, uint32_t np, uint32_t flags) {
+  unsigned long long* w = reinterpret_cast<unsigned long long*>(g);
+  static_assert(sizeof(GridMedian) == 32, "four 64-bit words");
+  st_cg(w + 0, (unsigned long long)__double_as_longlong(med));
+  st_cg(w + 1, (unsigned long long)__double_as_longlong(ymin));
+  st_cg(w + 2, count);
+  st_cg(w + 3, (unsigned long long)np | ((unsigned long long)flags << 32));
+}
+__device__ inline void keyed_link(const uint32_t* occ_cnt, const uint32_t* occ_val, uint32_t n, int use_abs, double c, uint32_t cap,
+                                  uint32_t* hist, GridMedian* g) {
+  uint32_t kmin = 0xffffffffu, kmax = 0;
+  unsigned int bad = 0;
+  for (uint32_t i = threadIdx.x; i < n; i += kThreads) {
+    const float xv = __uint_as_float(ld_cg(occ_val + i));
+    const float v = use_abs ? abs_dev_value(xv, c) : xv;
+    if (f32_out_of_range(v)) bad = 1;
+    const uint32_t k = f32_key(v);
+    kmin = k < kmin ? k : kmin;
+    kmax = k > kmax ? k : kmax;
+  }
+  block_minmax(kmin, kmax, bad);
+  const GridPlan pl = grid_plan_values(kmin, kmax, bad, cap);
+  for (uint32_t e = threadIdx.x; e < pl.np; e += kThreads) st_cg(hist + e, 0u);
+  if (threadIdx.x == 0) grid_record_store(g, 0.0, pl.ymin, 0ull, pl.np, pl.flags);
+  sync_drained();
+  if (pl.flags) return;
+  for (uint32_t i = threadIdx.x; i < n; i += kThreads) {
+    const float xv = __uint_as_float(ld_cg(occ_val + i));
+    const float v = use_abs ? abs_dev_value(xv, c) : xv;
+    atomicAdd(&hist[grid_bucket(v, pl.ymin, pl.np)], ld_cg(occ_cnt + i));
+  }
+  sync_drained();
+  grid_walk_block(hist, g, pl.np, pl.ymin);
+  sync_drained();
+}
+
+template <bool MASKED>
+__global__ __launch_bounds__(kThreads) void k_nb_keys(NbKeyArgs a, ExportPair ex, FillList fill) {
+  __shared__ unsigned int s_k[kKeyLds / 2];
+  __shared__ unsigned int s_n;
+  fill_ranges(fill);
+  const uint32_t K = a.K;
+  const uint32_t nl = K < kKeyLds ? K : kKeyLds;
+  for (uint32_t e = threadIdx.x; e < (nl + 1) / 2; e += kThreads) s_k[e] = 0;
+  __syncthreads();
+  {
+    const int64_t b0 = (int64_t)blockIdx.x * a.slice, b1 = b0 + a.slice < a.nb ? b0 + a.slice : a.nb;
+    unsigned int outside = 0;
+    auto one = [&](int64_t b, int64_t s) {
+      if (b < 3) { atomicAdd(&a.keyhist[K + (uint32_t)b], 1u); return; }
+      if (s < 0 || s >= (int64_t)K) { outside = 1; return; }
+      const uint32_t k = (uint32_t)s;
+      if (k < nl) atomicAdd(&s_k[k >> 1], 1u << ((k & 1u) << 4)); else atomicAdd(&a.keyhist[k], 1u);
+    };
+    int64_t b = b0 + threadIdx.x;
+    for (; b + 3 * kThreads < b1; b += 4 * kThreads) {
+      int64_t sv[4]; int mv[4] = {0, 0, 0, 0};
+#pragma unroll
+      for (int e = 0; e < 4; ++e) sv[e] = a.binsum[b + e * kThreads];
+      if (MASKED) {
+#pragma unroll
+        for (int e = 0; e < 4; ++e) mv[e] = a.mask[b + e * kThreads];
+      }
+#pragma unroll
+      for (int e = 0; e < 4; ++e) if (mv[e] == 0) one(b + e * kThreads, sv[e]);
+    }
+    for (; b < b1; b += kThreads) {
+      if (MASKED && a.mask[b] != 0) continue;
+      one(b, a.binsum[b]);
+    }
+    if (outside) atomicOr(a.flag, 1u);
+  }
+  __syncthreads();
+  for (uint32_t e = threadIdx.x; e < nl; e += kThreads) {
+    const unsigned int c = (s_k[e >> 1] >> ((e & 1u) << 4)) & 0xffffu;
+    if (c) atomicAdd(&a.keyhist[e], c);
+  }
+  if (!last_block_done(a.counter)) return;
+
+  if (threadIdx.x == 0) s_n = 0;
+  __syncthreads();
+  const uint32_t declined = ld_cg(a.flag);
+  {
+    const uint32_t nq = (K + 3 + 3) / 4;
+    const __amdgpu_buffer_rsrc_t rs = coherent_buffer(a.keyhist);
+    for (uint32_t q0 = threadIdx.x; q0 < nq; q0 += 4 * kThreads) {
+      u32x4 v[4];
+#pragma unroll
+      for (int j = 0; j < 4; ++j) { const uint32_t q = q0 + j * kThreads; v[j] = ld_cg_buf_x4(rs, (q < nq ? q : q0) * 16u, 0u); }
+#pragma unroll
+      for (int j = 0; j < 4; ++j) {
+        const uint32_t q = q0 + j * kThreads;
+        if (q >= nq) continue;
+        const unsigned int c[4] = {v[j].x, v[j].y, v[j].z, v[j].w};
+#pragma unroll
+        for (int e = 0; e < 4; ++e) {
+          if (!c[e]) continue;
+          const uint32_t slot = atomicAdd(&s_n, 1u);
+          st_cg(a.occ_key + slot, q * 4u + e);
+          st_cg(a.occ_cnt + slot, c[e]);
+          st_cg(a.keyhist + q * 4u + e, 0u);
+        }
+      }
+    }
+  }
+  sync_drained();
+  const uint32_t n = s_n;
+  if (declined) {
+    if (threadIdx.x == 0) { grid_record_store(a.g, 0.0, 0.0, 0ull, 0u, kGridDeclined); grid_record_store(a.g + 1, 0.0, 0.0, 0ull, 0u, 0u); st_cg(a.flag, 0u); }
+  } else {
+    const double m2 = (double)a.m;
+    auto slot_sum = [&](uint32_t key) { return key < K ? (double)key : (double)a.binsum[key - K]; };
+    if (!MASKED) {
+      uint32_t kmin = 0xffffffffu, kmax = 0;
+      unsigned int bad = 0;
+      for (uint32_t i = threadIdx.x; i < n; i += kThreads) {
+        const uint32_t k = f32_key(nb_raw_value(slot_sum(ld_cg(a.occ_key + i)), m2, a.r));
+        kmin = k < kmin ? k : kmin;
+      }
+      block_minmax(kmin, kmax, bad);
+      if (threadIdx.x == 0) st_cg(a.rawmin_inv, ~kmin);
+      const NbScale sc = nb_scale_constants(~kmin, a.lv);
+      for (uint32_t i = threadIdx.x; i < n; i += kThreads) {
+        const uint32_t key = ld_cg(a.occ_key + i);
+        const float v = key < K ? nb_scaled_value(nb_raw_value((double)key, m2, a.r), sc) : key == K ? sc.lev[0] : key == K + 1 ? sc.lev[1] : sc.lev[2];
+        a.tval[key] = v;
+        st_cg(a.occ_val + i, __float_as_uint(v));
+      }
+    } else {
+      for (uint32_t i = threadIdx.x; i < n; i += kThreads) st_cg(a.occ_val + i, __float_as_uint(a.tval[ld_cg(a.occ_key + i)]));
+    }
+    sync_drained();
+    keyed_link(a.occ_cnt, a.occ_val, n, 0, 0.0, a.cap, a.hist, a.g);
+    const double med = __longlong_as_double((long long)ld_cg(reinterpret_cast<const unsigned long long*>(&a.g->med)));
+    keyed_link(a.occ_cnt, a.occ_val, n, 1, med, a.cap, a.hist, a.g + 1);
+  }
+  sync_drained();
+  for (int k = 0; k < 2; ++k) export_words(ex.dst[k], ex.src[k], ex.bytes[k]);
+}
+
+__global__ __launch_bounds__(kThreads) void k_nb_apply(const int64_t* __restrict__ binsum, int64_t nb, uint32_t K, const float* __restrict__ tval,
+                                                       float* __restrict__ T, FillList fill) {
+  fill_ranges(fill);
+  for (int64_t b = (int64_t)blockIdx.x * kThreads + threadIdx.x; b < nb; b += (int64_t)gridDim.x * kThreads) {
+    const int64_t s = binsum[b];
+    float v = 0.0f;
+    if (b < 3) v = tval[K + (uint32_t)b];
+    else if (s >= 0 && s < (int64_t)K) v = tval[s];
+    T[b] = v;
+  }
 }
 
 constexpr int kScanTile = 256;
@@ -1177,6 +1374,40 @@
   if (pack16) RSI_LAUNCH(k_hist_walk<true>, dim3(grid), dim3(kThreads), lds, stream, x, mask, nb, use_abs, center, d_center, out, c.hist, c.counters + 1, e, f, bins);
   else { RSI_ALLOW_FULL_LDS(k_hist_walk<false>); RSI_LAUNCH(k_hist_walk<false>, dim3(grid), dim3(kThreads), lds, stream, x, mask, nb, use_abs, center, d_center, out, c.hist, c.counters + 1, e, f, bins); }
 }
+size_t nb_keys_workspace_bytes() { return (size_t)(5 * kKeyPad + 4) * 4; }
+static NbKeyArgs nb_key_args(const int64_t* binsum, const int32_t* mask, int64_t nb, int m, int64_t K, double r, const NbLevels& lv, void* ws,
+                             uint32_t* rawmin_bits, const GridChain& c, GridMedian* g) {
+  uint32_t* w = static_cast<uint32_t*>(ws);
+  NbKeyArgs a{};
+  a.binsum = binsum; a.mask = mask; a.nb = nb;
+  a.slice = (((nb + 127) / 128) + 255) & ~int64_t(255);
+  if (a.slice < 1024) a.slice = 1024;
+  if (a.slice > kKeySliceMax) a.slice = kKeySliceMax;
+  a.m = m; a.K = (uint32_t)K; a.r = r; a.lv = lv;
+  a.keyhist = w; a.tval = reinterpret_cast<float*>(w + kKeyPad); a.occ_key = w + 2 * kKeyPad; a.occ_cnt = w + 3 * kKeyPad;
+  a.occ_val = w + 4 * kKeyPad; a.flag = w + 5 * kKeyPad;
+  a.rawmin_inv = rawmin_bits; a.counter = c.counters; a.cap = c.cap; a.hist = c.hist; a.g = g;
+  return a;
+}
+void launch_nb_keys(const int64_t* binsum, const int32_t* mask, int64_t nb, int m, int64_t K, double r, double med_raw, double del_raw,
+                    double dup_raw, double RDmedian, void* ws, uint32_t* rawmin_bits, const GridChain& c, GridMedian* g,
+                    const GridExport* ex, const FillList* fill, hipStream_t stream) {
+  if (K < 1 || K > kNbKeyMax || nb < 3) { if (tl_launch_error == hipSuccess) tl_launch_error = hipErrorInvalidValue; return; }
+  const NbKeyArgs a = nb_key_args(binsum, mask, nb, m, K, r, NbLevels{med_raw, del_raw, dup_raw, RDmedian}, ws, rawmin_bits, c, g);
+  const int grid = (int)((nb + a.slice - 1) / a.slice);
+  ExportPair e{};
+  if (ex) for (int k = 0; k < 2; ++k) { e.src[k] = ex->src[k]; e.dst[k] = ex->dst[k]; e.bytes[k] = (unsigned int)ex->bytes[k]; }
+  FillList f{};
+  if (fill) f = *fill;
+  if (mask) RSI_LAUNCH(k_nb_keys<true>, dim3(grid), dim3(kThreads), 0, stream, a, e, f);
+  else RSI_LAUNCH(k_nb_keys<false>, dim3(grid), dim3(kThreads), 0, stream, a, e, f);
+}
+void launch_nb_apply(const int64_t* binsum, int64_t nb, int64_t K, const void* ws, float* T, const FillList* fill, hipStream_t stream) {
+  FillList f{};
+  if (fill) f = *fill;
+  RSI_LAUNCH(k_nb_apply, dim3(bounded_grid(nb, kThreads * 4, 512)), dim3(kThreads), 0, stream, binsum, nb, (uint32_t)K,
+             reinterpret_cast<const float*>(static_cast<const uint32_t*>(ws) + kKeyPad), T, f);
+}
 constexpr int kGTileGrid = 256;
 constexpr size_t kGTileBudget = size_t(8) << 30;
 struct ScanShape { int count, kcap, grid; bool gtile, wide; size_t tile_bytes; };
diff --git a/rsicnv_amd/csrc/pipeline.hip b/rsicnv_amd/csrc/pipeline.hip
--- a/rsicnv_amd/csrc/pipeline.hip
+++ b/rsicnv_amd/csrc/pipeline.hip
@@ -131,6 +131,38 @@
   *out = slot;
   return RSI_OK;
 }
+static_assert(rsih::kNbKeyLimit == kNbKeyMax, "the route's limit is the kernels' table size");
+struct NbKeyed { int64_t K = 0; const int64_t* d_binsum = nullptr; int m = 0; int64_t ncompact = 0; double r = 0, RDmedian = 0; rsih::NbLevels lev{0, 0, 0}; };
+int nb_keyed_issue(rsi_ctx* ctx, const NbKeyed& kd, const int32_t* d_mask, int64_t nb, int fill_pass, ChainOut** out) {
+  uint8_t* small = ctx->small.as<uint8_t>();
+  GridMedian* d_g = reinterpret_cast<GridMedian*>(small + kOffGrid);
+  hipStream_t st = ctx->stream;
+  HIPCHK(ctx->tnb.ensure((size_t)nb * 4));
+  HIPCHK(ctx->hist_f.ensure((size_t)kGridCap * 4));
+  const bool fresh = ctx->nb_keys.p == nullptr;
+  HIPCHK(ctx->nb_keys.ensure(nb_keys_workspace_bytes()));
+  if (fresh) HIPCHK(hipMemsetAsync(ctx->nb_keys.p, 0, nb_keys_workspace_bytes(), st));
+  ChainOut* slot = static_cast<ChainOut*>(mb_alloc(ctx, sizeof(ChainOut)));
+  if (!slot) return fail(ctx, RSI_ERR_INTERNAL, "out of pinned mailbox memory");
+  memset(slot, 0, sizeof(*slot));
+  GridExport ex{};
+  ex.src[0] = d_g; ex.dst[0] = slot->g; ex.bytes[0] = 2 * sizeof(GridMedian);
+  ex.src[1] = small + kOffRawMin; ex.dst[1] = &slot->rawmin_inv; ex.bytes[1] = 4;
+  FillList fl{};
+  if (fill_pass >= 0) scan_fill_list(ctx, fill_pass, nb, fl);
+  uint32_t* d_rawmin = reinterpret_cast<uint32_t*>(small + kOffRawMin);
+  GateShared gs(ctx);
+  if (!d_mask) {
+    { Timer t(ctx, "nb_keys"); launch_nb_keys(kd.d_binsum, nullptr, nb, kd.m, kd.K, kd.r, kd.lev.med_raw, kd.lev.del_raw, kd.lev.dup_raw, kd.RDmedian, ctx->nb_keys.p, d_rawmin, grid_chain(ctx), d_g, &ex, nullptr, st); }
+    { Timer t(ctx, "nb_apply"); launch_nb_apply(kd.d_binsum, nb, kd.K, ctx->nb_keys.p, ctx->tnb.as<float>(), &fl, st); }
+  } else {
+    Timer t(ctx, "nb_keys_masked");
+    launch_nb_keys(kd.d_binsum, d_mask, nb, kd.m, kd.K, kd.r, kd.lev.med_raw, kd.lev.del_raw, kd.lev.dup_raw, kd.RDmedian, ctx->nb_keys.p, d_rawmin, grid_chain(ctx), d_g, &ex, &fl, st);
+  }
+  *out = slot;
+  return RSI_OK;
+}
+
 struct Selection { const float* d_x; const int32_t* d_mask; int64_t nb; int use_abs; double center; };
 int grid_result(rsi_ctx* ctx, const GridMedian& g, const Selection& sel, double* med, uint64_t* count) {
   if (g.flags & kGridEmpty) { *count = 0; *med = 0; return RSI_OK; }
@@ -568,7 +600,7 @@
 }
 
 int run_scan(rsi_ctx* ctx, const rsi_params& P, bool use_med, const float* d_T, int64_t nb, double RDmedian,
-             double factor, int LmaxBase, ChainOut* first, double nb_med_raw, double nb_del_raw, double nb_dup_raw, ScanOut& out) {
+             double factor, int LmaxBase, ChainOut*& first, double nb_med_raw, double nb_del_raw, double nb_dup_raw, NbKeyed* keyed, ScanOut& out) {
   const int32_t* d_medint = ctx->binmed.as<int32_t>();
   double tmedian, absmed;
   uint64_t cnt;
@@ -577,6 +609,14 @@
   {
     Phase ph(ctx, "scan.quantiles");
     HIPCHK(CTX_SYNC());
+    if (keyed && keyed->K && (first->g[0].flags & kGridDeclined)) {
+      ctx->phases.push_back({"nb.keyed declined", 1.0});
+      rsih::NbLevels lev;
+      if ((rc = nb_transform(ctx, keyed->d_binsum, nb, keyed->m, keyed->ncompact, RDmedian, keyed->r, lev, nullptr)) != RSI_OK) return rc;
+      if ((rc = grid_pair_issue(ctx, d_T, nullptr, nb, true, 0.0, true, 0, &first)) != RSI_OK) return rc;
+      keyed->K = 0;
+      HIPCHK(CTX_SYNC());
+    }
     const GridMedian* g = first->g;
     if ((!use_med && (g[0].flags & kGridTooWide)) || (g[1].flags & kGridTooWide)) {
       GateShared gs(ctx);
@@ -631,8 +671,14 @@
   double tmed2;
   uint64_t k = 0;
   ChainOut* second = nullptr;
-  if ((rc = grid_pair_issue(ctx, d_T, d_st1f, nb, true, 0.0, false, 1, &second)) != RSI_OK) return rc;
+  const bool keyed2 = keyed && keyed->K && Lmax <= kMaxL;
+  if ((rc = keyed2 ? nb_keyed_issue(ctx, *keyed, d_st1f, nb, 1, &second) : grid_pair_issue(ctx, d_T, d_st1f, nb, true, 0.0, false, 1, &second)) != RSI_OK) return rc;
   HIPCHK(CTX_SYNC());
+  if (keyed2 && (second->g[0].flags & kGridDeclined)) {
+    ctx->phases.push_back({"nb.keyed declined", 1.0});
+    if ((rc = grid_pair_issue(ctx, d_T, d_st1f, nb, true, 0.0, false, 1, &second)) != RSI_OK) return rc;
+    HIPCHK(CTX_SYNC());
+  }
   const GridMedian* g2 = second->g;
   {
     GateShared gs_q2(ctx);
@@ -674,6 +720,7 @@
   size_t res_vals = 0;
   std::vector<uint32_t> hres_all;
   double RDmedian = 0;
+  int32_t capval = 0; bool capped = false;
   bool host_stats = false;
   double mads[31] = {};
 };
@@ -1082,6 +1129,7 @@
     S.RDsd = cs.sd;
     S.RDmedian = RDmed;
     pb.host_stats = true;
+    pb.capval = capval; pb.capped = want_cap;
     pb.ncompact = ncompact; pb.nb = nb; pb.res_vals = 0; pb.RDmedian = RDmed;
     return RSI_OK;
   }
@@ -1090,6 +1138,7 @@
   const double RDmedian = cs.median;
   S.RDsd = cs.sd;
   S.RDmedian = RDmedian;
+  pb.capval = capval; pb.capped = want_cap;
   pb.ncompact = ncompact; pb.nb = nb; pb.res_vals = res_vals; pb.RDmedian = RDmedian;
   pb.hres_all = std::move(hres_all);
   return RSI_OK;
@@ -1133,10 +1182,18 @@
 
     GridMedian* d_g = reinterpret_cast<GridMedian*>(small + kOffGrid);
     rsih::NbLevels lev;
-    if ((rc = nb_transform(ctx, ctx->binsum.as<int64_t>(), nb, P.m, ncompact, RDmedian, r, lev, nullptr)) != RSI_OK) return rc;
+    NbKeyed keyed;
+    const int64_t nkeys = pb.capped ? rsih::nb_key_count(P.m, pb.capval) : 0;
+    if (!env_off("RSI_HOT_NB_KEYED") && rsih::nb_keyed_applies(P.trans == 0, pb.capped && pb.capval >= 0, nkeys, nb, LmaxBase > kMaxL)) {
+      keyed.K = nkeys; keyed.d_binsum = ctx->binsum.as<int64_t>(); keyed.m = P.m; keyed.ncompact = ncompact; keyed.r = r; keyed.RDmedian = RDmedian;
+      keyed.lev = lev = rsih::nb_reference_levels(RDmedian, P.m, r);
+      ctx->phases.push_back({"nb.keyed", 1.0});
+    } else {
+      if ((rc = nb_transform(ctx, ctx->binsum.as<int64_t>(), nb, P.m, ncompact, RDmedian, r, lev, nullptr)) != RSI_OK) return rc;
+      ctx->have_nb = true;
+    }
     const double med_raw = lev.med_raw, del_raw = lev.del_raw, dup_raw = lev.dup_raw;
     bool nb_planned = true;
-    ctx->have_nb = true;
 
     ph_nb.stop();
     gs_nb.release();
@@ -1165,11 +1222,15 @@
         nb_planned = false;
         if ((rc2 = grid_pair_issue(ctx, d_T, nullptr, nb, false, RDmedian, true, 0, &first)) != RSI_OK) return rc2;
       } else {
+        if (keyed.K) {
+          if ((rc2 = nb_keyed_issue(ctx, keyed, nullptr, nb, 0, &first)) != RSI_OK) return rc2;
+          ctx->have_nb = true;
+        }
         d_T = ctx->tnb.as<float>();
-        if ((rc2 = grid_pair_issue(ctx, d_T, nullptr, nb, true, 0.0, nb_planned, 0, &first)) != RSI_OK) return rc2;
+        if (!keyed.K && (rc2 = grid_pair_issue(ctx, d_T, nullptr, nb, true, 0.0, nb_planned, 0, &first)) != RSI_OK) return rc2;
         nb_planned = false;
       }
-      rc2 = run_scan(ctx, P, use_med, d_T, nb, RDmedian, factor, LmaxBase, first, med_raw, del_raw, dup_raw, so);
+      rc2 = run_scan(ctx, P, use_med, d_T, nb, RDmedian, factor, LmaxBase, first, med_raw, del_raw, dup_raw, use_med ? nullptr : &keyed, so);
       if (rc2 != RSI_OK) return rc2;
       S.nb_tmin = rsih::unkey_f32(~first->rawmin_inv);
       ctx->last_scan_med = use_med;
@@ -2261,6 +2322,69 @@
   return RSI_OK;
 }
 
+int rsi_hot_debug_nb_keyed(rsi_ctx* ctx, const int64_t* binsum, const int32_t* mask, int64_t nb, int m, int64_t K, double RDmedian, double r,
+                           float* T, double* out, int32_t* info) {
+  int rc;
+  if (!ctx || !binsum || !T || m < 1 || !(r > 0.0) || nb < 3) return fail(ctx, RSI_ERR_BAD_ARG, "bad argument");
+  if ((rc = grid_debug_enter(ctx, nb, out, info)) != RSI_OK) return rc;
+  info[0] = info[2] = -1; info[4] = 0;
+  ctx->ktimes.clear(); ctx->event_next = 0; ctx->phases.clear();
+  ctx->nb = nb; ctx->run_m = 0;
+  ctx->have_nb = false;
+  if (!rsih::nb_keyed_applies(true, true, K, nb, false)) { info[5] = -1; return RSI_OK; }
+  uint8_t* small = ctx->small.as<uint8_t>();
+  HIPCHK(ctx->binsum.ensure((size_t)nb * 8));
+  HIPCHK(hipMemcpyAsync(ctx->binsum.p, binsum, (size_t)nb * 8, hipMemcpyHostToDevice, ctx->stream));
+  HIPCHK(hipMemsetAsync(small + kOffRawMin, 0, 4, ctx->stream));
+  const int32_t* d_mask = nullptr;
+  if (mask) {
+    HIPCHK(ctx->status1f.ensure((size_t)nb * 4));
+    HIPCHK(hipMemcpyAsync(ctx->status1f.p, mask, (size_t)nb * 4, hipMemcpyHostToDevice, ctx->stream));
+    d_mask = ctx->status1f.as<int32_t>();
+  }
+  NbKeyed kd;
+  kd.K = K; kd.d_binsum = ctx->binsum.as<int64_t>(); kd.m = m; kd.ncompact = nb * m; kd.r = r; kd.RDmedian = RDmedian;
+  kd.lev = rsih::nb_reference_levels(RDmedian, m, r);
+  ChainOut* co = nullptr;
+  if ((rc = nb_keyed_issue(ctx, kd, nullptr, nb, -1, &co)) != RSI_OK) return rc;
+  HIPCHK(CTX_SYNC());
+  info[5] = 1;
+  const float* d_x = ctx->tnb.as<float>();
+  if (co->g[0].flags & kGridDeclined) {
+    info[5] = 0;
+    rsih::NbLevels lev;
+    if ((rc = nb_transform(ctx, kd.d_binsum, nb, m, kd.ncompact, RDmedian, r, lev, nullptr)) != RSI_OK) return rc;
+    if ((rc = grid_pair_issue(ctx, d_x, nullptr, nb, true, 0.0, true, -1, &co)) != RSI_OK) return rc;
+    if (d_mask && (rc = grid_pair_issue(ctx, d_x, d_mask, nb, true, 0.0, false, -1, &co)) != RSI_OK) return rc;
+    HIPCHK(CTX_SYNC());
+  } else if (d_mask) {
+    if ((rc = nb_keyed_issue(ctx, kd, d_mask, nb, -1, &co)) != RSI_OK) return rc;
+    HIPCHK(CTX_SYNC());
+    if (co->g[0].flags & kGridDeclined) return fail(ctx, RSI_ERR_INTERNAL, "the masked keyed form declined sums the unmasked one took");
+  }
+  const GridMedian g0 = co->g[0], g1 = co->g[1];
+  const float tmin = rsih::unkey_f32(~co->rawmin_inv);
+  HIPCHK(hipMemcpyAsync(T, ctx->tnb.p, (size_t)nb * 4, hipMemcpyDeviceToHost, ctx->stream));
+  HIPCHK(CTX_SYNC());
+  grid_debug_record(g0, info);
+  grid_debug_record(g1, info + 2);
+  memcpy(&info[4], &tmin, 4);
+  double med = 0, mad = 0;
+  uint64_t c0 = 0, c1 = 0;
+  if ((g0.flags | g1.flags) & kGridTooWide) {
+    info[6] = 2;
+    if ((rc = grid_median(ctx, d_x, d_mask, nb, 0, 0.0, &med, &c0)) != RSI_OK) return rc;
+    if ((rc = grid_median(ctx, d_x, d_mask, nb, 1, med, &mad, &c1)) != RSI_OK) return rc;
+  } else {
+    if ((rc = grid_result(ctx, g0, Selection{d_x, d_mask, nb, 0, 0.0}, &med, &c0)) != RSI_OK) return rc;
+    if (g0.flags & kGridDegenerate) { info[6] = 1; rc = grid_median(ctx, d_x, d_mask, nb, 1, med, &mad, &c1); }
+    else rc = grid_result(ctx, g1, Selection{d_x, d_mask, nb, 1, med}, &mad, &c1);
+    if (rc != RSI_OK) return rc;
+  }
+  out[0] = med; out[1] = (double)c0; out[2] = mad; out[3] = (double)c1;
+  return RSI_OK;
+}
+
 int rsi_hot_debug_grid_mad_i32(rsi_ctx* ctx, const int32_t* x, int64_t nb, double center, double* out, int32_t* info) {
   int rc;
   if (!x) return fail(ctx, RSI_ERR_BAD_ARG, "bad argument");
diff --git a/rsicnv_amd/csrc/pipeline_internal.h b/rsicnv_amd/csrc/pipeline_internal.h
--- a/rsicnv_amd/csrc/pipeline_internal.h
+++ b/rsicnv_amd/csrc/pipeline_internal.h
@@ -202,6 +202,7 @@
   DevBuf cand_jobs, cand_chains, cand_outs, cand_i32, cand_i64, cand_mid, cand_hist;
   DevBuf sharpen_ws;
   DevBuf fs_ws, fs_out;
+  DevBuf nb_keys;
   DevBuf scan_tiles;
   DevBuf scan_ws;
   DevBuf joint_tot;
diff --git a/rsicnv_amd/csrc/pipeline_steps.h b/rsicnv_amd/csrc/pipeline_steps.h
--- a/rsicnv_amd/csrc/pipeline_steps.h
+++ b/rsicnv_amd/csrc/pipeline_steps.h
@@ -127,6 +127,12 @@
 inline NbScaled nb_scaled_levels(double tmin, double nb_med_raw, double nb_del_raw, double RDmedian) {
   const double med_nbt = nb_med_raw - tmin;
   return NbScaled{(float)((nb_del_raw - tmin) / med_nbt * RDmedian), (float)(med_nbt / med_nbt * RDmedian)};
+}
+
+constexpr int64_t kNbKeyLimit = 1 << 15;
+inline int64_t nb_key_count(int m, int32_t capval) { return (int64_t)m * (int64_t)capval + 1; }
+inline bool nb_keyed_applies(bool nb_route, bool capped, int64_t K, int64_t nb, bool long_scan) {
+  return nb_route && capped && K >= 1 && K <= kNbKeyLimit && nb >= 8 && !long_scan;
 }
 
 struct Lamda { double tsigma, tlamda; };
```

Result: faster. 275.8 billion, median of 6 (+4.6%).
